# JaronTu/Multimodal_MVD_Seg

Measured on AMD Instinct MI355X. Metric: train-step samples/sec on 4-modality 128^3 patches (PlainConvUNet 3d_fullres, fp32), higher is better.
Workload: dtype f32; 1 GPU; BASELINE configs[1]: PlainConvUNet 3d_fullres 6 stages 31.2M params, 4x128x128x128 patch, 5 classes, fp32, DC+CE deep supervision, SGD-Nesterov+clip; per_gpu_batch=2, global_batch=2, parallelism=dp1, step_launch=one hipGraph replay per step (captured after 3 eager steps)

## Files before the change

include/mvdseg_hip.h:

```cpp
#ifndef MVDSEG_HIP_H
#define MVDSEG_HIP_H
#include <stddef.h>
#include <stdint.h>

#ifdef __cplusplus
extern "C" {
#endif

#define MVD_VERSION 100
#define MVD_MAX_TAPS 27

int mvd_version(void);
const char *mvd_last_error(void);
int mvd_has_mfma(void);
int mvd_set_conv_engine(int mode);
int mvd_set_wino_min_items(long n);

int mvd_pack_weight(const float *w, float *wf, float *wb, int K, int C, int T, int transposed, void *stream);

size_t mvd_conv_fwd_workspace_bytes(int N, long out_voxels, int K);
int mvd_conv3d_fwd(const float *x1, int C1, const float *x2, int C2, const float *wf, const float *bias, float *y,
                   int N, int D, int H, int W, int K, const int ksize[3], const int stride[3], void *ws,
                   size_t ws_bytes, void *stream);
int mvd_conv3d_dgrad(const float *dy, const float *wb, float *dx1, int C1, float *dx2, int C2, int N, int D, int H,
                     int W, int K, const int ksize[3], const int stride[3], void *ws, size_t ws_bytes, void *stream);
int mvd_conv_wino_applicable(int N, int D, int H, int W, int C1, int C2, int K, const int ksize[3], const int stride[3]);
size_t mvd_wino_weight_elems(int C, int K);
int mvd_wino_mode(void);
int mvd_pack_weight_wino(const float *w, float *uf, float *ub, int K, int C, void *stream);
int mvd_pack_weights_batch(int n, const float *const *w, float *const *wf, float *const *wb, float *const *uf,
                           float *const *ub, const int *K, const int *C, const int *T, const int *transposed,
                           void *stream);
int mvd_conv3d_fwd_wino(const float *x1, int C1, const float *x2, int C2, const float *wf, const float *uf,
                        const float *bias, float *y, int N, int D, int H, int W, int K, const int ksize[3],
                        const int stride[3], void *ws, size_t ws_bytes, void *stream);
size_t mvd_conv_stats_tiles(int D, int H, int W);
int mvd_conv3d_fwd_wino_stats(const float *x1, int C1, const float *x2, int C2, const float *wf, const float *uf,
                              const float *bias, float *y, float *stats, int *stats_done, int N, int D, int H, int W,
                              int K, const int ksize[3], const int stride[3], void *ws, size_t ws_bytes, void *stream);
int mvd_conv3d_dgrad_wino(const float *dy, const float *wb, const float *ub, float *dx1, int C1, float *dx2, int C2, int N,
                          int D, int H, int W, int K, const int ksize[3], const int stride[3], void *ws, size_t ws_bytes,
                          void *stream);
int mvd_set_wino3_min_items(long n);
int mvd_conv_wino3_applicable(int N, int D, int H, int W, int C1, int C2, int K, const int ksize[3], const int stride[3]);
size_t mvd_wino3_weight_elems(int C, int K);
int mvd_pack_weight_wino3(const float *w, float *vf, float *vb, int K, int C, void *stream);
int mvd_pack_weights_batch3(int n, const float *const *w, float *const *wf, float *const *wb, float *const *uf,
                            float *const *ub, float *const *vf, float *const *vb, const int *K, const int *C,
                            const int *T, const int *transposed, void *stream);
int mvd_conv3d_fwd_wino3(const float *x1, int C1, const float *x2, int C2, const float *wf, const float *vf,
                         const float *bias, float *y, int N, int D, int H, int W, int K, const int ksize[3],
                         const int stride[3], void *ws, size_t ws_bytes, void *stream);
int mvd_conv3d_fwd_wino3_stats(const float *x1, int C1, const float *x2, int C2, const float *wf, const float *vf,
                               const float *bias, float *y, float *stats, int *stats_done, int N, int D, int H, int W,
                               int K, const int ksize[3], const int stride[3], void *ws, size_t ws_bytes, void *stream);
int mvd_conv3d_dgrad_wino3(const float *dy, const float *wb, const float *vb, float *dx1, int C1, float *dx2, int C2,
                           int N, int D, int H, int W, int K, const int ksize[3], const int stride[3], void *ws,
                           size_t ws_bytes, void *stream);
int mvd_set_wgrad_wino3_min_items(long n);
int mvd_conv_wgrad_wino3_applicable(int N, int D, int H, int W, int C1, int C2, int K, const int ksize[3],
                                    const int stride[3]);
long mvd_wgrad_wino3_launches(void);
size_t mvd_conv3d_wgrad_workspace_bytes(int C, int K, int T, int N, int Do, int Ho, int Wo);
int mvd_conv3d_wgrad(const float *x1, int C1, const float *x2, int C2, const float *dy, float *dw, float *dbias,
                     int N, int D, int H, int W, int K, const int ksize[3], const int stride[3], void *ws,
                     size_t ws_bytes, void *stream);

int mvd_convT3d_fwd(const float *x, const float *wf, const float *bias, float *y, int N, int D, int H, int W, int C,
                    int K, const int stride[3], void *ws, size_t ws_bytes, void *stream);
int mvd_convT3d_dgrad(const float *dy, const float *wb, float *dx, int N, int D, int H, int W, int C, int K,
                      const int stride[3], void *ws, size_t ws_bytes, void *stream);
size_t mvd_convT3d_wgrad_workspace_bytes(int C, int K, int T, int N, int D, int H, int W);
int mvd_convT3d_wgrad(const float *x, const float *dy, float *dw, float *dbias, int N, int D, int H, int W, int C,
                      int K, const int stride[3], void *ws, size_t ws_bytes, void *stream);

int mvd_pack_weight_bf16(const float *w, uint16_t *wf, uint16_t *wb, int K, int C, int T, int transposed, void *stream);
int mvd_pack_weights_bf16_batch(int n, const float *const *w, uint16_t *const *wf, uint16_t *const *wb, const int *K,
                                const int *C, const int *T, const int *transposed, void *stream);
int mvd_pack_weights_bf16_batch_pad(int n, const float *const *w, uint16_t *const *wf, uint16_t *const *wb, const int *K,
                                    const int *C, const int *T, const int *transposed, const int *Csrc, void *stream);
int mvd_conv3d_fwd_bf16(const uint16_t *x1, int C1, const uint16_t *x2, int C2, const uint16_t *wf, const float *bias,
                        uint16_t *y, int N, int D, int H, int W, int K, const int ksize[3], const int stride[3],
                        void *ws, size_t ws_bytes, void *stream);
int mvd_conv3d_dgrad_bf16(const uint16_t *dy, const uint16_t *wb, uint16_t *dx1, int C1, uint16_t *dx2, int C2, int N,
                          int D, int H, int W, int K, const int ksize[3], const int stride[3], void *ws, size_t ws_bytes,
                          void *stream);
int mvd_convT3d_fwd_bf16(const uint16_t *x, const uint16_t *wf, const float *bias, uint16_t *y, int N, int D, int H, int W,
                         int C, int K, const int stride[3], void *ws, size_t ws_bytes, void *stream);
int mvd_convT3d_dgrad_bf16(const uint16_t *dy, const uint16_t *wb, uint16_t *dx, int N, int D, int H, int W, int C, int K,
                           const int stride[3], void *ws, size_t ws_bytes, void *stream);
int mvd_conv3d_wgrad_bf16(const uint16_t *x1, int C1, const uint16_t *x2, int C2, const uint16_t *dy, float *dw,
                          float *dbias, int N, int D, int H, int W, int K, const int ksize[3], const int stride[3],
                          void *ws, size_t ws_bytes, void *stream);
int mvd_convT3d_wgrad_bf16(const uint16_t *x, const uint16_t *dy, float *dw, float *dbias, int N, int D, int H, int W,
                           int C, int K, const int stride[3], void *ws, size_t ws_bytes, void *stream);
// ... 30 lines not shown
                                const float *mean, const float *rstd, void *dx, float *dgamma, float *dbeta, int N,
                                long V, int C, float slope, void *ws, size_t ws_bytes, void *stream);
int mvd_seghead_fwd_bf16(const uint16_t *x, const float *w, const float *bias, float *logits, int N, long V, int C,
                         int K, void *stream);
int mvd_seghead_bwd_bf16(const uint16_t *x, const float *w, const float *dlogits, uint16_t *dx, float *dw, float *dbias,
                         int N, long V, int C, int K, int accumulate, void *ws, size_t ws_bytes, void *stream);
int mvd_seghead_bf16_fused_ok(int N, long V, int C, int K);
int mvd_seghead_fwd_fused(const float *x, const float *mean, const float *rstd, const float *gamma, const float *beta, float slope,
                          const float *w, const float *bias, float *logits, int N, long V, int C, int K, void *stream);
int mvd_seghead_bwd_fused(const float *x, const float *mean, const float *rstd, const float *gamma, const float *beta, float slope,
                          const float *w, const float *dlogits, float *dx, float *dw, float *dbias, int N, long V, int C, int K,
                          int accumulate, void *ws, size_t ws_bytes, void *stream);
int mvd_instnorm_stats_from_tiles(const float *tile_stats, long ntiles, float *mean, float *rstd, int N, long V, int C, float eps,
                                  void *ws, size_t ws_bytes, void *stream);
int mvd_seghead_fwd_bf16_fused(const uint16_t *x, const float *scale, const float *shift, float slope, const float *w,
                               const float *bias, float *logits, int N, long V, int C, int K, void *stream);
int mvd_seghead_bwd_bf16_fused(const uint16_t *x, const float *scale, const float *shift, float slope, const float *w,
                               const float *dlogits, uint16_t *dx, float *dw, float *dbias, int N, long V, int C, int K,
                               int accumulate, void *ws, size_t ws_bytes, void *stream);
int mvd_cast_f32_to_bf16(const float *src, uint16_t *dst, long n, void *stream);
int mvd_cast_bf16_to_f32(const uint16_t *src, float *dst, long n, void *stream);

int mvd_instnorm_nblk(int N, long V, int C);
size_t mvd_instnorm_workspace_bytes(int N, long V, int C);
int mvd_instnorm_lrelu_fwd(const float *x, const float *gamma, const float *beta, float *y, float *mean,
                           float *rstd, int N, long V, int C, float eps, float slope, void *ws, size_t ws_bytes,
                           void *stream);
int mvd_instnorm_lrelu_fwd_prestats(const float *x, const float *tile_stats, long ntiles, const float *gamma,
                                    const float *beta, float *y, float *mean, float *rstd, int N, long V, int C, float eps,
                                    float slope, void *ws, size_t ws_bytes, void *stream);
int mvd_instnorm_lrelu_bwd(const float *x, const float *dy, const float *gamma, const float *beta,
                           const float *mean, const float *rstd, float *dx, float *dgamma, float *dbeta, int N,
                           long V, int C, float slope, void *ws, size_t ws_bytes, void *stream);

int mvd_seghead_fwd(const float *x, const float *w, const float *bias, float *logits, int N, long V, int C, int K,
                    void *stream);
size_t mvd_seghead_bwd_workspace_bytes(int N, long V, int C, int K);
int mvd_seghead_bwd(const float *x, const float *w, const float *dlogits, float *dx, float *dw, float *dbias, int N,
                    long V, int C, int K, int accumulate, void *ws, size_t ws_bytes, void *stream);

size_t mvd_dcce_workspace_bytes(int N, long V, int K);
int mvd_dcce_fwd(const float *logits, const float *target, float *stats , int N, long V, int K, void *ws,
                 size_t ws_bytes, void *stream);
int mvd_dcce_finalize(const float *stats, int N, const float *dstats, int Nd, float *loss, float *coef, long V, int K,
                      int batch_dice, int do_bg, float smooth, float w_ce, float w_dice, void *stream);
int mvd_dcce_bwd(const float *logits, const float *target, const float *coef , const float *gscale_dev,
                 float gscale_host, float *dlogits, int N, long V, int K, float w_ce, void *stream);
int mvd_softmax_select_fwd(const float *logits, float *p_sel, int N, long V, int K, int sel, void *stream);
int mvd_softmax_select_bwd(const float *logits, const float *g, float *dlogits, int N, long V, int K, int sel,
                           void *stream);
int mvd_label_mask(const float *labels, float *mask, long n, float value, void *stream);
int mvd_argmax_counts(const float *logits, const float *target, long long *counts, int N, long V, int K,
                      void *stream);

size_t mvd_kl_workspace_bytes(int N, long V);
int mvd_kl_fwd(const float *ys, const float *yt, float *out, int N, int C, long V, long sn, long sc, long sv,
               float T, float eps_s, int pad_zero_channel, void *ws, size_t ws_bytes, void *stream);
int mvd_kl_bwd(const float *ys, const float *yt, const float *gscale_dev, float gscale_host, float *gs, float *gt,
               int N, int C, long V, long sn, long sc, long sv, float T, float eps_s, int pad_zero_channel,
               void *stream);
int mvd_kl_fwd_bf16(const uint16_t *ys, const uint16_t *yt, float *out, int N, int C, long V, float T, float eps_s,
                    void *ws, size_t ws_bytes, void *stream);
int mvd_kl_bwd_bf16(const uint16_t *ys, const uint16_t *yt, const float *gscale_dev, float gscale_host, uint16_t *gs,
                    uint16_t *gt, int N, int C, long V, float T, float eps_s, void *stream);

size_t mvd_mse_workspace_bytes(long n);
// ... 135 lines not shown
```

multimodal_mvd_seg_amd/_lib.py:

```python
import ctypes
import os
from ctypes import c_float, c_int, c_long, c_size_t, c_uint64, c_void_p

_HERE = os.path.dirname(os.path.abspath(__file__))
LIB_PATH = os.path.join(_HERE, "libmvdseg_hip.so")

_P = c_void_p
_I3 = ctypes.c_int * 3

SIGNATURES = {
    "mvd_version": (c_int, []),
    "mvd_last_error": (ctypes.c_char_p, []),
    "mvd_has_mfma": (c_int, []),
    "mvd_set_conv_engine": (c_int, [c_int]),
    "mvd_set_wino_min_items": (c_int, [c_long]),
    "mvd_pack_weight": (c_int, [_P, _P, _P, c_int, c_int, c_int, c_int, _P]),
    "mvd_conv_fwd_workspace_bytes": (c_size_t, [c_int, c_long, c_int]),
    "mvd_conv3d_fwd": (c_int, [_P, c_int, _P, c_int, _P, _P, _P, c_int, c_int, c_int, c_int, c_int, _I3, _I3, _P,
                               c_size_t, _P]),
    "mvd_conv3d_dgrad": (c_int, [_P, _P, _P, c_int, _P, c_int, c_int, c_int, c_int, c_int, c_int, _I3, _I3, _P,
                                 c_size_t, _P]),
    "mvd_conv3d_wgrad_workspace_bytes": (c_size_t, [c_int, c_int, c_int, c_int, c_int, c_int, c_int]),
    "mvd_conv3d_wgrad": (c_int, [_P, c_int, _P, c_int, _P, _P, _P, c_int, c_int, c_int, c_int, c_int, _I3, _I3, _P,
                                 c_size_t, _P]),
    "mvd_convT3d_fwd": (c_int, [_P, _P, _P, _P, c_int, c_int, c_int, c_int, c_int, c_int, _I3, _P, c_size_t, _P]),
    "mvd_convT3d_dgrad": (c_int, [_P, _P, _P, c_int, c_int, c_int, c_int, c_int, c_int, _I3, _P, c_size_t, _P]),
    "mvd_convT3d_wgrad_workspace_bytes": (c_size_t, [c_int, c_int, c_int, c_int, c_int, c_int, c_int]),
    "mvd_convT3d_wgrad": (c_int, [_P, _P, _P, _P, c_int, c_int, c_int, c_int, c_int, c_int, _I3, _P, c_size_t, _P]),
    "mvd_conv_wino_applicable": (c_int, [c_int, c_int, c_int, c_int, c_int, c_int, c_int, _I3, _I3]),
    "mvd_wino_mode": (c_int, []),
    "mvd_wino_weight_elems": (c_size_t, [c_int, c_int]),
    "mvd_pack_weight_wino": (c_int, [_P, _P, _P, c_int, c_int, _P]),
    "mvd_pack_weights_batch": (c_int, [c_int] + [_P] * 9 + [_P]),
    "mvd_conv3d_fwd_wino": (c_int, [_P, c_int, _P, c_int, _P, _P, _P, _P, c_int, c_int, c_int, c_int, c_int, _I3, _I3, _P,
                                    c_size_t, _P]),
    "mvd_conv_stats_tiles": (c_size_t, [c_int, c_int, c_int]),
    "mvd_conv3d_fwd_wino_stats": (c_int, [_P, c_int, _P, c_int, _P, _P, _P, _P, _P, _P, c_int, c_int, c_int, c_int, c_int,
                                          _I3, _I3, _P, c_size_t, _P]),
    "mvd_conv3d_dgrad_wino": (c_int, [_P, _P, _P, _P, c_int, _P, c_int, c_int, c_int, c_int, c_int, c_int, _I3, _I3, _P,
                                      c_size_t, _P]),
    "mvd_set_wino3_min_items": (c_int, [c_long]),
    "mvd_conv_wino3_applicable": (c_int, [c_int, c_int, c_int, c_int, c_int, c_int, c_int, _I3, _I3]),
    "mvd_wino3_weight_elems": (c_size_t, [c_int, c_int]),
    "mvd_pack_weight_wino3": (c_int, [_P, _P, _P, c_int, c_int, _P]),
    "mvd_pack_weights_batch3": (c_int, [c_int] + [_P] * 11 + [_P]),
    "mvd_conv3d_fwd_wino3": (c_int, [_P, c_int, _P, c_int, _P, _P, _P, _P, c_int, c_int, c_int, c_int, c_int, _I3, _I3, _P,
                                     c_size_t, _P]),
    "mvd_conv3d_fwd_wino3_stats": (c_int, [_P, c_int, _P, c_int, _P, _P, _P, _P, _P, _P, c_int, c_int, c_int, c_int, c_int,
                                           _I3, _I3, _P, c_size_t, _P]),
    "mvd_conv3d_dgrad_wino3": (c_int, [_P, _P, _P, _P, c_int, _P, c_int, c_int, c_int, c_int, c_int, c_int, _I3, _I3, _P,
                                       c_size_t, _P]),
    "mvd_set_wgrad_wino3_min_items": (c_int, [c_long]),
    "mvd_conv_wgrad_wino3_applicable": (c_int, [c_int, c_int, c_int, c_int, c_int, c_int, c_int, _I3, _I3]),
    "mvd_wgrad_wino3_launches": (c_long, []),
    "mvd_conv3d_wgrad_bf16": (c_int, [_P, c_int, _P, c_int, _P, _P, _P, c_int, c_int, c_int, c_int, c_int, _I3, _I3, _P,
                                      c_size_t, _P]),
    "mvd_convT3d_wgrad_bf16": (c_int, [_P, _P, _P, _P, c_int, c_int, c_int, c_int, c_int, c_int, _I3, _P, c_size_t,
                                       _P]),
    "mvd_instnorm_lrelu_fwd_prestats": (c_int, [_P, _P, c_long, _P, _P, _P, _P, _P, c_int, c_long, c_int, c_float, c_float,
                                                _P, c_size_t, _P]),
    "mvd_conv3d_fwd_bf16_stats_tiles": (c_int, [c_int, c_int, c_int, c_int, c_int, c_int, c_int, _I3, _I3]),
    "mvd_set_bf16_zmarch_kernel": (c_int, [c_int]),
    "mvd_set_bf16_wgrad_kernel": (c_int, [c_int]),
    "mvd_conv3d_dgrad_acc_ok": (c_int, [c_int, c_int, c_int, c_int, c_int, c_int, c_int, _I3, _I3]),
    "mvd_conv3d_dgrad_acc": (c_int, [_P, _P, _P, c_int, c_int, c_int, c_int, c_int, c_int, _I3, _I3, _P]),
    "mvd_conv3d_dgrad_bf16_acc": (c_int, [_P, _P, _P, c_int, c_int, c_int, c_int, c_int, c_int, _I3, _I3, _P, c_size_t, _P]),
    "mvd_conv3d_fwd_bf16_prologue_ok": (c_int, [c_int, c_int, c_int, c_int, c_int, c_int, c_int, _I3, _I3]),
    "mvd_conv3d_wgrad_bf16_prologue_ok": (c_int, [c_int, c_int, c_int, c_int, c_int, c_int, c_int, _I3, _I3]),
    "mvd_conv3d_wgrad_bf16_fused": (c_int, [_P, c_int, _P, _P, _P, c_int, c_int, c_int, c_int, c_int, _I3, _I3, _P, _P, c_float,
                                            _P, c_size_t, _P]),
    "mvd_instnorm_stats_bf16": (c_int, [_P, c_int, _P, _P, _P, _P, _P, _P, c_int, c_long, c_int, c_float, _P, c_size_t, _P]),
    "mvd_conv3d_fwd_bf16_fused": (c_int, [_P, c_int, _P, c_int, _P, _P, _P, c_int, c_int, c_int, c_int, c_int, _I3, _I3, _P,
                                          _P, c_float, _P, _P, _P, c_size_t, _P]),
    "mvd_instnorm_finalize_tiles": (c_int, [_P, c_long, _P, _P, _P, _P, _P, _P, c_int, c_long, c_int, c_float, _P]),
    "mvd_instnorm_lrelu_apply_bf16": (c_int, [_P, _P, _P, _P, c_int, c_long, c_int, c_float, _P]),
    "mvd_instnorm_lrelu_fwd_bf16": (c_int, [_P, c_int, _P, _P, _P, _P, _P, c_int, c_long, c_int, c_float, c_float, _P,
                                            c_size_t, _P]),
    "mvd_instnorm_lrelu_bwd_bf16": (c_int, [_P, c_int, _P, _P, _P, _P, _P, _P, _P, _P, c_int, c_long, c_int, c_float, _P,
                                            c_size_t, _P]),
    "mvd_seghead_fwd_bf16": (c_int, [_P, _P, _P, _P, c_int, c_long, c_int, c_int, _P]),
    "mvd_seghead_bwd_bf16": (c_int, [_P, _P, _P, _P, _P, _P, c_int, c_long, c_int, c_int, c_int, _P, c_size_t, _P]),
    "mvd_seghead_bf16_fused_ok": (c_int, [c_int, c_long, c_int, c_int]),
    "mvd_seghead_fwd_fused": (c_int, [_P, _P, _P, _P, _P, c_float, _P, _P, _P, c_int, c_long, c_int, c_int, _P]),
    "mvd_seghead_bwd_fused": (c_int, [_P, _P, _P, _P, _P, c_float, _P, _P, _P, _P, _P, c_int, c_long, c_int, c_int, c_int, _P,
                                      c_size_t, _P]),
    "mvd_instnorm_stats_from_tiles": (c_int, [_P, c_long, _P, _P, c_int, c_long, c_int, c_float, _P, c_size_t, _P]),
    "mvd_seghead_fwd_bf16_fused": (c_int, [_P, _P, _P, c_float, _P, _P, _P, c_int, c_long, c_int, c_int, _P]),
    "mvd_seghead_bwd_bf16_fused": (c_int, [_P, _P, _P, c_float, _P, _P, _P, _P, _P, c_int, c_long, c_int, c_int, c_int, _P,
                                           c_size_t, _P]),
    "mvd_cast_f32_to_bf16": (c_int, [_P, _P, c_long, _P]),
    "mvd_cast_bf16_to_f32": (c_int, [_P, _P, c_long, _P]),
    "mvd_pack_weight_bf16": (c_int, [_P, _P, _P, c_int, c_int, c_int, c_int, _P]),
    "mvd_pack_weights_bf16_batch": (c_int, [c_int] + [_P] * 7 + [_P]),
    "mvd_pack_weights_bf16_batch_pad": (c_int, [c_int] + [_P] * 8 + [_P]),
    "mvd_conv3d_fwd_bf16": (c_int, [_P, c_int, _P, c_int, _P, _P, _P, c_int, c_int, c_int, c_int, c_int, _I3, _I3, _P,
                                    c_size_t, _P]),
    "mvd_conv3d_dgrad_bf16": (c_int, [_P, _P, _P, c_int, _P, c_int, c_int, c_int, c_int, c_int, c_int, _I3, _I3, _P,
                                      c_size_t, _P]),
    "mvd_convT3d_fwd_bf16": (c_int, [_P, _P, _P, _P, c_int, c_int, c_int, c_int, c_int, c_int, _I3, _P, c_size_t, _P]),
    "mvd_convT3d_dgrad_bf16": (c_int, [_P, _P, _P, c_int, c_int, c_int, c_int, c_int, c_int, _I3, _P, c_size_t, _P]),
    "mvd_instnorm_nblk": (c_int, [c_int, c_long, c_int]),
    "mvd_instnorm_workspace_bytes": (c_size_t, [c_int, c_long, c_int]),
    "mvd_instnorm_lrelu_fwd": (c_int, [_P, _P, _P, _P, _P, _P, c_int, c_long, c_int, c_float, c_float, _P, c_size_t, _P]),
    "mvd_instnorm_lrelu_bwd": (c_int, [_P, _P, _P, _P, _P, _P, _P, _P, _P, c_int, c_long, c_int, c_float, _P, c_size_t,
                                       _P]),
    "mvd_seghead_fwd": (c_int, [_P, _P, _P, _P, c_int, c_long, c_int, c_int, _P]),
    "mvd_seghead_bwd_workspace_bytes": (c_size_t, [c_int, c_long, c_int, c_int]),
    "mvd_seghead_bwd": (c_int, [_P, _P, _P, _P, _P, _P, c_int, c_long, c_int, c_int, c_int, _P, c_size_t, _P]),
    "mvd_dcce_workspace_bytes": (c_size_t, [c_int, c_long, c_int]),
    "mvd_dcce_fwd": (c_int, [_P, _P, _P, c_int, c_long, c_int, _P, c_size_t, _P]),
    "mvd_dcce_finalize": (c_int, [_P, c_int, _P, c_int, _P, _P, c_long, c_int, c_int, c_int, c_float, c_float, c_float,
                                  _P]),
    "mvd_dcce_bwd": (c_int, [_P, _P, _P, _P, c_float, _P, c_int, c_long, c_int, c_float, _P]),
    "mvd_argmax_counts": (c_int, [_P, _P, _P, c_int, c_long, c_int, _P]),
    "mvd_softmax_select_fwd": (c_int, [_P, _P, c_int, c_long, c_int, c_int, _P]),
    "mvd_softmax_select_bwd": (c_int, [_P, _P, _P, c_int, c_long, c_int, c_int, _P]),
    "mvd_label_mask": (c_int, [_P, _P, c_long, c_float, _P]),
    "mvd_cldice_combine": (c_int, [_P, _P, c_float, _P]),
    "mvd_kl_workspace_bytes": (c_size_t, [c_int, c_long]),
    "mvd_kl_fwd": (c_int, [_P, _P, _P, c_int, c_int, c_long, c_long, c_long, c_long, c_float, c_float, c_int, _P,
                           c_size_t, _P]),
    "mvd_kl_bwd": (c_int, [_P, _P, _P, c_float, _P, _P, c_int, c_int, c_long, c_long, c_long, c_long, c_float, c_float,
                           c_int, _P]),
    "mvd_kl_fwd_bf16": (c_int, [_P, _P, _P, c_int, c_int, c_long, c_float, c_float, _P, c_size_t, _P]),
    "mvd_kl_bwd_bf16": (c_int, [_P, _P, _P, c_float, _P, _P, c_int, c_int, c_long, c_float, c_float, _P]),
    "mvd_mse_workspace_bytes": (c_size_t, [c_long]),
    "mvd_mse_fwd": (c_int, [_P, _P, _P, c_long, _P, c_size_t, _P]),
    "mvd_mse_bwd": (c_int, [_P, _P, _P, _P, _P, c_long, _P]),
    "mvd_soft_erode_fwd": (c_int, [_P, _P, _P, c_int, c_int, c_int, c_int, _P]),
    "mvd_soft_erode_bwd": (c_int, [_P, _P, _P, c_int, c_int, c_int, c_int, _P]),
    "mvd_soft_dilate_fwd": (c_int, [_P, _P, _P, c_int, c_int, c_int, c_int, _P]),
    "mvd_soft_dilate_bwd": (c_int, [_P, _P, _P, c_int, c_int, c_int, c_int, _P]),
    "mvd_skel_update_fwd": (c_int, [_P, _P, _P, _P, c_long, c_int, _P]),
    "mvd_skel_update_bwd": (c_int, [_P, _P, _P, _P, _P, _P, _P, c_long, c_int, _P]),
    "mvd_skel_iter_fwd": (c_int, [_P] * 8 + [c_int] * 5 + [_P]),
    "mvd_dot_sum": (c_int, [_P, _P, _P, c_long, _P, c_size_t, _P]),
    "mvd_dot_sum_workspace_bytes": (c_size_t, [c_long]),
    "mvd_cc_label": (c_int, [_P, _P, _P, c_int, c_int, c_int, c_int, _P]),
# ... 95 lines not shown
```

multimodal_mvd_seg_amd/csrc/conv.hip:

```cpp
#include "common.h"
#include "conv_geom.h"

namespace mvd {

static int g_engine_mode = 0;
#define g_wino_off (wino_mode() == 0)
static const int g_transp_off = getenv("MVD_TRANSP") ? (atoi(getenv("MVD_TRANSP")) == 0) : 0;
static long g_wino_min_items = getenv("MVD_WINO_MIN") ? atol(getenv("MVD_WINO_MIN")) : 256;
static const long kWino3MinItemsDefault = 128;
static long g_wino3_min_items = getenv("MVD_WINO3_MIN") ? atol(getenv("MVD_WINO3_MIN")) : kWino3MinItemsDefault;
static long wino3_items(int D, int H, int W, int K) { return (long)((D + 3) / 4) * ((H + 7) / 8) * ((W + 7) / 8) * (K / 32); }

__global__ void k_fwd_scalar(FwdGeom g, const float *__restrict__ a1, const float *__restrict__ a2,
                             const float *__restrict__ w, const float *__restrict__ bias, float *__restrict__ y1,
                             float *__restrict__ y2) {
    const int K = g.K1 + g.K2, C = g.C1 + g.C2;
    const int CK = wl_ck(C);
    const long total = (long)g.N * g.Do * g.Ho * g.Wo * K;
    for (long idx = (long)blockIdx.x * blockDim.x + threadIdx.x; idx < total; idx += (long)gridDim.x * blockDim.x) {
        int k = (int)(idx % K);
        long r = idx / K;
        int ow = (int)(r % g.Wo);
        r /= g.Wo;
        int oh = (int)(r % g.Ho);
// ... 235 lines not shown
        }
    }
    return 0;
}

static void conv_fwd_geom(FwdGeom &g, int N, int D, int H, int W, int C1, int C2, int K, const int ks[3],
                          const int st[3]) {
    memset(&g, 0, sizeof(g));
    g.N = N;
    g.Di = D; g.Hi = H; g.Wi = W;
    g.Do = out_dim(D, ks[0], st[0]); g.Ho = out_dim(H, ks[1], st[1]); g.Wo = out_dim(W, ks[2], st[2]);
    g.Dy = g.Do; g.Hy = g.Ho; g.Wy = g.Wo;
    g.C1 = C1; g.C2 = C2; g.K1 = K; g.K2 = 0;
    int t = 0;
    for (int a = 0; a < ks[0]; a++)
        for (int b = 0; b < ks[1]; b++)
            for (int c = 0; c < ks[2]; c++) {
                g.off[t][0] = a - (ks[0] - 1) / 2;
                g.off[t][1] = b - (ks[1] - 1) / 2;
                g.off[t][2] = c - (ks[2] - 1) / 2;
                g.wt[t] = t;
                t++;
            }
    g.ntaps = g.T = t;
    for (int a = 0; a < 3; a++) {
        g.sa[a] = st[a];
        g.so[a] = 1;
        g.oo[a] = 0;
    }
}

static int run_fwd(const FwdGeom &g, const float *a1, const float *a2, const float *w, const float *bias, float *y1,
                   float *y2, void *ws, size_t ws_bytes, hipStream_t s, const float *u = nullptr, float *stats = nullptr,
                   int *stats_done = nullptr, bool u3d = false) {
    if (stats_done) *stats_done = 0;
    if (u3d) {
        if (g_engine_mode == 0 && u && !g_wino_off && wino3_enabled() &&
            wino3_items(g.Do, g.Ho, g.Wo, g.K1 + g.K2) >= g_wino3_min_items) {
            int r = fwd_wino3(g, a1, a2, u, bias, y1, y2, s, stats, stats_done);
            if (r >= 0) return r;
            if (stats_done) *stats_done = 0;
        }
        u = nullptr;
    }
    if (g_engine_mode == 0 && u && !g_wino_off) {
        const long tiles = (long)g.N * ((g.Do + 3) / 4) * ((g.Ho + 3) / 4) * ((g.Wo + 7) / 8) * ((g.K1 + g.K2) / 32);
        if (tiles >= g_wino_min_items) {
            int r = fwd_wino(g, a1, a2, u, bias, y1, y2, s, stats, stats_done);
            if (r >= 0) return r;
            if (stats_done) *stats_done = 0;
        }
    }
    if (g_engine_mode == 0) {
        int r = fwd_mfma(g, a1, a2, w, bias, y1, y2, ws, ws_bytes, s);
        if (r >= 0) return r;
    }
    return fwd_scalar(g, a1, a2, w, bias, y1, y2, s);
}

static int run_wgrad(const WgradGeom &g, const float *a1, const float *a2, const float *b, float *dw, void *ws,
                     size_t ws_bytes, hipStream_t s, float *dbias = nullptr, int *dbias_done = nullptr) {
    if (dbias_done) *dbias_done = 0;
    if (g_engine_mode == 0) {
        int r = wgrad_mfma(g, a1, a2, b, dw, ws, ws_bytes, s, false, dbias, dbias_done);
        if (r >= 0) return r;
        if (dbias_done) *dbias_done = 0;
    }
    return wgrad_scalar(g, a1, a2, b, dw, ws, ws_bytes, s);
// ... 19 lines not shown
                       size_t ws_bytes, hipStream_t s, float *dbias = nullptr, int *dbias_done = nullptr) {
    int r = wgrad_mfma(g, reinterpret_cast<const float *>(a1), reinterpret_cast<const float *>(a2),
                       reinterpret_cast<const float *>(b), dw, ws, ws_bytes, s, true, dbias, dbias_done);
    if (r < 0) {
        set_error("bf16 wgrad: unsupported shape (needs C %% 32 == 0 and K %% 32 == 0; C=%d+%d K=%d)", g.C1, g.C2, g.K);
        return 3;
    }
    return r;
}

static size_t max_sz(size_t a, size_t b) { return a > b ? a : b; }

}

using namespace mvd;

extern "C" {

int mvd_set_conv_engine(int mode) {
    g_engine_mode = mode ? 1 : 0;
    return 0;
}

int mvd_set_wino_min_items(long n) {
    g_wino_min_items = n < 0 ? 256 : n;
    return 0;
}

size_t mvd_conv_fwd_workspace_bytes(int N, long out_voxels, int K) { return fwd_mfma_ws(N, out_voxels, K); }

static int conv3d_fwd_impl(const float *x1, int C1, const float *x2, int C2, const float *wf, const float *uf,
                           const float *bias, float *y, int N, int D, int H, int W, int K, const int ksize[3],
                           const int stride[3], void *ws, size_t ws_bytes, void *stream, float *stats = nullptr,
                           int *stats_done = nullptr, bool u3d = false) {
    MVD_REQUIRE(x1 && wf && y && C1 > 0 && C2 >= 0 && (C2 == 0 || x2), "conv3d_fwd: null pointer / bad channels");
    MVD_REQUIRE(N > 0 && D > 0 && H > 0 && W > 0 && K > 0, "conv3d_fwd: bad shape");
    if (check_ks(ksize, stride, "conv3d_fwd")) return 2;
    FwdGeom g;
    conv_fwd_geom(g, N, D, H, W, C1, C2, K, ksize, stride);
    return run_fwd(g, x1, x2, wf, bias, y, nullptr, ws, ws_bytes, as_stream(stream), uf, stats, stats_done, u3d);
}

int mvd_conv3d_fwd(const float *x1, int C1, const float *x2, int C2, const float *wf, const float *bias, float *y, int N,
                   int D, int H, int W, int K, const int ksize[3], const int stride[3], void *ws, size_t ws_bytes,
                   void *stream) {
    return conv3d_fwd_impl(x1, C1, x2, C2, wf, nullptr, bias, y, N, D, H, W, K, ksize, stride, ws, ws_bytes, stream);
}

int mvd_conv3d_fwd_wino(const float *x1, int C1, const float *x2, int C2, const float *wf, const float *uf,
                        const float *bias, float *y, int N, int D, int H, int W, int K, const int ksize[3],
                        const int stride[3], void *ws, size_t ws_bytes, void *stream) {
    return conv3d_fwd_impl(x1, C1, x2, C2, wf, uf, bias, y, N, D, H, W, K, ksize, stride, ws, ws_bytes, stream);
}

int mvd_conv_wino_applicable(int N, int D, int H, int W, int C1, int C2, int K, const int ksize[3], const int stride[3]) {
    if (g_engine_mode != 0 || g_wino_off) return 0;
    for (int a = 0; a < 3; a++)
        if (ksize[a] != 3 || stride[a] != 1) return 0;
    if (C1 % 32 || C2 % 32 || K % 32 || C1 <= 0 || K <= 0) return 0;
    const long tiles_f = (long)N * ((D + 3) / 4) * ((H + 3) / 4) * ((W + 7) / 8) * (K / 32);
    const long tiles_b = (long)N * ((D + 3) / 4) * ((H + 3) / 4) * ((W + 7) / 8) * ((C1 + C2) / 32);
    return (tiles_f >= g_wino_min_items ? 1 : 0) | (tiles_b >= g_wino_min_items ? 2 : 0);
}

size_t mvd_wino_weight_elems(int C, int K) { return wino_weight_elems(C, K); }
int mvd_wino_mode(void) { return wino_mode(); }

size_t mvd_conv_stats_tiles(int D, int H, int W) { return (size_t)((D + 3) / 4) * ((H + 3) / 4) * ((W + 7) / 8); }

int mvd_conv3d_fwd_wino_stats(const float *x1, int C1, const float *x2, int C2, const float *wf, const float *uf,
                              const float *bias, float *y, float *stats, int *stats_done, int N, int D, int H, int W,
                              int K, const int ksize[3], const int stride[3], void *ws, size_t ws_bytes, void *stream) {
    MVD_REQUIRE(stats_done, "conv3d_fwd_wino_stats: stats_done is required");
    return conv3d_fwd_impl(x1, C1, x2, C2, wf, uf, bias, y, N, D, H, W, K, ksize, stride, ws, ws_bytes, stream, stats,
                           stats_done);
}

int mvd_pack_weights_batch(int n, const float *const *w, float *const *wf, float *const *wb, float *const *uf,
                           float *const *ub, const int *K, const int *C, const int *T, const int *transposed,
                           void *stream) {
    MVD_REQUIRE(n > 0 && w && wf && wb && uf && ub && K && C && T && transposed, "pack_weights_batch: null table");
    for (int q = 0; q < n; q++) {
        MVD_REQUIRE(w[q] && (wf[q] || wb[q] || uf[q] || ub[q]), "pack_weights_batch: job without source or destination");
        MVD_REQUIRE(K[q] > 0 && C[q] > 0 && T[q] > 0 && T[q] <= MVD_MAX_TAPS, "pack_weights_batch: bad K / C / T");
        if (uf[q] || ub[q]) {
            MVD_REQUIRE(wino_mode() == 2, "pack_weights_batch: Winograd tables need MVD_WINO=2 (F(2x2,3x3) layout)");
            MVD_REQUIRE(T[q] == 27 && !transposed[q] && K[q] % 32 == 0 && C[q] % 32 == 0,
                        "pack_weights_batch: Winograd tables need a 3x3x3 conv with C %% 32 == 0 and K %% 32 == 0");
        }
    }
    return pack_weights_batch(n, w, wf, wb, uf, ub, K, C, T, transposed, as_stream(stream));
}

int mvd_pack_weight_wino(const float *w, float *uf, float *ub, int K, int C, void *stream) {
    MVD_REQUIRE(w && (uf || ub) && K > 0 && C > 0, "pack_weight_wino: bad arguments");
    MVD_REQUIRE(K % 32 == 0 && C % 32 == 0, "pack_weight_wino: needs C %% 32 == 0 and K %% 32 == 0");
    return pack_weight_wino(w, uf, ub, K, C, as_stream(stream));
}

int mvd_set_wino3_min_items(long n) {
    g_wino3_min_items = n < 0 ? kWino3MinItemsDefault : n;
    return 0;
}

int mvd_conv_wino3_applicable(int N, int D, int H, int W, int C1, int C2, int K, const int ksize[3], const int stride[3]) {
    if (!wino3_enabled()) return 0;
    const int two = mvd_conv_wino_applicable(N, D, H, W, C1, C2, K, ksize, stride);
    return two & ((wino3_items(D, H, W, K) >= g_wino3_min_items ? 1 : 0) |
// ... 149 lines not shown
    g.ntaps = g.T = t;
    for (int a = 0; a < 3; a++) {
        g.sa[a] = st[a];
        g.sb[a] = 1;
    }
    g.transposed_out = 0;
}

size_t mvd_conv3d_wgrad_workspace_bytes(int C, int K, int T, int N, int Do, int Ho, int Wo) {
    WgradGeom g;
    memset(&g, 0, sizeof(g));
    g.N = N; g.Do = Do; g.Ho = Ho; g.Wo = Wo; g.C1 = C; g.C2 = 0; g.K = K; g.ntaps = g.T = T;
    size_t a = max_sz(wgrad_scalar_ws(g), wgrad_mfma_ws(g));
    return max_sz(a, colsum_ws((long)N * Do * Ho * Wo, K));
}

int mvd_set_wgrad_wino3_min_items(long n) {
    set_wgrad_wino3_min_items(n);
    return 0;
}

int mvd_conv_wgrad_wino3_applicable(int N, int D, int H, int W, int C1, int C2, int K, const int ksize[3],
                                    const int stride[3]) {
    if (N <= 0 || D <= 0 || H <= 0 || W <= 0 || C1 <= 0 || C2 < 0 || K <= 0 || !ksize || !stride) return 0;
    for (int a = 0; a < 3; a++)
        if (ksize[a] != 3 || stride[a] != 1) return 0;
    WgradGeom g;
    conv_wgrad_geom(g, N, D, H, W, C1, C2, K, ksize, stride);
    return wgrad_wino3_selected(g) ? 1 : 0;
}

long mvd_wgrad_wino3_launches(void) { return wgrad_wino3_launches(); }

int mvd_conv3d_wgrad(const float *x1, int C1, const float *x2, int C2, const float *dy, float *dw, float *dbias, int N,
                     int D, int H, int W, int K, const int ksize[3], const int stride[3], void *ws, size_t ws_bytes,
                     void *stream) {
    MVD_REQUIRE(x1 && dy && dw && ws && C1 > 0 && C2 >= 0 && (C2 == 0 || x2), "conv3d_wgrad: null pointer / bad channels");
    MVD_REQUIRE(N > 0 && D > 0 && H > 0 && W > 0 && K > 0, "conv3d_wgrad: bad shape");
    if (check_ks(ksize, stride, "conv3d_wgrad")) return 2;
    WgradGeom g;
    conv_wgrad_geom(g, N, D, H, W, C1, C2, K, ksize, stride);
    MVD_REQUIRE(ws_bytes >= mvd_conv3d_wgrad_workspace_bytes(C1 + C2, K, g.T, N, g.Do, g.Ho, g.Wo),
                "conv3d_wgrad: workspace too small");
    hipStream_t s = as_stream(stream);
    int dbias_done = 0;
    int r = run_wgrad(g, x1, x2, dy, dw, ws, ws_bytes, s, dbias, &dbias_done);
    if (r) return r;
    if (dbias && !dbias_done) return colsum(dy, dbias, (long)N * g.Do * g.Ho * g.Wo, K, ws, s);
    return 0;
}

int mvd_convT3d_fwd(const float *x, const float *wf, const float *bias, float *y, int N, int D, int H, int W, int C, int K,
                    const int stride[3], void *ws, size_t ws_bytes, void *stream) {
    MVD_REQUIRE(x && wf && y && N > 0 && D > 0 && H > 0 && W > 0 && C > 0 && K > 0, "convT3d_fwd: bad arguments");
    for (int a = 0; a < 3; a++) MVD_REQUIRE(stride[a] == 1 || stride[a] == 2, "convT3d_fwd: stride must be 1 or 2");
    if (g_engine_mode == 0 && !g_transp_off) {
        int r = convT_fwd_direct(x, wf, bias, y, N, D, H, W, C, K, stride, as_stream(stream));
        if (r >= 0) return r;
    }
    for (int pd = 0; pd < stride[0]; pd++)
        for (int ph = 0; ph < stride[1]; ph++)
            for (int pw = 0; pw < stride[2]; pw++) {
                FwdGeom g;
                memset(&g, 0, sizeof(g));
                g.N = N;
                g.Di = g.Do = D; g.Hi = g.Ho = H; g.Wi = g.Wo = W;
// ... 53 lines not shown
    g.C1 = C; g.C2 = 0; g.K = K;
    int t = 0;
    for (int pd = 0; pd < st[0]; pd++)
        for (int ph = 0; ph < st[1]; ph++)
            for (int pw = 0; pw < st[2]; pw++) {
                g.ob[t][0] = pd; g.ob[t][1] = ph; g.ob[t][2] = pw;
                g.wt[t] = t;
                t++;
            }
    g.ntaps = g.T = t;
    for (int a = 0; a < 3; a++) {
        g.sa[a] = 1;
        g.sb[a] = st[a];
    }
    g.transposed_out = 1;
}

size_t mvd_convT3d_wgrad_workspace_bytes(int C, int K, int T, int N, int D, int H, int W) {
    WgradGeom g;
    memset(&g, 0, sizeof(g));
    g.N = N; g.Do = D; g.Ho = H; g.Wo = W; g.C1 = C; g.K = K; g.ntaps = g.T = T;
    size_t a = max_sz(wgrad_scalar_ws(g), wgrad_mfma_ws(g));
    return max_sz(a, colsum_ws((long)N * D * H * W * T, K));
}

int mvd_convT3d_wgrad(const float *x, const float *dy, float *dw, float *dbias, int N, int D, int H, int W, int C, int K,
                      const int stride[3], void *ws, size_t ws_bytes, void *stream) {
    MVD_REQUIRE(x && dy && dw && ws && N > 0 && D > 0 && H > 0 && W > 0 && C > 0 && K > 0, "convT3d_wgrad: bad arguments");
    for (int a = 0; a < 3; a++) MVD_REQUIRE(stride[a] == 1 || stride[a] == 2, "convT3d_wgrad: stride must be 1 or 2");
    WgradGeom g;
    convT_wgrad_geom(g, N, D, H, W, C, K, stride);
    MVD_REQUIRE(ws_bytes >= mvd_convT3d_wgrad_workspace_bytes(C, K, g.T, N, D, H, W), "convT3d_wgrad: workspace too small");
    hipStream_t s = as_stream(stream);
    if (dbias) {
        int r = colsum(dy, dbias, (long)N * g.Db * g.Hb * g.Wb, K, ws, s);
        if (r) return r;
    }
    return run_wgrad(g, x, nullptr, dy, dw, ws, ws_bytes, s);
}

int mvd_pack_weight_bf16(const float *w, uint16_t *wf, uint16_t *wb, int K, int C, int T, int transposed, void *stream) {
    MVD_REQUIRE(w && (wf || wb) && K > 0 && C > 0 && T > 0 && T <= MVD_MAX_TAPS, "pack_weight_bf16: bad arguments");
    MVD_REQUIRE(!wf || C % 32 == 0, "pack_weight_bf16: wf needs C %% 32 == 0");
    MVD_REQUIRE(!wb || K % 32 == 0, "pack_weight_bf16: wb needs K %% 32 == 0");
    return pack_weight16(w, wf, wb, K, C, T, transposed, as_stream(stream));
}

int mvd_pack_weights_bf16_batch(int n, const float *const *w, uint16_t *const *wf, uint16_t *const *wb, const int *K,
                                const int *C, const int *T, const int *transposed, void *stream) {
    MVD_REQUIRE(n > 0 && w && wf && wb && K && C && T && transposed, "pack_weights_bf16_batch: null table");
    for (int q = 0; q < n; q++) {
        MVD_REQUIRE(w[q] && (wf[q] || wb[q]), "pack_weights_bf16_batch: job without source or destination");
        MVD_REQUIRE(K[q] > 0 && C[q] > 0 && T[q] > 0 && T[q] <= MVD_MAX_TAPS, "pack_weights_bf16_batch: bad K / C / T");
        MVD_REQUIRE(!wf[q] || C[q] % 32 == 0, "pack_weights_bf16_batch: wf needs C %% 32 == 0");
        MVD_REQUIRE(!wb[q] || K[q] % 32 == 0, "pack_weights_bf16_batch: wb needs K %% 32 == 0");
    }
    return pack_weights16_batch(n, w, reinterpret_cast<unsigned short *const *>(wf), reinterpret_cast<unsigned short *const *>(wb),
                                K, C, T, transposed, nullptr, as_stream(stream));
}

int mvd_pack_weights_bf16_batch_pad(int n, const float *const *w, uint16_t *const *wf, uint16_t *const *wb, const int *K,
                                    const int *C, const int *T, const int *transposed, const int *Csrc, void *stream) {
    MVD_REQUIRE(n > 0 && w && wf && wb && K && C && T && transposed && Csrc, "pack_weights_bf16_batch_pad: null table");
    for (int q = 0; q < n; q++) {
        MVD_REQUIRE(w[q] && (wf[q] || wb[q]), "pack_weights_bf16_batch_pad: job without source or destination");
        MVD_REQUIRE(K[q] > 0 && C[q] > 0 && T[q] > 0 && T[q] <= MVD_MAX_TAPS, "pack_weights_bf16_batch_pad: bad K / C / T");
        MVD_REQUIRE(Csrc[q] > 0 && Csrc[q] <= C[q], "pack_weights_bf16_batch_pad: needs 0 < Csrc <= C");
        MVD_REQUIRE(Csrc[q] == C[q] || !transposed[q], "pack_weights_bf16_batch_pad: no padding for transposed-conv weights");
        MVD_REQUIRE(!wf[q] || C[q] % 32 == 0, "pack_weights_bf16_batch_pad: wf needs C %% 32 == 0");
        MVD_REQUIRE(!wb[q] || K[q] % 32 == 0, "pack_weights_bf16_batch_pad: wb needs K %% 32 == 0");
    }
// ... 305 lines not shown
```

multimodal_mvd_seg_amd/csrc/conv_geom.h:

```cpp
#pragma once
#include <stdint.h>

namespace mvd {

__host__ __device__ inline int wl_ck(int C) {
    return (C % 32 == 0) ? 32 : ((C % 8 == 0) ? 8 : ((C % 4 == 0) ? 4 : 0));
}
__host__ __device__ inline size_t widx(int CK, int T, int C, int K, int t, int c, int k) {
    if (CK == 0) return ((size_t)t * C + c) * K + k;
    const int hh = CK / 2;
    const int cc = c / CK, r = c % CK;
    return ((((size_t)cc * T + t) * 2 + r / hh) * K + k) * hh + (r % hh);
}

struct FwdGeom {
    int N;
    int T;
    int Di, Hi, Wi;
    int Do, Ho, Wo;
    int Dy, Hy, Wy;
    int C1, C2, K1, K2;
    int ntaps;
    int sa[3], so[3], oo[3];
    int8_t off[27][3];
    int8_t wt[27];
    int8_t acc;
};

struct WgradGeom {
    int N;
    int Di, Hi, Wi;
    int Db, Hb, Wb;
    int Do, Ho, Wo;
    int C1, C2, K;
    int ntaps;
    int T;
    int sa[3], sb[3];
    int8_t off[27][3], ob[27][3];
    int8_t wt[27];
    int transposed_out;
};

int fwd_scalar(const FwdGeom &g, const float *a1, const float *a2, const float *w, const float *bias, float *y1,
               float *y2, hipStream_t s);
size_t fwd_mfma_ws(int N, long out_vox, int K);
int fwd_mfma(const FwdGeom &g, const float *a1, const float *a2, const float *w, const float *bias, float *y1, float *y2,
             void *ws, size_t ws_bytes, hipStream_t s);
size_t wgrad_scalar_ws(const WgradGeom &g);
int wgrad_scalar(const WgradGeom &g, const float *a1, const float *a2, const float *b, float *dw, void *ws,
                 size_t ws_bytes, hipStream_t s);
size_t wgrad_mfma_ws(const WgradGeom &g);
int wgrad_mfma(const WgradGeom &g, const float *a1, const float *a2, const float *b, float *dw, void *ws, size_t ws_bytes,
               hipStream_t s, bool bf16_in = false, float *dbias = nullptr, int *dbias_done = nullptr);

int fwd_wino(const FwdGeom &g, const float *a1, const float *a2, const float *u, const float *bias, float *y1, float *y2,
             hipStream_t s, float *stats = nullptr, int *stats_done = nullptr);
int pack_weight_wino(const float *w, float *uf, float *ub, int K, int C, hipStream_t s);
int fwd_wino3(const FwdGeom &g, const float *a1, const float *a2, const float *u, const float *bias, float *y1, float *y2,
              hipStream_t s, float *stats = nullptr, int *stats_done = nullptr);
int pack_weight_wino3(const float *w, float *uf, float *ub, int K, int C, hipStream_t s);
int wino3_enabled();
int dgrad32s(int N, int D, int H, int W, int C, int K, int Do, int Ho, int Wo, const float *dy, const float *wb, float *dx,
             hipStream_t s, int accumulate = 0);
int dgrad16s(int N, int D, int H, int W, int C, int K, int Do, int Ho, int Wo, const unsigned short *dy, const unsigned short *wb,
             unsigned short *dx, hipStream_t s, int accumulate = 0);
int launch_fwd16ys(const FwdGeom &g, const unsigned short *a1, const unsigned short *a2, const unsigned short *w, const float *bias,
                   unsigned short *y1, unsigned short *y2, hipStream_t s, int ncu);
int wgrad16z(const WgradGeom &g, const unsigned short *a1, const unsigned short *a2, const unsigned short *b, void *ws,
             size_t ws_bytes, bool want_bias, int *nsplit_out, float **pbias_out, hipStream_t s, const float *in_scale = nullptr,
             const float *in_shift = nullptr, float slope = 0.f);
int wgrad16z_run(const WgradGeom &g, const unsigned short *a1, const unsigned short *a2, const unsigned short *b, float *dw, void *ws,
                 size_t ws_bytes, hipStream_t s, float *dbias, int *dbias_done, const float *in_scale, const float *in_shift,
                 float slope);
bool wgrad16z_prologue_ok(const WgradGeom &g);
int wgrad16zs(const WgradGeom &g, const unsigned short *a1, const unsigned short *a2, const unsigned short *b, void *ws,
              size_t ws_bytes, int *nsplit_out, hipStream_t s);
void wgrad16z_enable(int on);
int pack_weights_batch(int n, const float *const *w, float *const *wf, float *const *wb, float *const *uf, float *const *ub,
                       const int *K, const int *C, const int *T, const int *transposed, hipStream_t s,
                       float *const *vf = nullptr, float *const *vb = nullptr);
int wino_mode();
int wgrad_wino3(const WgradGeom &g, const float *a1, const float *a2, const float *b, float *dw, void *ws, size_t ws_bytes,
                int nsplit, hipStream_t s, float *dbias, int *dbias_done);
bool wgrad_wino3_selected(const WgradGeom &g);
size_t wgrad_wino3_ws(int nsplit, int C, int K);
int wgrad_wino3_enabled();
void set_wgrad_wino3_min_items(long n);
long wgrad_wino3_launches();
int dbias_reduce(const float *pbias, float *dbias, int K, int nrows, hipStream_t s);
size_t wino_weight_elems(int C, int K);

int convT_fwd_direct(const float *x, const float *wf, const float *bias, float *y, int N, int D, int H, int W, int C, int K,
                     const int st[3], hipStream_t s);
int convT_dgrad_direct(const float *dy, const float *wb, float *dx, int N, int D, int H, int W, int C, int K,
                       const int st[3], hipStream_t s);

int convT_fwd_direct16(const unsigned short *x, const unsigned short *wf, const float *bias, unsigned short *y, int N, int D,
                       int H, int W, int C, int K, const int st[3], hipStream_t s);
int convT_dgrad_direct16(const unsigned short *dy, const unsigned short *wb, unsigned short *dx, int N, int D, int H, int W,
                         int C, int K, const int st[3], hipStream_t s);

struct Fwd16Fuse {
    float *tile_stats = nullptr;
    int *ntiles = nullptr;
    const float *in_scale = nullptr, *in_shift = nullptr;
    float slope = 0.01f;
};
int fwd_bf16(const FwdGeom &g, const unsigned short *a1, const unsigned short *a2, const unsigned short *w,
             const float *bias, unsigned short *y1, unsigned short *y2, void *ws, size_t ws_bytes, hipStream_t s,
             const Fwd16Fuse *fuse = nullptr);
int fwd16y_enabled();
void fwd16y_enable(int on);
int launch_fwd16y(const FwdGeom &g, const unsigned short *a1, const unsigned short *a2, const unsigned short *w,
                  const float *bias, unsigned short *y1, unsigned short *y2, hipStream_t s, const Fwd16Fuse *fuse, int ncu,
                  int *stats_tiles_only);
int fwd_bf16_stats_tiles(const FwdGeom &g);
int fwd_bf16_prologue_ok(const FwdGeom &g);
int pack_weight16(const float *w, unsigned short *wf, unsigned short *wb, int K, int C, int T, int transposed,
                  hipStream_t s);
int pack_weights16_batch(int n, const float *const *w, unsigned short *const *wf, unsigned short *const *wb, const int *K,
// ... 4 lines not shown
```

multimodal_mvd_seg_amd/csrc/conv_mfma.hip:

```cpp
#include <stdlib.h>
#include <type_traits>

#include "common.h"
#include "conv_geom.h"

namespace mvd {

typedef float f32x16 __attribute__((ext_vector_type(16)));

struct FwdTile {
    int ED, EH, EW, nslots;
    int min_off[3];
    int ntd, nth, ntw;
    int K;
    int toff[27];
    int dbg;
};

__device__ __forceinline__ void store_tile32(const FwdGeom &g, const f32x16 &acc, float bv, int n, int od, int ohb, int ow0,
                                             int k, int hh, int S, int split, int Ktot, float *__restrict__ part,
                                             float *__restrict__ y1, float *__restrict__ y2) {
    const int owl = ow0 + 4 * hh;
    if (S > 1) {
        float *pl = part + (size_t)(4 * hh) * Ktot + k;
// ... 5 lines not shown
            if (oh < g.Ho && owl + (r & 3) < g.Wo) pl[uo] = acc[r];
        }
    } else if (g.K2 == 0 || g.K1 == g.K2) {
        const int Ks = g.K1;
        float *yl = (k < g.K1 ? y1 + k : y2 + (k - g.K1)) + (size_t)(4 * hh * g.so[2]) * Ks;
        const size_t pb = ((size_t)n * g.Dy + (od * g.so[0] + g.oo[0])) * g.Hy;
#pragma unroll
        for (int r = 0; r < 16; r++) {
            const int oh = ohb + (r >> 2), owu = ow0 + (r & 3);
            const size_t uo = ((pb + (oh * g.so[1] + g.oo[1])) * g.Wy + (owu * g.so[2] + g.oo[2])) * Ks;
            if (oh < g.Ho && owl + (r & 3) < g.Wo) yl[uo] = acc[r] + bv;
        }
    } else {
#pragma unroll
        for (int r = 0; r < 16; r++) {
            const int oh = ohb + (r >> 2), ow = owl + (r & 3);
            if (oh < g.Ho && ow < g.Wo) {
                const size_t ov = (((size_t)n * g.Dy + (od * g.so[0] + g.oo[0])) * g.Hy + (oh * g.so[1] + g.oo[1])) * g.Wy +
                                  (ow * g.so[2] + g.oo[2]);
                const float val = acc[r] + bv;
                if (k < g.K1)
                    y1[ov * g.K1 + k] = val;
                else
                    y2[ov * g.K2 + (k - g.K1)] = val;
            }
        }
    }
}

template <int CK, int NT, int MT, bool L32>
__global__ __launch_bounds__(256, 2) void k_fwd_mfma(const FwdGeom g, const FwdTile tg, const float *__restrict__ a1,
                                                     const float *__restrict__ a2, const float *__restrict__ w,
                                                     const float *__restrict__ bias, float *__restrict__ y1,
                                                     float *__restrict__ y2, const int S, float *__restrict__ part) {
    extern __shared__ __attribute__((aligned(16))) float lds[];
    constexpr int HH = CK / 2;
    constexpr int KT = 32 * NT;
    float *Xs = lds;
    float *Ws = lds + (size_t)tg.nslots * CK;
    int *tapoff = reinterpret_cast<int *>(Ws + (size_t)g.ntaps * 2 * KT * HH);
    int *wts = tapoff + 32;

    const int tid = threadIdx.x, lane = tid & 63;
    const int wave = __builtin_amdgcn_readfirstlane(tid >> 6);
    const int i = lane & 31, h = lane >> 5;
    const int tile = blockIdx.x;
    const int tw_ = tile % tg.ntw, th_ = (tile / tg.ntw) % tg.nth, td_ = tile / (tg.ntw * tg.nth);
    const int nkb = tg.K / (32 * NT);
    const int kb = blockIdx.y % nkb, split = blockIdx.y / nkb, n = blockIdx.z;
    const int od0 = td_ * 4, oh0 = th_ * (4 * MT), ow0 = tw_ * 8;
    const int iz0 = od0 * g.sa[0] + tg.min_off[0], iy0 = oh0 * g.sa[1] + tg.min_off[1],
              ix0 = ow0 * g.sa[2] + tg.min_off[2];
#pragma unroll
    for (int t = 0; t < 27; t++)
        if (tid == t && t < g.ntaps) {
            tapoff[t] = tg.toff[t];
            wts[t] = g.wt[t];
        }

    f32x16 acc[MT][NT];
#pragma unroll
    for (int m = 0; m < MT; m++)
#pragma unroll
        for (int q = 0; q < NT; q++)
#pragma unroll
            for (int r = 0; r < 16; r++) acc[m][q][r] = 0.f;

// ... 78 lines not shown
#pragma unroll
            for (int m = 0; m < MT; m++) {
                const float *pa = Xs + (size_t)(sbase[m] + to) * CK + h * HH;
                if (CK == 8) {
                    float4 q = *reinterpret_cast<const float4 *>(pa);
                    af[m][0] = q.x; af[m][1] = q.y; af[m][HH - 2] = q.z; af[m][HH - 1] = q.w;
                } else {
                    float2 q = *reinterpret_cast<const float2 *>(pa);
                    af[m][0] = q.x; af[m][1] = q.y;
                }
            }
#pragma unroll
            for (int q_ = 0; q_ < NT; q_++) {
                const float *pb = Ws + ((size_t)(t * 2 + h) * KT + q_ * 32 + i) * HH;
                if (CK == 8) {
                    float4 q = *reinterpret_cast<const float4 *>(pb);
                    bf[q_][0] = q.x; bf[q_][1] = q.y; bf[q_][HH - 2] = q.z; bf[q_][HH - 1] = q.w;
                } else {
                    float2 q = *reinterpret_cast<const float2 *>(pb);
                    bf[q_][0] = q.x; bf[q_][1] = q.y;
                }
            }
#pragma unroll
            for (int e = 0; e < HH; e++)
#pragma unroll
                for (int m = 0; m < MT; m++)
#pragma unroll
                    for (int q_ = 0; q_ < NT; q_++)
                        acc[m][q_] = __builtin_amdgcn_mfma_f32_32x32x2f32(af[m][e], bf[q_][e], acc[m][q_], 0, 0, 0);
        }
    }

    const int od = od0 + wave;
    if (od >= g.Do) return;
#pragma unroll
    for (int m = 0; m < MT; m++)
#pragma unroll
        for (int q_ = 0; q_ < NT; q_++) {
            const int k = kb * KT + q_ * 32 + i;
            const float bv = settled((bias && S == 1) ? bias[k] : 0.f);
            store_tile32(g, acc[m][q_], bv, n, od, oh0 + 4 * m, ow0, k, h, S, split, tg.K, part, y1, y2);
        }
}

static const size_t LDS_LIMIT = 160 * 1024;
static const int MAX_SPLIT = 16;

__global__ void k_split_reduce(const FwdGeom g, const float *__restrict__ part, const float *__restrict__ bias,
                               float *__restrict__ y1, float *__restrict__ y2, int S) {
    const int K = g.K1 + g.K2;
    const size_t per = (size_t)g.N * g.Do * g.Ho * g.Wo * K;
    for (size_t idx = (size_t)blockIdx.x * blockDim.x + threadIdx.x; idx < per; idx += (size_t)gridDim.x * blockDim.x) {
        float s = bias ? bias[idx % K] : 0.f;
        int j = 0;
        for (; j + 3 < S; j += 4) {
            const float p0 = part[(size_t)j * per + idx], p1 = part[(size_t)(j + 1) * per + idx];
            const float p2 = part[(size_t)(j + 2) * per + idx], p3 = part[(size_t)(j + 3) * per + idx];
            s += p0;
            s += p1;
            s += p2;
            s += p3;
        }
        for (; j < S; j++) s += part[(size_t)j * per + idx];
        const int k = (int)(idx % K);
        size_t r = idx / K;
        const int ow = (int)(r % g.Wo);
// ... 172 lines not shown
#pragma unroll
                            for (int c4 = 0; c4 < 4; c4++)
#pragma unroll
                                for (int m = 0; m < MT; m++)
#pragma unroll
                                    for (int q = 0; q < NT; q++) {
                                        const float avv = c4 == 0 ? af[m][e].x : (c4 == 1 ? af[m][e].y : (c4 == 2 ? af[m][e].z : af[m][e].w));
                                        const float bvv = c4 == 0 ? bf[q][e].x : (c4 == 1 ? bf[q][e].y : (c4 == 2 ? bf[q][e].z : bf[q][e].w));
                                        acc[m][q] = __builtin_amdgcn_mfma_f32_32x32x2f32(avv, bvv, acc[m][q], 0, 0, 0);
                                    }
                        }
                    }
                }
            }
        }
    }
    const int od = od0 + wave;
    if (od >= g.Do) return;
#pragma unroll
    for (int m = 0; m < MT; m++)
#pragma unroll
        for (int q = 0; q < NT; q++) {
            const int k = kb * KT + q * 32 + i;
            const float bv = settled((bias && tg.S == 1) ? bias[k] : 0.f);
            store_tile32(g, acc[m][q], bv, n, od, oh0 + 4 * m, ow0, k, h, tg.S, split, tg.K, part, y1, y2);
        }
}

constexpr int SXR = 12;
constexpr int SXB = 6;
__global__ __launch_bounds__(512, 1) void k_fwd32s(const FwdGeom g, const Fwd32Tile tg, const float *__restrict__ a1,
                                                   const float *__restrict__ a2, const float *__restrict__ w,
                                                   const float *__restrict__ bias, float *__restrict__ y1,
                                                   float *__restrict__ y2) {
    extern __shared__ __attribute__((aligned(16))) float Xs[];
    constexpr int XS = 36;
    const int tid = threadIdx.x, lane = tid & 63;
    const int wave = __builtin_amdgcn_readfirstlane(tid >> 6);
    const int i = lane & 31, h = lane >> 5;
    const int per_xcd = (tg.nitems + 7) >> 3;
    const int item = (int)(blockIdx.x & 7) * per_xcd + (int)(blockIdx.x >> 3);
    if (item >= tg.nitems) return;
    unsigned r_ = (unsigned)item;
    const int kb = (int)(r_ % (unsigned)tg.nkb); r_ /= (unsigned)tg.nkb;
    const int tw_ = (int)(r_ % (unsigned)tg.ntw); r_ /= (unsigned)tg.ntw;
    const int th_ = (int)(r_ % (unsigned)tg.nth); r_ /= (unsigned)tg.nth;
    const int td_ = (int)(r_ % (unsigned)tg.ntd);
    const int n = (int)(r_ / (unsigned)tg.ntd);

    const int C = g.C1 + g.C2;
    const int nch = C >> 5;
    const int EHW = tg.EH * tg.EW;
    const int nx = tg.nslots * 8;
    const int od0 = td_ * 2, oh0 = th_ * 4, ow0 = tw_ * 8;
    const int iz0 = od0 * 2 + tg.min_off[0], iy0 = oh0 * 2 + tg.min_off[1], ix0 = ow0 * 2 + tg.min_off[2];
    const int dl = wave & 1, kh = (wave >> 1) & 1, tap_half = wave >> 2;
    const int tb = tap_half ? 14 : 0, nt = tap_half ? g.ntaps - 14 : 14;
    const int sbase = ((2 * dl) * tg.EH + 2 * (i >> 3)) * tg.EW + 2 * (i & 7);
    const float4 *xlane = reinterpret_cast<const float4 *>(Xs + (size_t)sbase * XS + h * 16);
    const int kcol = kb * 64 + kh * 32 + i;
    const float *wlane = w + (((size_t)h * tg.K + kcol) << 4);
    const size_t wtap = (size_t)2 * tg.K * 16;

    const bool fastst = tg.EH == 9 && tg.EW == 17 && tg.nslots == 765;
    const int r3 = tid / 136, rem = tid - r3 * 136;
    const int sx = rem >> 3, part = rem & 7;
    const bool st_act = tid < 408;
// ... 93 lines not shown
#pragma unroll
                    for (int e = 0; e < 4; e++)
                        wb[(u + 3) & 3][e] =
                            *reinterpret_cast<const float4 *>(wc + (size_t)__builtin_amdgcn_readlane(wt_l, tn) * wtap + e * 4);
                    const float4 *pa = xlane + (size_t)__builtin_amdgcn_readlane(toff_l, sidx + 1 < nt ? t + 1 : tb + nt - 1) * (XS / 4);
#pragma unroll
                    for (int e = 0; e < 4; e++) af[(u + 1) & 1][e] = pa[e];
#pragma unroll
                    for (int e = 0; e < 4; e++) {
                        acc = __builtin_amdgcn_mfma_f32_32x32x2f32(af[u & 1][e].x, wb[u][e].x, acc, 0, 0, 0);
                        acc = __builtin_amdgcn_mfma_f32_32x32x2f32(af[u & 1][e].y, wb[u][e].y, acc, 0, 0, 0);
                        acc = __builtin_amdgcn_mfma_f32_32x32x2f32(af[u & 1][e].z, wb[u][e].z, acc, 0, 0, 0);
                        acc = __builtin_amdgcn_mfma_f32_32x32x2f32(af[u & 1][e].w, wb[u][e].w, acc, 0, 0, 0);
                    }
                    __builtin_amdgcn_sched_barrier(0);
                }
            }
        }
    }
    __syncthreads();
    if (tap_half) {
        float *xo = Xs + (size_t)(wave & 3) * 1024 + lane;
#pragma unroll
        for (int r = 0; r < 16; r++) xo[r * 64] = acc[r];
    }
    __syncthreads();
    if (tap_half) return;
    {
        const float *xi = Xs + (size_t)wave * 1024 + lane;
#pragma unroll
        for (int r = 0; r < 16; r++) acc[r] += xi[r * 64];
    }
    const int od = od0 + dl;
    if (od >= g.Do) return;
    const float bv = settled(bias ? bias[kcol] : 0.f);
#pragma unroll
    for (int r = 0; r < 16; r++) {
        const int row = (r & 3) + 8 * (r >> 2) + 4 * h;
        const int oh = oh0 + (row >> 3), ow = ow0 + (row & 7);
        if (oh < g.Ho && ow < g.Wo) {
            const size_t ov = (((size_t)n * g.Dy + od) * g.Hy + oh) * g.Wy + ow;
            const float val = acc[r] + bv;
            if (kcol < g.K1)
                y1[ov * g.K1 + kcol] = val;
            else
                y2[ov * g.K2 + (kcol - g.K1)] = val;
        }
    }
}

struct Dg2Tile {
    int ntd, nth, ntw, ncb, nitems, C;
    int acc;
};
__global__ __launch_bounds__(512, 2) void k_dgrad32s(const FwdGeom g, const Dg2Tile tg, const float *__restrict__ dy,
                                                     const float *__restrict__ wb, float *__restrict__ dx) {
    __shared__ __attribute__((aligned(16))) float Xs[135 * 36];
    constexpr int XS = 36;
    const int tid = threadIdx.x, lane = tid & 63;
    const int wave = __builtin_amdgcn_readfirstlane(tid >> 6);
    const int i = lane & 31, h = lane >> 5;
    const int per_xcd = (tg.nitems + 7) >> 3;
    const int item = (int)(blockIdx.x & 7) * per_xcd + (int)(blockIdx.x >> 3);
    if (item >= tg.nitems) return;
    unsigned r_ = (unsigned)item;
    const int cb = (int)(r_ % (unsigned)tg.ncb); r_ /= (unsigned)tg.ncb;
    const int tw_ = (int)(r_ % (unsigned)tg.ntw); r_ /= (unsigned)tg.ntw;
    const int th_ = (int)(r_ % (unsigned)tg.nth); r_ /= (unsigned)tg.nth;
// ... 90 lines not shown
        for (int r = 0; r < 16; r++) {
            const int iy = 2 * (oy0 + (r >> 2)) + py, ixu = 2 * (ox0 + (r & 3)) + px;
            const size_t uo = ((((size_t)n * g.Dy + iz) * g.Hy + iy) * g.Wy + ixu) * C;
            if (iz < g.Dy && iy < g.Hy && ixu + 8 * h < g.Wy) xl[uo] = tg.acc ? xl[uo] + acc[m][r] : acc[m][r];
        }
    }
}

int dgrad32s(int N, int D, int H, int W, int C, int K, int Do, int Ho, int Wo, const float *dy, const float *wb, float *dx,
             hipStream_t s, int accumulate) {
    if (C % 32 || K % 32 || (((uintptr_t)dy | (uintptr_t)wb) & 15)) return -1;
    if ((long)Do * Ho * Wo * K * 4 >= (1L << 31)) return -1;
    FwdGeom g;
    memset(&g, 0, sizeof(g));
    g.N = N;
    g.Di = Do; g.Hi = Ho; g.Wi = Wo;
    g.Dy = D; g.Hy = H; g.Wy = W;
    g.C1 = K;
    Dg2Tile tg;
    tg.ntd = (Do + 1) / 2; tg.nth = (Ho + 3) / 4; tg.ntw = (Wo + 7) / 8;
    tg.ncb = C / 32;
    tg.C = C;
    tg.acc = accumulate;
    const long nitems = (long)N * tg.ntd * tg.nth * tg.ntw * tg.ncb;
    if (nitems > (1L << 30)) return -1;
    tg.nitems = (int)nitems;
    const unsigned grid = (unsigned)(((nitems + 7) / 8) * 8);
    hipLaunchKernelGGL(k_dgrad32s, dim3(grid), dim3(512), 0, s, g, tg, dy, wb, dx);
    return check_launch("conv dgrad (stride 2, fused parity classes)");
}

static int num_cus();
static int launch_fwd32s(const FwdGeom &g, const float *a1, const float *a2, const float *w, const float *bias, float *y1,
                         float *y2, hipStream_t s) {
    const int K = g.K1 + g.K2;
    Fwd32Tile tg;
    memset(&tg, 0, sizeof(tg));
    int mn[3] = {127, 127, 127}, mx[3] = {-127, -127, -127};
    for (int t = 0; t < g.ntaps; t++)
        for (int a = 0; a < 3; a++) {
            if (g.off[t][a] < mn[a]) mn[a] = g.off[t][a];
            if (g.off[t][a] > mx[a]) mx[a] = g.off[t][a];
        }
    const int T3[3] = {2, 4, 8};
    int E[3];
    for (int a = 0; a < 3; a++) {
        E[a] = (T3[a] - 1) * 2 + (mx[a] - mn[a]) + 1;
        tg.min_off[a] = mn[a];
    }
    tg.EH = E[1]; tg.EW = E[2];
    tg.nslots = E[0] * E[1] * E[2];
    if (tg.nslots > SXR * 64 || g.ntaps != 27) return -1;
    int m = (1 << 16) / tg.EW + 1;
    for (int nn = 0; nn < tg.EH * tg.EW; nn++)
        if (((nn * m) >> 16) != nn / tg.EW) return -1;
    tg.magW = m;
    for (int t = 0; t < g.ntaps; t++)
        tg.toff[t] = ((g.off[t][0] - mn[0]) * tg.EH + (g.off[t][1] - mn[1])) * tg.EW + (g.off[t][2] - mn[2]);
    tg.ntd = (g.Do + 1) / 2;
    tg.nth = (g.Ho + 3) / 4;
    tg.ntw = (g.Wo + 7) / 8;
    tg.nkb = K / 64;
    tg.K = K;
    const long nitems = (long)g.N * tg.ntd * tg.nth * tg.ntw * tg.nkb;
    if (nitems > (1L << 30)) return -1;
    tg.nitems = (int)nitems;
    const size_t lds = (size_t)tg.nslots * 36 * sizeof(float);
    static PerDeviceFlag cfgd;
    if (!cfgd()) {
        if (hipFuncSetAttribute(reinterpret_cast<const void *>(k_fwd32s), hipFuncAttributeMaxDynamicSharedMemorySize,
                                (int)LDS_LIMIT) != hipSuccess) {
            set_error("conv fwd (stride 2): cannot raise the dynamic LDS limit");
            return 1;
        }
        cfgd() = true;
    }
    const unsigned grid = (unsigned)(((nitems + 7) / 8) * 8);
    hipLaunchKernelGGL(k_fwd32s, dim3(grid), dim3(512), lds, s, g, tg, a1, a2, w, bias, y1, y2);
    return check_launch("conv fwd (stride 2, CK=32)");
}

static int num_cus() {
    static int n = 0;
    if (!n) {
        hipDeviceProp_t p;
        int dev = 0;
        if (hipGetDevice(&dev) == hipSuccess && hipGetDeviceProperties(&p, dev) == hipSuccess) n = p.multiProcessorCount;
        if (n <= 0) n = 256;
    }
    return n;
}

static int split_for(const void *ws, size_t ws_bytes, long wgs, int nch, size_t out_elems, int nkb) {
    int S = 1;
    if (ws && wgs < 256 && nch >= 4) {
        long want = 512 / wgs;
        if (want > MAX_SPLIT) want = MAX_SPLIT;
        if (want > nch / 2) want = nch / 2;
        while (want > 1 && (size_t)want * out_elems * sizeof(float) > ws_bytes) want--;
        if (want > 1 && (long)nkb * want <= 65535) S = (int)want;
    }
    return S;
}

static int run_split_reduce(const FwdGeom &g, const float *part, const float *bias, float *y1, float *y2, int S,
                            size_t out_elems, hipStream_t s) {
    long blocks = cdiv((long)out_elems, 256);
    if (blocks > 2048) blocks = 2048;
    hipLaunchKernelGGL(k_split_reduce, dim3(blocks), dim3(256), 0, s, g, part, bias, y1, y2, S);
    return check_launch("conv fwd split reduce");
}

template <int NT, int TG>
static int launch_fwd32(const FwdGeom &g, Fwd32Tile &tg, const float *a1, const float *a2, const float *w,
                        const float *bias, float *y1, float *y2, void *ws, size_t ws_bytes, hipStream_t s) {
    auto kern = k_fwd32<NT, TG>;
    constexpr int XR = 12;
    const size_t lds = ((size_t)XR * 32 * 36 + 2 * (size_t)TG * 2 * (32 * NT) * 20) * 4;
    static PerDeviceFlag configured;
    if (!configured()) {
        if (hipFuncSetAttribute(reinterpret_cast<const void *>(kern), hipFuncAttributeMaxDynamicSharedMemorySize,
                                (int)LDS_LIMIT) != hipSuccess) {
            set_error("conv fwd32 (mfma): cannot raise the dynamic LDS limit");
            return 1;
        }
        configured() = true;
    }
    const int K = g.K1 + g.K2;
    tg.nkb = K / (32 * NT);
    const long tiles = (long)tg.ntd * tg.nth * tg.ntw;
    const size_t out_elems = (size_t)g.N * g.Do * g.Ho * g.Wo * K;
    tg.S = split_for(ws, ws_bytes, tiles * tg.nkb * g.N, (g.C1 + g.C2) / 32, out_elems, tg.nkb);
    const long nitems = tiles * tg.nkb * tg.S * g.N;
    if (nitems > (1L << 30)) return -1;
    tg.nitems = (int)nitems;
    const long grid = ((nitems + 7) / 8) * 8;
    float *part = reinterpret_cast<float *>(ws);
    hipLaunchKernelGGL(kern, dim3((unsigned)grid), dim3(256), lds, s, g, tg, a1, a2, w, bias, y1, y2, part);
    if (check_launch("conv fwd32 (mfma)")) return 1;
    if (tg.S > 1) return run_split_reduce(g, part, bias, y1, y2, tg.S, out_elems, s);
    return 0;
}

template <int CK, int NT, int MT, bool L32>
static int launch_fwd(const FwdGeom &g, FwdTile &tg, size_t lds, const float *a1, const float *a2, const float *w,
                      const float *bias, float *y1, float *y2, void *ws, size_t ws_bytes, hipStream_t s) {
    auto kern = k_fwd_mfma<CK, NT, MT, L32>;
    static size_t configured = 0;
    if (lds > configured) {
        if (hipFuncSetAttribute(reinterpret_cast<const void *>(kern), hipFuncAttributeMaxDynamicSharedMemorySize,
                                (int)LDS_LIMIT) != hipSuccess) {
            set_error("conv fwd (mfma): cannot raise the dynamic LDS limit");
            return 1;
        }
        configured = LDS_LIMIT;
    }
    const int K = g.K1 + g.K2;
    const int nkb = K / (32 * NT);
    const long tiles = (long)tg.ntd * tg.nth * tg.ntw;
    const size_t out_elems = (size_t)g.N * g.Do * g.Ho * g.Wo * K;
    const int S = split_for(ws, ws_bytes, tiles * nkb * g.N, (g.C1 + g.C2) / CK, out_elems, nkb);
    dim3 grid((unsigned)tiles, nkb * S, g.N);
    float *part = reinterpret_cast<float *>(ws);
    hipLaunchKernelGGL(kern, grid, dim3(256), lds, s, g, tg, a1, a2, w, bias, y1, y2, S, part);
    if (check_launch("conv fwd (mfma)")) return 1;
    if (S > 1) return run_split_reduce(g, part, bias, y1, y2, S, out_elems, s);
    return 0;
}

int fwd_mfma(const FwdGeom &g, const float *a1, const float *a2, const float *w, const float *bias, float *y1, float *y2,
             void *ws, size_t ws_bytes, hipStream_t s) {
    const int C = g.C1 + g.C2, K = g.K1 + g.K2;
    const int LCK = wl_ck(C);
    if (LCK == 0 || g.ntaps < 1 || g.ntaps > 27) return -1;
    if (g.C1 % LCK != 0 || g.C2 % LCK != 0) return -1;
    if (K % 32 != 0 || g.K1 % 32 != 0 || g.K2 % 32 != 0) return -1;
    if (g.N > 65535 || K / 32 > 65535) return -1;
    if (((uintptr_t)a1 | (uintptr_t)a2 | (uintptr_t)w) & 15) return -1;
    static int dbg = -1;
    if (dbg < 0) dbg = getenv("MVD_CONV_DBG") ? atoi(getenv("MVD_CONV_DBG")) : 0;
    int mn[3] = {127, 127, 127}, mx[3] = {-127, -127, -127};
    for (int t = 0; t < g.ntaps; t++)
        for (int a = 0; a < 3; a++) {
            if (g.off[t][a] < mn[a]) mn[a] = g.off[t][a];
            if (g.off[t][a] > mx[a]) mx[a] = g.off[t][a];
        }
    const bool unit_stride = g.sa[0] == 1 && g.sa[1] == 1 && g.sa[2] == 1;
    if (LCK == 32 && unit_stride && !(dbg & 4)) {
        static int nt_rule = -1;
        if (nt_rule < 0) nt_rule = getenv("MVD_CONV_NT") ? atoi(getenv("MVD_CONV_NT")) : 1;
        const long wg64 = (long)g.N * ((g.Do + 3) / 4) * ((g.Ho + 3) / 4) * ((g.Wo + 7) / 8) * (K / 64);
        const int NT = (K % 64 == 0 && !(nt_rule == 1 && wg64 < 128)) ? 2 : 1;
        Fwd32Tile t32;
        memset(&t32, 0, sizeof(t32));
        t32.dbg = dbg;
        const int T3[3] = {4, 4, 8};
        int E[3];
        for (int a = 0; a < 3; a++) {
            E[a] = (T3[a] - 1) + (mx[a] - mn[a]) + 1;
            t32.min_off[a] = mn[a];
        }
        t32.EH = E[1]; t32.EW = E[2];
        t32.nslots = E[0] * E[1] * E[2];
        auto magic = [](int d, int nmax) -> int {
            int m = (1 << 16) / d + 1;
            for (int n = 0; n < nmax; n++)
                if (((n * m) >> 16) != n / d) return -1;
            return m;
        };
        t32.magHW = magic(t32.EH * t32.EW, t32.nslots);
        t32.magW = magic(t32.EW, t32.EH * t32.EW);
        if (t32.nslots <= 12 * 32 && t32.magHW > 0 && t32.magW > 0) {
            for (int t = 0; t < g.ntaps; t++)
                t32.toff[t] = ((g.off[t][0] - mn[0]) * t32.EH + (g.off[t][1] - mn[1])) * t32.EW + (g.off[t][2] - mn[2]);
            t32.ntd = (g.Do + 3) / 4;
            t32.nth = (g.Ho + 3) / 4;
            t32.ntw = (g.Wo + 7) / 8;
            t32.K = K;
            if (NT == 2) return launch_fwd32<2, 1>(g, t32, a1, a2, w, bias, y1, y2, ws, ws_bytes, s);
            return launch_fwd32<1, 2>(g, t32, a1, a2, w, bias, y1, y2, ws, ws_bytes, s);
        }
    }
    if (LCK == 32 && g.sa[0] == 2 && g.sa[1] == 2 && g.sa[2] == 2 && g.ntaps == 27 && g.T == 27 && K % 64 == 0 &&
        g.K1 % 64 == 0 && g.so[0] == 1 && g.so[1] == 1 && g.so[2] == 1 && g.oo[0] == 0 && g.oo[1] == 0 && g.oo[2] == 0 &&
        !(dbg & 8)) {
        const long items = (long)g.N * ((g.Do + 1) / 2) * ((g.Ho + 3) / 4) * ((g.Wo + 7) / 8) * (K / 64);
        if (items >= 256) {
            int r = launch_fwd32s(g, a1, a2, w, bias, y1, y2, s);
            if (r >= 0) return r;
        }
    }
    const int CK = LCK == 32 ? 8 : LCK;
    FwdTile tg;
    memset(&tg, 0, sizeof(tg));
    tg.dbg = dbg;
    tg.K = K;
    const int cand[3][2] = {{2, 2}, {2, 1}, {1, 1}};
    for (int ci = 0; ci < 3; ci++) {
        const int MT = cand[ci][0], NT = cand[ci][1];
        if (K % (32 * NT) != 0) continue;
        const int T3[3] = {4, 4 * MT, 8};
        int E[3];
        for (int a = 0; a < 3; a++) {
            E[a] = (T3[a] - 1) * g.sa[a] + (mx[a] - mn[a]) + 1;
            tg.min_off[a] = mn[a];
        }
        tg.ED = E[0]; tg.EH = E[1]; tg.EW = E[2];
        tg.nslots = E[0] * E[1] * E[2];
        const size_t lds = ((size_t)tg.nslots * CK + (size_t)g.ntaps * 2 * (32 * NT) * (CK / 2)) * 4 + 64 * 4;
        const bool fits2 = lds <= LDS_LIMIT / 2;
        const bool last = (ci == 2);
        if (!fits2 && !(last && lds <= LDS_LIMIT)) {
            if (!last) continue;
            return -1;
        }
        for (int t = 0; t < g.ntaps; t++)
            tg.toff[t] = ((g.off[t][0] - mn[0]) * tg.EH + (g.off[t][1] - mn[1])) * tg.EW + (g.off[t][2] - mn[2]);
        tg.ntd = (g.Do + 3) / 4;
        tg.nth = (g.Ho + 4 * MT - 1) / (4 * MT);
        tg.ntw = (g.Wo + 7) / 8;
#define MVD_FWD_DISPATCH(CKV, L32V)                                                                                      \
    {                                                                                                                    \
        if (MT == 2 && NT == 2) return launch_fwd<CKV, 2, 2, L32V>(g, tg, lds, a1, a2, w, bias, y1, y2, ws, ws_bytes, s); \
        if (MT == 2 && NT == 1) return launch_fwd<CKV, 1, 2, L32V>(g, tg, lds, a1, a2, w, bias, y1, y2, ws, ws_bytes, s); \
        return launch_fwd<CKV, 1, 1, L32V>(g, tg, lds, a1, a2, w, bias, y1, y2, ws, ws_bytes, s);                         \
    }
        if (LCK == 32) MVD_FWD_DISPATCH(8, true)
        else if (CK == 8) MVD_FWD_DISPATCH(8, false)
        else MVD_FWD_DISPATCH(4, false)
#undef MVD_FWD_DISPATCH
    }
    return -1;
}

struct WgTile {
    int TD, TH, TW, lTH, lTW;
    int EAh, EAw, nslotsA, minA[3];
    int EBh, EBw, nslotsB, minB[3];
    int magAw, magAhw, magBw, magBhw;
    int ntd, nth, ntw, nsplit, nkb;
    int ntiles;
    int toffA[27], toffB[27];
    int dbg;
};

template <int TPW, int NA, int NB, int SH>
__global__ __launch_bounds__(512, 1) void k_wgrad_mfma(const WgradGeom g, const WgTile tg, const float *__restrict__ a1,
                                                       const float *__restrict__ a2, const float *__restrict__ b,
                                                       float *__restrict__ partial, float *__restrict__ pbias) {
    extern __shared__ __attribute__((aligned(16))) float lds[];
    float *As = lds;
    float *Bs = lds + (size_t)NA * 2048;
    const int tid = threadIdx.x, lane = tid & 63;
    const int wave8 = __builtin_amdgcn_readfirstlane(tid >> 6);
    const int wave = wave8 & 3, grp = wave8 >> 2;
    const int i = lane & 31, h = lane >> 5;
    const int cb = blockIdx.y / tg.nkb, kb = blockIdx.y % tg.nkb;
    const int split = blockIdx.x;
// ... 126 lines not shown
                rb[u] = make_float4(0.f, 0.f, 0.f, 0.f);
                if (bok && idx < nb && !(tg.dbg & 1) && id >= 0 && id < g.Db && ih >= 0 && ih < g.Hb && iw >= 0 && iw < g.Wb) {
                    const size_t e = ((((size_t)n * g.Db + id) * g.Hb + ih) * g.Wb + iw) * K + k0 + part * 4;
                    rb[u] = *reinterpret_cast<const float4 *>(b + e);
                }
            }
        }
    };
    constexpr int IMG = (NA + NB) * 2048;
    auto store_tile = [&](int par) {
#pragma unroll
        for (int u = 0; u < NA; u++) *reinterpret_cast<float4 *>(As + par * IMG + (size_t)(u * 512 + tid) * 4) = ra[u];
#pragma unroll
        for (int u = 0; u < NB; u++) *reinterpret_cast<float4 *>(Bs + par * IMG + (size_t)(u * 512 + tid) * 4) = rb[u];
    };
    int aoff[TPW], boff[TPW];
#pragma unroll
    for (int j = 0; j < TPW; j++) {
        aoff[j] = ta[j] * 128 + i * 4 + h * g.sa[2] * 128;
        boff[j] = tb[j] * 128 + i * 4 + h * g.sb[2] * 128;
    }
    const char *Ab = reinterpret_cast<const char *>(As), *Bb = reinterpret_cast<const char *>(Bs);
    constexpr int NAV = SH == 2 ? 1 : TPW, NBV = SH == 1 ? 1 : TPW;
    auto read_ops = [&](int s2, float (&av)[NAV], float (&bv)[NBV]) {
        const int v = s2 < TV ? s2 : TV - 2;
        const int wx = v & (tg.TW - 1), hy = (v >> tg.lTW) & (tg.TH - 1), dz = v >> (tg.lTW + tg.lTH);
        const int sa_ = (((dz * g.sa[0]) * tg.EAh + hy * g.sa[1]) * tg.EAw + wx * g.sa[2]) * 128;
        const int sb_ = (((dz * g.sb[0]) * tg.EBh + hy * g.sb[1]) * tg.EBw + wx * g.sb[2]) * 128;
#pragma unroll
        for (int j = 0; j < NAV; j++) av[j] = *reinterpret_cast<const float *>(Ab + sa_ + aoff[j]);
#pragma unroll
        for (int j = 0; j < NBV; j++) bv[j] = *reinterpret_cast<const float *>(Bb + sb_ + boff[j]);
    };
    const bool dob = SH == 1 && pbias != nullptr && cb == 0 && wave == 0;
    float bsum = 0.f;
    auto mfmas = [&](const float (&av)[NAV], const float (&bv)[NBV]) {
#pragma unroll
        for (int j = 0; j < TPW; j++)
            acc[j] = __builtin_amdgcn_mfma_f32_32x32x2f32(av[SH == 2 ? 0 : j], bv[SH == 1 ? 0 : j], acc[j], 0, 0, 0);
        if (SH == 1 && dob) bsum += bv[0];
    };
    auto interleave = [&]() {
#pragma unroll
        for (int j = 0; j < TPW; j++) {
            __builtin_amdgcn_sched_group_barrier(0x008, 1, 0);
            __builtin_amdgcn_sched_group_barrier(0x100, 2, 0);
            __builtin_amdgcn_sched_group_barrier(0x002, 4, 0);
        }
    };

    int tile = split, par = 0;
    if (tile < tg.ntiles) load_tile(tile);
    if (db) {
        if (tile < tg.ntiles) store_tile(0);
        __syncthreads();
    }
    while (tile < tg.ntiles) {
        if (!db) {
            __syncthreads();
            store_tile(0);
            __syncthreads();
        }
        const int next = tile + tg.nsplit;
        if (db) load_tile_buf(next);
        else if (next < tg.ntiles) load_tile(next);
        if (!(tg.dbg & 2)) {
            float a0[NAV], b0[NBV], a1_[NAV], b1_[NBV];
            read_ops(2 * grp, a0, b0);
            __builtin_amdgcn_sched_barrier(0);
            for (int s2 = 2 * grp; s2 < TV; s2 += 8) {
                read_ops(s2 + 4, a1_, b1_);
                mfmas(a0, b0);
                interleave();
                __builtin_amdgcn_sched_barrier(0);
                read_ops(s2 + 8, a0, b0);
                mfmas(a1_, b1_);
                interleave();
                __builtin_amdgcn_sched_barrier(0);
            }
        }
        if (db) {
            if (next < tg.ntiles) store_tile(par ^ 1);
            __syncthreads();
            par ^= 1;
            Ab = reinterpret_cast<const char *>(As + par * IMG);
            Bb = reinterpret_cast<const char *>(Bs + par * IMG);
        }
        tile = next;
    }
    if (SH == 1 && dob && i < kvalid) pbias[((size_t)(split * 2 + grp) * 2 + h) * K + k0 + i] = bsum;
#pragma unroll
    for (int j = 0; j < TPW; j++) {
        const int t = wave + 4 * j;
        if (t < g.ntaps) {
            float *po = partial + ((size_t)(split * 2 + grp) * g.ntaps + t) * C * K;
#pragma unroll
            for (int r = 0; r < 16; r++) {
                const int row = (r & 3) + 8 * (r >> 2) + 4 * h;
                if (row < cvalid && i < kvalid) po[(size_t)(c0 + row) * K + k0 + i] = acc[j][r];
            }
        }
    }
}

template <int NA, int NB, int NQ>
__global__ __launch_bounds__(256, 1) void k_wgrad_wino(const WgradGeom g, const WgTile tg, const float *__restrict__ a1,
                                                       const float *__restrict__ a2, const float *__restrict__ b,
                                                       float *__restrict__ partial) {
    extern __shared__ __attribute__((aligned(16))) float lds[];
    float *As = lds;
    float *Bs = lds + (size_t)NA * 1024;
    const int tid = threadIdx.x, lane = tid & 63;
    const int wave = __builtin_amdgcn_readfirstlane(tid >> 6);
    const int i = lane & 31, h = lane >> 5;
    const int cb = blockIdx.y / tg.nkb, kb = blockIdx.y % tg.nkb;
    const int split = blockIdx.x;
    const int C = g.C1 + g.C2, K = g.K;

    const int ja = wave == 0 ? 0 : (wave == 2 ? 2 : 1);
    const int jb = wave == 0 ? 2 : (wave == 1 ? 2 : (wave == 2 ? 1 : 3));
    const float sg = wave == 1 ? 1.f : -1.f;
    const float ea = wave == 3 ? 0.f : 1.f;
    const float eb = wave == 0 ? 0.f : (wave == 1 ? 1.f : -1.f);
// ... 557 lines not shown

__global__ __launch_bounds__(256) void k_wgrad_reduce_wino(const float *__restrict__ partial, float *__restrict__ dw,
                                                           int C, int K, int nsplit) {
    __shared__ double red[4][64];
    const long per = (long)36 * C * K;
    const long nout = (long)9 * C * K;
    const int e = threadIdx.x & 63, p = threadIdx.x >> 6;
    const long j = (long)blockIdx.x * 64 + e;
    double s0 = 0, s1 = 0;
    if (j < nout) {
        const long gi = j / ((long)C * K), ck = j - gi * (long)C * K;
        const float *src = partial + ((size_t)gi * 4 + p) * C * K + ck;
        int bsp = 0;
        for (; bsp + 1 < nsplit; bsp += 2) {
            s0 += (double)src[(size_t)bsp * per];
            s1 += (double)src[(size_t)(bsp + 1) * per];
        }
        if (bsp < nsplit) s0 += (double)src[(size_t)bsp * per];
    }
    red[p][e] = s0 + s1;
    __syncthreads();
    if (p != 0 || j >= nout) return;
    const double m0 = red[0][e], m1 = red[1][e], m2 = red[2][e], m3 = red[3][e];
    const long gi = j / ((long)C * K), ck = j - gi * (long)C * K;
    const int c = (int)(ck / K), k = (int)(ck - (long)c * K);
    float *o = dw + ((size_t)k * C + c) * 27 + gi * 3;
    o[0] = (float)(m0 + 0.5 * (m1 + m2));
    o[1] = (float)(0.5 * (m1 - m2));
    o[2] = (float)(0.5 * (m1 + m2) + m3);
}

template <int NAS, int NB>
__global__ __launch_bounds__(256, 2) void k_wgrad_smallc(const WgradGeom g, const WgTile tg, const float *__restrict__ a1,
                                                         const float *__restrict__ b, float *__restrict__ partial) {
    extern __shared__ __attribute__((aligned(16))) float lds[];
    float *As = lds;
    float *Bs = lds + (size_t)NAS * 1024;
    int *toffs = reinterpret_cast<int *>(Bs + (size_t)NB * 1024);
    const int tid = threadIdx.x, lane = tid & 63;
    const int wave = __builtin_amdgcn_readfirstlane(tid >> 6);
    const int i = lane & 31, h = lane >> 5;
    const int kb = blockIdx.y, split = blockIdx.x;
    const int C = g.C1, K = g.K;
    const int PARTS = C / 4;
#pragma unroll
    for (int t = 0; t < 27; t++)
        if (tid == t && t < g.ntaps) toffs[t] = tg.toffA[t];
    __syncthreads();
    const int row = wave * 32 + i;
    const bool rvalid = row < g.ntaps * C;
    const int rtap = rvalid ? row / C : 0, rc = rvalid ? row % C : 0;
    const int arow = (toffs[rtap] * C + rc) * 4 + h * g.sa[2] * C * 4;
    const int k0 = kb * 32;
    const int kvalid = (K - k0) < 32 ? (K - k0) : 32;
    const int EAhw = tg.EAh * tg.EAw, EBhw = tg.EBh * tg.EBw;
    const int TV = tg.TD * tg.TH * tg.TW;
    const int na = tg.nslotsA * PARTS, nb = tg.nslotsB * 8;
    const int tb0 = tg.toffB[0] * 128 + i * 4 + h * g.sb[2] * 128;
    f32x16 acc;
#pragma unroll
    for (int r = 0; r < 16; r++) acc[r] = 0.f;
    float4 ra[NAS], rb[NB];
    auto load_tile = [&](int tile) {
        unsigned r_ = (unsigned)tile;
        const int tw_ = (int)(r_ % (unsigned)tg.ntw); r_ /= (unsigned)tg.ntw;
        const int th_ = (int)(r_ % (unsigned)tg.nth); r_ /= (unsigned)tg.nth;
        const int td_ = (int)(r_ % (unsigned)tg.ntd);
        const int n = (int)(r_ / (unsigned)tg.ntd);
        const int od0 = td_ * tg.TD, oh0 = th_ * tg.TH, ow0 = tw_ * tg.TW;
        {
            const int z0 = od0 * g.sa[0] + tg.minA[0], y0 = oh0 * g.sa[1] + tg.minA[1], x0 = ow0 * g.sa[2] + tg.minA[2];
#pragma unroll
            for (int u = 0; u < NAS; u++) {
                const int idx = u * 256 + tid;
                const int slot = idx / PARTS, part = idx - slot * PARTS;
                const int ez = (slot * tg.magAhw) >> 16, rem = slot - ez * EAhw;
                const int ey = (rem * tg.magAw) >> 16, ex = rem - ey * tg.EAw;
                const int id = z0 + ez, ih = y0 + ey, iw = x0 + ex;
                ra[u] = make_float4(0.f, 0.f, 0.f, 0.f);
                if (idx < na && id >= 0 && id < g.Di && ih >= 0 && ih < g.Hi && iw >= 0 && iw < g.Wi)
                    ra[u] = *reinterpret_cast<const float4 *>(
                        a1 + ((((size_t)n * g.Di + id) * g.Hi + ih) * g.Wi + iw) * C + part * 4);
            }
        }
        {
            const int z0 = od0 * g.sb[0] + tg.minB[0], y0 = oh0 * g.sb[1] + tg.minB[1], x0 = ow0 * g.sb[2] + tg.minB[2];
            const int part = tid & 7;
#pragma unroll
            for (int u = 0; u < NB; u++) {
                const int idx = u * 256 + tid;
                const int slot = idx >> 3;
                const int ez = (slot * tg.magBhw) >> 16, rem = slot - ez * EBhw;
                const int ey = (rem * tg.magBw) >> 16, ex = rem - ey * tg.EBw;
                const int id = z0 + ez, ih = y0 + ey, iw = x0 + ex;
                rb[u] = make_float4(0.f, 0.f, 0.f, 0.f);
                if (part * 4 < kvalid && idx < nb && id >= 0 && id < g.Db && ih >= 0 && ih < g.Hb && iw >= 0 && iw < g.Wb)
                    rb[u] = *reinterpret_cast<const float4 *>(
                        b + ((((size_t)n * g.Db + id) * g.Hb + ih) * g.Wb + iw) * K + k0 + part * 4);
            }
        }
    };
    const char *Ab = reinterpret_cast<const char *>(As), *Bb = reinterpret_cast<const char *>(Bs);
    auto read_ops = [&](int s2, float &av, float &bv) {
        const int v = s2 < TV ? s2 : TV - 2;
        const int wx = v & (tg.TW - 1), hy = (v >> tg.lTW) & (tg.TH - 1), dz = v >> (tg.lTW + tg.lTH);
        const int sa_ = ((dz * g.sa[0]) * tg.EAh + hy * g.sa[1]) * tg.EAw + wx * g.sa[2];
        const int sb_ = ((dz * g.sb[0]) * tg.EBh + hy * g.sb[1]) * tg.EBw + wx * g.sb[2];
        av = *reinterpret_cast<const float *>(Ab + sa_ * C * 4 + arow);
        bv = *reinterpret_cast<const float *>(Bb + sb_ * 128 + tb0);
    };
    int tile = split;
    if (tile < tg.ntiles) load_tile(tile);
    while (tile < tg.ntiles) {
        __syncthreads();
#pragma unroll
        for (int u = 0; u < NAS; u++) *reinterpret_cast<float4 *>(As + (size_t)(u * 256 + tid) * 4) = ra[u];
#pragma unroll
        for (int u = 0; u < NB; u++) *reinterpret_cast<float4 *>(Bs + (size_t)(u * 256 + tid) * 4) = rb[u];
        __syncthreads();
        const int next = tile + tg.nsplit;
        if (next < tg.ntiles) load_tile(next);
        float a0, b0, a1_, b1_;
        read_ops(0, a0, b0);
        for (int s2 = 0; s2 < TV; s2 += 4) {
            read_ops(s2 + 2, a1_, b1_);
            __builtin_amdgcn_sched_barrier(0);
            acc = __builtin_amdgcn_mfma_f32_32x32x2f32(a0, b0, acc, 0, 0, 0);
            __builtin_amdgcn_sched_barrier(0);
            read_ops(s2 + 4, a0, b0);
            __builtin_amdgcn_sched_barrier(0);
            acc = __builtin_amdgcn_mfma_f32_32x32x2f32(a1_, b1_, acc, 0, 0, 0);
            __builtin_amdgcn_sched_barrier(0);
        }
        tile = next;
    }
#pragma unroll
    for (int r = 0; r < 16; r++) {
        const int rr = wave * 32 + (r & 3) + 8 * (r >> 2) + 4 * h;
        if (rr < g.ntaps * C && i < kvalid) {
            const int t = rr / C, c = rr - t * C;
            partial[(((size_t)split * g.ntaps + t) * C + c) * K + k0 + i] = acc[r];
        }
    }
}

typedef short s16x4 __attribute__((ext_vector_type(4)));
typedef short s16x8 __attribute__((ext_vector_type(8)));
typedef __bf16 bf16x8w __attribute__((ext_vector_type(8)));

__device__ inline bf16x8w tr_operand(const unsigned char *p0, const unsigned char *p1) {
    typedef __attribute__((address_space(3))) s16x4 lds_s16x4;
    const s16x4 lo = __builtin_amdgcn_ds_read_tr16_b64_v4i16((lds_s16x4 *)p0);
    const s16x4 hi = __builtin_amdgcn_ds_read_tr16_b64_v4i16((lds_s16x4 *)p1);
    return __builtin_bit_cast(bf16x8w, __builtin_shufflevector(lo, hi, 0, 1, 2, 3, 4, 5, 6, 7));
}

template <int TPW, int NA, int NB, int SH, bool TRI = false>
__global__ __launch_bounds__(256, 2) void k_wgrad16(const WgradGeom g, const WgTile tg,
                                                    const unsigned short *__restrict__ a1,
                                                    const unsigned short *__restrict__ a2,
                                                    const unsigned short *__restrict__ b, float *__restrict__ partial,
                                                    float *__restrict__ pbias) {
    extern __shared__ __attribute__((aligned(16))) unsigned char lds8[];
    unsigned char *As = lds8;
    unsigned char *Bs = lds8 + (size_t)NA * 4096;
    const int tid = threadIdx.x, lane = tid & 63;
    const int wave = __builtin_amdgcn_readfirstlane(tid >> 6);
    const int i = lane & 31, h = lane >> 5;
    const int cb = blockIdx.y / tg.nkb, kb = blockIdx.y % tg.nkb;
    const int split = blockIdx.x;
    const int C = g.C1 + g.C2, K = g.K;

    static_assert(!TRI || (TPW == 7 && SH == 1), "TRI: 27 taps over 4 waves x 7 slots, one dy fragment for all taps");
    auto tap_of = [&](int j) { return TRI ? (j < 6 ? 6 * wave + j : 24 + wave) : wave + 4 * j; };
    int ta[TPW], tb[TPW];
// ... 339 lines not shown
    }
    red[q][e] = (s0 + s1) + (s2 + s3);
    __syncthreads();
    if (q != 0 || j >= per) return;
    const double s = combine();
    const int k = (int)(j % K);
    const int c = (int)((j / K) % C);
    const int t = g.wt[(int)(j / ((long)K * C))];
    size_t o = g.transposed_out ? ((size_t)c * K + k) * g.T + t : ((size_t)k * C + c) * g.T + t;
    dw[o] = (float)s;
}

static void launch_wgrad_reduce_f(unsigned blocks, hipStream_t s, const WgradGeom &g, const float *partial, float *dw, int nsplit,
                                  const float *pbias, float *dbias, int nrows, int wblocks) {
    static const int g16 = getenv("MVD_WGRAD_REDUCE_G16") ? atoi(getenv("MVD_WGRAD_REDUCE_G16")) : 1;
    if (g16 && nsplit >= 64)
        hipLaunchKernelGGL(k_wgrad_reduce_f<16>, dim3(blocks), dim3(1024), 0, s, g, partial, dw, nsplit, pbias, dbias, nrows, wblocks);
    else
        hipLaunchKernelGGL(k_wgrad_reduce_f<4>, dim3(blocks), dim3(256), 0, s, g, partial, dw, nsplit, pbias, dbias, nrows, wblocks);
}

static int wgrad_max_split(const WgradGeom &g, int per_cu = 2) {
    const int C = g.C1 + g.C2;
    const int ncb = (C + 31) / 32, nkb = (g.K + 31) / 32;
    long ns = 256L * per_cu / ((long)ncb * nkb);
    if (ns < 1) ns = 1;
    const long per = (long)g.ntaps * C * g.K * 4;
    long cap = (256L << 20) / per;
    if (cap < 1) cap = 1;
    if (ns > cap) ns = cap;
    return (int)ns;
}

static bool wgrad_mfma_ok(const WgradGeom &g) {
    const int C = g.C1 + g.C2;
    if (g.ntaps < 1 || g.ntaps > 27) return false;
    if (g.C1 % 4 != 0 || g.C2 % 4 != 0 || g.K % 4 != 0) return false;
    if (g.C2 > 0 && g.C1 % 32 != 0) return false;
    if (C < 4 || g.K < 4) return false;
    return true;
}

size_t wgrad_mfma_ws(const WgradGeom &g) {
    if (!wgrad_mfma_ok(g)) return 0;
    size_t ws = (size_t)wgrad_max_split(g) * (g.ntaps * (size_t)(g.C1 + g.C2) + 2) * g.K * sizeof(float) + 256;
    const int C = g.C1 + g.C2;
    if (g.ntaps == 27 && C % 32 == 0 && g.K % 32 == 0) {
        const size_t w3 = wgrad_wino3_ws(wgrad_max_split(g, 1), C, g.K) + 256;
        if (w3 > ws) ws = w3;
    }
    return ws;
}

int wgrad16z_run(const WgradGeom &g, const unsigned short *a1, const unsigned short *a2, const unsigned short *b, float *dw, void *ws,
                 size_t ws_bytes, hipStream_t s, float *dbias, int *dbias_done, const float *in_scale, const float *in_shift,
                 float slope) {
    int nsplit_z = 0;
    float *pbias_z = nullptr;
    const int C = g.C1 + g.C2;
    const int rz = wgrad16z(g, a1, a2, b, ws, ws_bytes, dbias && dbias_done, &nsplit_z, &pbias_z, s, in_scale, in_shift, slope);
    if (rz != 0) return rz;
    float *partial_z = reinterpret_cast<float *>(ws);
    const int wblocks = (int)cdiv((long)27 * C * g.K, 64);
    if (pbias_z) {
        launch_wgrad_reduce_f((unsigned)(wblocks + cdiv(g.K, 64)), s, g, partial_z, dw, nsplit_z, pbias_z, dbias,
                           nsplit_z, wblocks);
        *dbias_done = 1;
    } else {
        launch_wgrad_reduce_f((unsigned)(wblocks), s, g, partial_z, dw, nsplit_z, (const float *)nullptr,
                           (float *)nullptr, 0, 0);
    }
    return check_launch("conv wgrad reduce (bf16 z-marching)");
}

int wgrad_mfma(const WgradGeom &g, const float *a1, const float *a2, const float *b, float *dw, void *ws, size_t ws_bytes,
               hipStream_t s, bool bf16_in, float *dbias, int *dbias_done) {
    if (dbias_done) *dbias_done = 0;
    if (!wgrad_mfma_ok(g)) return -1;
// ... 88 lines not shown
    tg.ntw = (g.Wo + tg.TW - 1) / tg.TW;
    const long ntiles = (long)g.N * tg.ntd * tg.nth * tg.ntw;
    if (ntiles > (1L << 30)) return -1;
    tg.ntiles = (int)ntiles;
    const int ncb = (C + 31) / 32;
    tg.nkb = (g.K + 31) / 32;
    long ns = wgrad_max_split(g, bf16_in ? 2 : 1);
    if (ns > ntiles) ns = ntiles;
    tg.nsplit = (int)ns;
    const size_t need_ws = (size_t)tg.nsplit * g.ntaps * C * g.K * sizeof(float);
    if (ws_bytes < need_ws) {
        set_error("conv wgrad (mfma): workspace too small (%zu < %zu)", ws_bytes, need_ws);
        return 1;
    }
    if ((long)ncb * tg.nkb > 65535) return -1;
    float *partial = reinterpret_cast<float *>(ws);
    const int tpw = (g.ntaps + 3) / 4;
    dim3 grid(tg.nsplit, ncb * tg.nkb);
    static const int db_mfma = getenv("MVD_WGRAD_DB") ? atoi(getenv("MVD_WGRAD_DB")) : 1;
    if (!bf16_in) tg.dbg = (tg.dbg & ~16) | (db_mfma ? 0 : 16);
#define WG_LAUNCH(TPW, NA, NB, SH)                                                                                   \
    {                                                                                                              \
        auto kern = k_wgrad_mfma<TPW, NA, NB, SH>;                                                                 \
        const size_t lds = (size_t)(NA + NB) * 8192 * (db_mfma ? 2 : 1);                                           \
        static PerDeviceFlag cfgd;                                                                                  \
        if (!cfgd()) {                                                                                               \
            if (hipFuncSetAttribute(reinterpret_cast<const void *>(kern), hipFuncAttributeMaxDynamicSharedMemorySize, \
                                    (int)LDS_LIMIT) != hipSuccess) {                                               \
                set_error("conv wgrad (mfma): cannot raise the dynamic LDS limit");                                \
                return 1;                                                                                          \
            }                                                                                                      \
            cfgd() = true;                                                                                           \
        }                                                                                                          \
        hipLaunchKernelGGL(kern, grid, dim3(512), lds, s, g, tg, a1, a2, b, partial, (SH) == 1 ? pbias_g : nullptr); \
    }
    bool sameA = true, sameB = true;
    for (int t = 1; t < g.ntaps; t++) {
        sameA = sameA && tg.toffA[t] == tg.toffA[0];
        sameB = sameB && tg.toffB[t] == tg.toffB[0];
    }
    if (bf16_in) {
        const unsigned short *h1 = reinterpret_cast<const unsigned short *>(a1);
        const unsigned short *h2 = reinterpret_cast<const unsigned short *>(a2);
        const unsigned short *hb = reinterpret_cast<const unsigned short *>(b);
        float *pbias16 = nullptr;
        if (dbias && dbias_done && (cfg == 0 || cfg == 2) && sameB && tpw == 7 && g.ntaps < 28 &&
            need_ws + (size_t)tg.nsplit * g.K * sizeof(float) <= ws_bytes)
            pbias16 = partial + need_ws / sizeof(float);
        static int tri_env = -1;
        if (tri_env < 0) tri_env = getenv("MVD_WGRAD16_TRI") ? atoi(getenv("MVD_WGRAD16_TRI")) : 1;
        bool tri = tri_env != 0 && sameB && tpw == 7 && g.ntaps == 27 && tg.TW == 8 && g.sa[2] == 1 &&
                   tg.TD * tg.TH * tg.TW == (cfg == 2 ? 256 : 128);
        for (int t = 0; t < 27 && tri; t++) tri = tg.toffA[t] == tg.toffA[t - t % 3] + t % 3;
#define WG16T(TPW, NA, NB, SH, TRI)                                                                                          \
    hipLaunchKernelGGL((k_wgrad16<TPW, NA, NB, SH, TRI>), grid, dim3(256),                                                  \
                       (size_t)(NA + NB) * 4096 + (size_t)(tg.TD * tg.TH * tg.TW) * 64 + ((TRI) ? 64 : 0), s, g, tg, h1, h2, \
                       hb, partial,                                                                                          \
                       (TPW) == 7 && (SH) == 1 ? pbias16 : nullptr)
#define WG16(TPW, NA, NB, SH) WG16T(TPW, NA, NB, SH, false)
#define WG16_TPW(NA, NB, SH)                  \
    {                                         \
        if (tpw <= 1) WG16(1, NA, NB, SH);    \
        else if (tpw == 2) WG16(2, NA, NB, SH); \
        else if (tpw <= 4) WG16(4, NA, NB, SH); \
        else WG16(7, NA, NB, SH);             \
    }
        if (cfg == 2) {
// ... 80 lines not shown
                    hipLaunchKernelGGL(k_dbias_reduce, dim3(cdiv(g.K, 64)), dim3(1024), 0, s, pbias, dbias, g.K, tg.nsplit * 2);
                    if (check_launch("conv wgrad dbias reduce")) return 1;
                    *dbias_done = 1;
                }
                hipLaunchKernelGGL(k_wgrad_reduce_wino2, dim3(cdiv((long)3 * C * g.K, 64)), dim3(1024), 0, s, partial, dw, C,
                                   g.K, tg.nsplit);
                return check_launch("conv wgrad reduce (winograd 2-D)");
            }
            auto kern = tg.TW == 8 ? k_wgrad_wino<13, 4, 4> : k_wgrad_wino<13, 4, 2>;
            static PerDeviceFlag cfgd_w[2];
            if (!cfgd_w[tg.TW == 8]()) {
                if (hipFuncSetAttribute(reinterpret_cast<const void *>(kern), hipFuncAttributeMaxDynamicSharedMemorySize,
                                        (int)LDS_LIMIT) != hipSuccess) {
                    set_error("conv wgrad (winograd): cannot raise the dynamic LDS limit");
                    return 1;
                }
                cfgd_w[tg.TW == 8]() = true;
            }
            hipLaunchKernelGGL(kern, grid, dim3(256), (size_t)(13 + 4) * 4096, s, g, tg, a1, a2, b, partial);
            if (check_launch("conv wgrad (winograd)")) return 1;
            hipLaunchKernelGGL(k_wgrad_reduce_wino, dim3(cdiv((long)9 * C * g.K, 64)), dim3(256), 0, s, partial, dw, C, g.K,
                               tg.nsplit);
            return check_launch("conv wgrad reduce (winograd)");
        }
    }
    if (cfg == 0 && sameB && g.C2 == 0 && C <= 8 && C % 4 == 0 && g.ntaps * C <= 128 && tg.nslotsA * (C / 4) <= 2 * 256) {
        long ns2 = 512 / tg.nkb;
        if (ns2 < 1) ns2 = 1;
        if (ns2 > tg.nsplit * 2) ns2 = tg.nsplit * 2;
        if (ns2 > ntiles) ns2 = ntiles;
        if ((size_t)ns2 * g.ntaps * C * g.K * sizeof(float) <= ws_bytes) tg.nsplit = (int)ns2;
        auto kern = k_wgrad_smallc<2, 4>;
        const size_t lds2 = (size_t)(2 + 4) * 4096 + 32 * 4;
        hipLaunchKernelGGL(kern, dim3(tg.nsplit, tg.nkb), dim3(256), lds2, s, g, tg, a1, b, partial);
        if (check_launch("conv wgrad (mfma, narrow input)")) return 1;
        const long per2 = (long)g.ntaps * C * g.K;
        launch_wgrad_reduce_f((unsigned)(cdiv(per2, 64)), s, g, partial, dw, tg.nsplit, (const float *)nullptr,
                           (float *)nullptr, 0, 0);
        return check_launch("conv wgrad reduce (mfma)");
    }
#define WG_TPW(NA, NB, SH)                     \
    {                                          \
        if (tpw <= 1) WG_LAUNCH(1, NA, NB, SH) \
        else if (tpw == 2) WG_LAUNCH(2, NA, NB, SH) \
        else if (tpw <= 4) WG_LAUNCH(4, NA, NB, SH) \
        else WG_LAUNCH(7, NA, NB, SH)          \
    }
    if ((size_t)2 * tg.nsplit * g.ntaps * C * g.K * sizeof(float) > ws_bytes) {
        set_error("conv wgrad (mfma): workspace too small for two partials per split");
        return 1;
    }
    const size_t need_g = (size_t)2 * tg.nsplit * g.ntaps * C * g.K * sizeof(float);
    float *pbias_g = nullptr;
    if (dbias && dbias_done && cfg == 0 && sameB && need_g + (size_t)4 * tg.nsplit * g.K * sizeof(float) <= ws_bytes)
        pbias_g = partial + need_g / sizeof(float);
    if (cfg == 0) {
        if (sameB) WG_TPW(7, 2, 1)
        else WG_TPW(7, 2, 0)
    } else {
        if (sameA) WG_TPW(1, 8, 2)
        else WG_TPW(1, 8, 0)
    }
#undef WG_TPW
#undef WG_LAUNCH
    if (check_launch("conv wgrad (mfma)")) return 1;
    const long per = (long)g.ntaps * C * g.K;
    const int wblocks = (int)cdiv(per, 64);
    if (pbias_g) {
        launch_wgrad_reduce_f((unsigned)(wblocks + cdiv(g.K, 64)), s, g, partial, dw, 2 * tg.nsplit,
                           (const float *)pbias_g, dbias, tg.nsplit * 4, wblocks);
        *dbias_done = 1;
    } else {
        launch_wgrad_reduce_f((unsigned)(wblocks), s, g, partial, dw, 2 * tg.nsplit, (const float *)nullptr,
                           (float *)nullptr, 0, 0);
    }
    return check_launch("conv wgrad reduce (mfma)");
}

}
```

multimodal_mvd_seg_amd/csrc/instnorm.hip:

```cpp
#include "common.h"

namespace mvd {

struct NormGeom {
    int C, CG, R, threads, nblk;
    long V, chunk;
};

static NormGeom norm_geom(int N, long V, int C) {
    NormGeom g;
    g.C = C;
    g.V = V;
    int vec = (C % 4 == 0) ? 4 : 1;
    g.CG = C / vec;
    if (g.CG > 256) {
        g.CG = C;
    }
    g.R = 256 / g.CG;
    if (g.R < 1) g.R = 1;
    g.threads = ((g.R * g.CG + 63) / 64) * 64;
    if (g.threads > 1024) g.threads = 1024;
    long want = 2048 / (N > 0 ? N : 1);
    if (want < 1) want = 1;
    long rows_min = (long)g.R * 16;
// ... 202 lines not shown
        be[i] = beta[c];
    }
    const size_t base = ((size_t)n * V) * C + (size_t)g * 4;
    long v = v0 + r;
    for (; v + 3L * R < v1; v += 4L * R) {
        float4 q[4];
#pragma unroll
        for (int u = 0; u < 4; u++) q[u] = ld4<XB>(x, base + (size_t)(v + (long)u * R) * C);
#pragma unroll
        for (int u = 0; u < 4; u++) {
            float f[4] = {q[u].x, q[u].y, q[u].z, q[u].w};
#pragma unroll
            for (int i = 0; i < 4; i++) {
                const float xh = (f[i] - mu[i]) * rs[i];
                const float z = fmaf(xh, ga[i], be[i]);
                f[i] = z > 0.f ? z : z * slope;
            }
            st4<YB>(y, base + (size_t)(v + (long)u * R) * C, f[0], f[1], f[2], f[3]);
        }
    }
    for (; v < v1; v += R) {
        float4 q = ld4<XB>(x, base + (size_t)v * C);
        float f[4] = {q.x, q.y, q.z, q.w};
#pragma unroll
        for (int i = 0; i < 4; i++) {
            const float xh = (f[i] - mu[i]) * rs[i];
            const float z = fmaf(xh, ga[i], be[i]);
            f[i] = z > 0.f ? z : z * slope;
        }
        st4<YB>(y, base + (size_t)v * C, f[0], f[1], f[2], f[3]);
    }
}

#ifndef MVD_IN_NRB
#define MVD_IN_NRB 4
#endif
constexpr int NRB = MVD_IN_NRB;
template <bool XB, bool YB>
__global__ void k_in_bwd_apply_rows(const float *__restrict__ x, const float *__restrict__ dy,
                                    const float *__restrict__ gamma, const float *__restrict__ beta,
                                    const float *__restrict__ mean, const float *__restrict__ rstd,
                                    const float *__restrict__ sums, float *__restrict__ dx, int C, int CG, int R, long V,
                                    long chunk, float slope) {
    const int n = blockIdx.y, t = threadIdx.x;
    const int g = t % CG, r = t / CG;
    if (r >= R) return;
    const long v0 = (long)blockIdx.x * chunk;
    long v1 = v0 + chunk;
    if (v1 > V) v1 = V;
    const float invV = 1.0f / (float)V;
    float mu[4], rs[4], ga[4], be[4], m1[4], m2[4];
#pragma unroll
    for (int i = 0; i < 4; i++) {
        const int c = g * 4 + i;
        const size_t nc = (size_t)n * C + c;
        mu[i] = mean[nc];
        rs[i] = rstd[nc];
        ga[i] = gamma[c];
        be[i] = beta[c];
        m1[i] = sums[nc * 2 + 0] * invV;
        m2[i] = sums[nc * 2 + 1] * invV;
    }
    const size_t base = ((size_t)n * V) * C + (size_t)g * 4;
    long v = v0 + r;
    for (; v + (NRB - 1L) * R < v1; v += (long)NRB * R) {
        float4 q[NRB], e[NRB];
#pragma unroll
        for (int u = 0; u < NRB; u++) {
            q[u] = ld4<XB>(x, base + (size_t)(v + (long)u * R) * C);
            e[u] = ld4<YB>(dy, base + (size_t)(v + (long)u * R) * C);
        }
#pragma unroll
        for (int u = 0; u < NRB; u++) {
            float f[4] = {q[u].x, q[u].y, q[u].z, q[u].w}, d[4] = {e[u].x, e[u].y, e[u].z, e[u].w};
#pragma unroll
            for (int i = 0; i < 4; i++) {
                const float xh = (f[i] - mu[i]) * rs[i];
                const float z = fmaf(xh, ga[i], be[i]);
                const float dz = z > 0.f ? d[i] : d[i] * slope;
                f[i] = ga[i] * rs[i] * (dz - m1[i] - xh * m2[i]);
            }
            st4<XB>(dx, base + (size_t)(v + (long)u * R) * C, f[0], f[1], f[2], f[3]);
        }
    }
    for (; v < v1; v += R) {
        float4 q = ld4<XB>(x, base + (size_t)v * C);
        float4 e = ld4<YB>(dy, base + (size_t)v * C);
        float f[4] = {q.x, q.y, q.z, q.w}, d[4] = {e.x, e.y, e.z, e.w};
#pragma unroll
        for (int i = 0; i < 4; i++) {
            const float xh = (f[i] - mu[i]) * rs[i];
            const float z = fmaf(xh, ga[i], be[i]);
            const float dz = z > 0.f ? d[i] : d[i] * slope;
            f[i] = ga[i] * rs[i] * (dz - m1[i] - xh * m2[i]);
        }
        st4<XB>(dx, base + (size_t)v * C, f[0], f[1], f[2], f[3]);
    }
}

template <int VEC, bool XB, bool YB>
__global__ void k_in_bwd_stats(const float *__restrict__ x, const float *__restrict__ dy,
                               const float *__restrict__ gamma, const float *__restrict__ beta,
                               const float *__restrict__ mean, const float *__restrict__ rstd,
                               double *__restrict__ partial, int C, int CG, int R, long V, long chunk, float slope) {
    extern __shared__ double sm[];
    const int n = blockIdx.y, b = blockIdx.x, nblk = gridDim.x;
    const int t = threadIdx.x;
    const int g = t % CG, r = t / CG;
    const long v0 = (long)b * chunk;
    long v1 = v0 + chunk;
    if (v1 > V) v1 = V;
    double s[VEC], ss[VEC];
    float mu[VEC], rs[VEC], ga[VEC], be[VEC];
#pragma unroll
    for (int i = 0; i < VEC; i++) s[i] = ss[i] = 0.0;
    if (r < R) {
#pragma unroll
        for (int i = 0; i < VEC; i++) {
            int c = g * VEC + i;
            mu[i] = mean[(size_t)n * C + c];
            rs[i] = rstd[(size_t)n * C + c];
            ga[i] = gamma[c];
            be[i] = beta[c];
        }
        const size_t base = ((size_t)n * V) * C + (size_t)g * VEC;
        long v = v0 + r;
        if (VEC == 4) {
            for (; v + R < v1; v += 2L * R) {
                const float4 q0 = ld4<XB>(x, base + (size_t)v * C), e0 = ld4<YB>(dy, base + (size_t)v * C);
                const float4 q1 = ld4<XB>(x, base + (size_t)(v + R) * C), e1 = ld4<YB>(dy, base + (size_t)(v + R) * C);
                const float fx[2][4] = {{q0.x, q0.y, q0.z, q0.w}, {q1.x, q1.y, q1.z, q1.w}};
                const float dd[2][4] = {{e0.x, e0.y, e0.z, e0.w}, {e1.x, e1.y, e1.z, e1.w}};
#pragma unroll
                for (int u = 0; u < 2; u++)
#pragma unroll
                    for (int i = 0; i < 4; i++) {
                        const float xh = (fx[u][i] - mu[i]) * rs[i];
                        const float z = fmaf(xh, ga[i], be[i]);
                        const float dz = z > 0.f ? dd[u][i] : dd[u][i] * slope;
                        s[i] += (double)dz;
                        ss[i] += (double)dz * (double)xh;
                    }
            }
        }
        for (; v < v1; v += R) {
            float f[VEC], d[VEC];
            if (VEC == 4) {
                float4 q = ld4<XB>(x, base + (size_t)v * C);
                float4 e = ld4<YB>(dy, base + (size_t)v * C);
                f[0] = q.x; f[1] = q.y; f[2] = q.z; f[3] = q.w;
                d[0] = e.x; d[1] = e.y; d[2] = e.z; d[3] = e.w;
            } else {
                f[0] = x[base + (size_t)v * C];
                d[0] = dy[base + (size_t)v * C];
            }
#pragma unroll
            for (int i = 0; i < VEC; i++) {
                float xh = (f[i] - mu[i]) * rs[i];
                float z = fmaf(xh, ga[i], be[i]);
                float dz = z > 0.f ? d[i] : d[i] * slope;
                s[i] += (double)dz;
                ss[i] += (double)dz * (double)xh;
            }
        }
#pragma unroll
        for (int i = 0; i < VEC; i++) {
            sm[((size_t)r * C + g * VEC + i) * 2 + 0] = s[i];
            sm[((size_t)r * C + g * VEC + i) * 2 + 1] = ss[i];
        }
    }
    __syncthreads();
    for (int c = t; c < C; c += blockDim.x) {
        double a = 0, q = 0;
        for (int rr = 0; rr < R; rr++) {
            a += sm[((size_t)rr * C + c) * 2 + 0];
            q += sm[((size_t)rr * C + c) * 2 + 1];
        }
        size_t o = (((size_t)n * nblk + b) * C + c) * 2;
        partial[o] = a;
        partial[o + 1] = q;
    }
}
// ... 120 lines not shown
    const int n = blockIdx.y;
    const long per_n = V * C / VEC;
    const size_t off = (size_t)n * V * C;
    const float invV = 1.0f / (float)V;
    for (long i = (long)blockIdx.x * blockDim.x + threadIdx.x; i < per_n; i += (long)gridDim.x * blockDim.x) {
        int c = (int)((i * VEC) % C);
        float f[VEC], d[VEC];
        if (VEC == 4) {
            float4 q = reinterpret_cast<const float4 *>(x + off)[i];
            float4 e = reinterpret_cast<const float4 *>(dy + off)[i];
            f[0] = q.x; f[1] = q.y; f[2] = q.z; f[3] = q.w;
            d[0] = e.x; d[1] = e.y; d[2] = e.z; d[3] = e.w;
        } else {
            f[0] = x[off + i];
            d[0] = dy[off + i];
        }
#pragma unroll
        for (int k = 0; k < VEC; k++) {
            size_t nc = (size_t)n * C + c + k;
            float rs = rstd[nc];
            float xh = (f[k] - mean[nc]) * rs;
            float z = fmaf(xh, gamma[c + k], beta[c + k]);
            float dz = z > 0.f ? d[k] : d[k] * slope;
            float m1 = sums[nc * 2 + 0] * invV, m2 = sums[nc * 2 + 1] * invV;
            f[k] = gamma[c + k] * rs * (dz - m1 - xh * m2);
        }
        if (VEC == 4)
            reinterpret_cast<float4 *>(dx + off)[i] = make_float4(f[0], f[1], f[2], f[3]);
        else
            dx[off + i] = f[0];
    }
}

}

using namespace mvd;

extern "C" {

int mvd_instnorm_nblk(int N, long V, int C) { return norm_geom(N, V, C).nblk; }

size_t mvd_instnorm_workspace_bytes(int N, long V, int C) {
    NormGeom g = norm_geom(N, V, C);
    return (size_t)N * g.nblk * C * 2 * sizeof(double) + (size_t)N * C * 2 * sizeof(float) + 256;
}

static int in_fwd(const float *x, bool xb, const float *gamma, const float *beta, float *y, bool yb, float *mean,
                  float *rstd, int N, long V, int C, float eps, float slope, void *ws, size_t ws_bytes, void *stream,
                  const float *tile_stats = nullptr, long ntiles = 0) {
    MVD_REQUIRE(x && gamma && beta && y && mean && rstd && ws, "instnorm_fwd: null pointer");
    MVD_REQUIRE(N > 0 && N <= 65535 && V > 0 && C > 0 && C <= 1024, "instnorm_fwd: bad shape N=%d V=%ld C=%d", N, V, C);
    MVD_REQUIRE(ws_bytes >= mvd_instnorm_workspace_bytes(N, V, C), "instnorm_fwd: workspace too small");
    NormGeom g = norm_geom(N, V, C);
    hipStream_t s = as_stream(stream);
    double *partial = reinterpret_cast<double *>(ws);
    size_t sm = (size_t)g.R * C * 2 * sizeof(double);
    MVD_REQUIRE(sm <= 64 * 1024, "instnorm_fwd: C too large for the LDS reduce");
    const bool v4 = (C % 4 == 0) && (g.CG * 4 == C);
    MVD_REQUIRE(v4 || !(xb || yb), "instnorm_fwd: bf16 I/O needs C %% 4 == 0");
    dim3 grid(g.nblk, N);
    if (tile_stats) {
        long nb2 = (ntiles + 63) / 64;
        if (nb2 > g.nblk) nb2 = g.nblk;
        if (nb2 > 64) nb2 = 64;
        const long chunk2 = (ntiles + nb2 - 1) / nb2;
        nb2 = (ntiles + chunk2 - 1) / chunk2;
        const int CW = C < 256 ? C : 256, R2 = 256 / CW;
        hipLaunchKernelGGL(k_in_tiles_reduce, dim3((unsigned)nb2, N), dim3(256), (size_t)R2 * CW * 2 * sizeof(double), s,
                           tile_stats, partial, C, CW, R2, ntiles, chunk2);
        if (check_launch("instnorm statistics from conv tiles")) return 1;
        hipLaunchKernelGGL(k_in_finalize, dim3(C, N), dim3(64), 0, s, partial, mean, rstd, C, (int)nb2, V, eps);
        if (check_launch("instnorm finalize")) return 1;
    } else {
        if (v4 && xb)
            hipLaunchKernelGGL((k_in_stats<4, true>), grid, dim3(g.threads), sm, s, x, partial, C, g.CG, g.R, V, g.chunk);
        else if (v4)
            hipLaunchKernelGGL((k_in_stats<4, false>), grid, dim3(g.threads), sm, s, x, partial, C, g.CG, g.R, V, g.chunk);
        else
            hipLaunchKernelGGL((k_in_stats<1, false>), grid, dim3(g.threads), sm, s, x, partial, C, g.CG, g.R, V, g.chunk);
        if (check_launch("instnorm stats")) return 1;
        float *ss = reinterpret_cast<float *>(partial + (size_t)N * g.nblk * C * 2);
        const bool ssf = v4 && xb && yb;
        hipLaunchKernelGGL(k_in_finalize, dim3(C, N), dim3(64), 0, s, partial, mean, rstd, C, g.nblk, V, eps,
                           ssf ? gamma : nullptr, ssf ? beta : nullptr, ssf ? ss : nullptr, ssf ? ss + (size_t)N * C : nullptr);
        if (check_launch("instnorm finalize")) return 1;
        if (ssf) {
            long nb2 = V / ((long)g.R * 8);
            if (nb2 < 1) nb2 = 1;
            long cap2 = 8192 / N > 0 ? 8192 / N : 1;
            if (nb2 > cap2) nb2 = cap2;
            const long chunk2 = cdiv(V, nb2);
            hipLaunchKernelGGL(k_in_apply_ss16, dim3((unsigned)cdiv(V, chunk2), N), dim3(g.threads), 0, s,
                               reinterpret_cast<const unsigned short *>(x), ss, ss + (size_t)N * C,
                               reinterpret_cast<unsigned short *>(y), C, g.CG, g.R, V, chunk2, slope);
            return check_launch("instnorm apply (scale / shift form)");
        }
    }
    long per_n = V * C / (v4 ? 4 : 1);
    long bx = cdiv(per_n, 256);
    long cap = 4096 / N > 0 ? 4096 / N : 1;
    if (bx > cap) bx = cap;
    if (v4) {
        long nb2 = V / ((long)g.R * 8);
        if (nb2 < 1) nb2 = 1;
        long cap2 = 8192 / N > 0 ? 8192 / N : 1;
        if (nb2 > cap2) nb2 = cap2;
        const long chunk2 = cdiv(V, nb2);
        auto kern = xb ? (yb ? k_in_apply_rows<true, true> : k_in_apply_rows<true, false>)
                       : (yb ? k_in_apply_rows<false, true> : k_in_apply_rows<false, false>);
        hipLaunchKernelGGL(kern, dim3((unsigned)cdiv(V, chunk2), N), dim3(g.threads), 0, s, x, gamma, beta, mean, rstd, y, C,
                           g.CG, g.R, V, chunk2, slope);
    }
    else
        hipLaunchKernelGGL(k_in_apply<1>, dim3(bx, N), dim3(256), 0, s, x, gamma, beta, mean, rstd, y, C, V, slope);
    return check_launch("instnorm apply");
}

static int in_bwd(const float *x, bool xb, const float *dy, bool yb, const float *gamma, const float *beta,
                  const float *mean, const float *rstd, float *dx, float *dgamma, float *dbeta, int N, long V, int C,
                  float slope, void *ws, size_t ws_bytes, void *stream) {
    MVD_REQUIRE(x && dy && gamma && beta && mean && rstd && dx && dgamma && dbeta && ws, "instnorm_bwd: null pointer");
    MVD_REQUIRE(N > 0 && N <= 65535 && V > 0 && C > 0 && C <= 1024, "instnorm_bwd: bad shape");
    MVD_REQUIRE(ws_bytes >= mvd_instnorm_workspace_bytes(N, V, C), "instnorm_bwd: workspace too small");
    NormGeom g = norm_geom(N, V, C);
    hipStream_t s = as_stream(stream);
    double *partial = reinterpret_cast<double *>(ws);
    float *sums = reinterpret_cast<float *>(partial + (size_t)N * g.nblk * C * 2);
    size_t sm = (size_t)g.R * C * 2 * sizeof(double);
    MVD_REQUIRE(sm <= 64 * 1024, "instnorm_bwd: C too large for the LDS reduce");
    const bool v4 = (C % 4 == 0) && (g.CG * 4 == C);
    dim3 grid(g.nblk, N);
    MVD_REQUIRE(v4 || !(xb || yb), "instnorm_bwd: bf16 I/O needs C %% 4 == 0");
    if (v4) {
        auto kern = xb ? (yb ? k_in_bwd_stats<4, true, true> : k_in_bwd_stats<4, true, false>)
                       : (yb ? k_in_bwd_stats<4, false, true> : k_in_bwd_stats<4, false, false>);
        hipLaunchKernelGGL(kern, grid, dim3(g.threads), sm, s, x, dy, gamma, beta, mean, rstd, partial, C, g.CG, g.R, V,
                           g.chunk, slope);
    } else
        hipLaunchKernelGGL((k_in_bwd_stats<1, false, false>), grid, dim3(g.threads), sm, s, x, dy, gamma, beta, mean, rstd,
                           partial, C, g.CG, g.R, V, g.chunk, slope);
    if (check_launch("instnorm bwd stats")) return 1;
    hipLaunchKernelGGL(k_in_bwd_finalize, dim3(C), dim3(64), 0, s, partial, sums, dgamma, dbeta, N, C,
                       g.nblk);
    if (check_launch("instnorm bwd finalize")) return 1;
    long per_n = V * C / (v4 ? 4 : 1);
    long bx = cdiv(per_n, 256);
    long cap = 4096 / N > 0 ? 4096 / N : 1;
    if (bx > cap) bx = cap;
    if (v4) {
        long nb2 = V / ((long)g.R * 8);
        if (nb2 < 1) nb2 = 1;
        long cap2 = 8192 / N > 0 ? 8192 / N : 1;
        if (nb2 > cap2) nb2 = cap2;
        const long chunk2 = cdiv(V, nb2);
        auto kern = xb ? (yb ? k_in_bwd_apply_rows<true, true> : k_in_bwd_apply_rows<true, false>)
                       : (yb ? k_in_bwd_apply_rows<false, true> : k_in_bwd_apply_rows<false, false>);
        hipLaunchKernelGGL(kern, dim3((unsigned)cdiv(V, chunk2), N), dim3(g.threads), 0, s, x, dy, gamma, beta, mean, rstd,
                           sums, dx, C, g.CG, g.R, V, chunk2, slope);
    }
    else
        hipLaunchKernelGGL(k_in_bwd_apply<1>, dim3(bx, N), dim3(256), 0, s, x, dy, gamma, beta, mean, rstd, sums, dx, C,
                           V, slope);
    return check_launch("instnorm bwd apply");
}

int mvd_instnorm_lrelu_fwd(const float *x, const float *gamma, const float *beta, float *y, float *mean, float *rstd,
                           int N, long V, int C, float eps, float slope, void *ws, size_t ws_bytes, void *stream) {
    return in_fwd(x, false, gamma, beta, y, false, mean, rstd, N, V, C, eps, slope, ws, ws_bytes, stream);
}

int mvd_instnorm_lrelu_bwd(const float *x, const float *dy, const float *gamma, const float *beta, const float *mean,
                           const float *rstd, float *dx, float *dgamma, float *dbeta, int N, long V, int C,
                           float slope, void *ws, size_t ws_bytes, void *stream) {
    return in_bwd(x, false, dy, false, gamma, beta, mean, rstd, dx, dgamma, dbeta, N, V, C, slope, ws, ws_bytes, stream);
}

int mvd_instnorm_lrelu_fwd_prestats(const float *x, const float *tile_stats, long ntiles, const float *gamma,
                                    const float *beta, float *y, float *mean, float *rstd, int N, long V, int C, float eps,
                                    float slope, void *ws, size_t ws_bytes, void *stream) {
    MVD_REQUIRE(tile_stats && ntiles > 0, "instnorm_fwd_prestats: tile statistics required");
    return in_fwd(x, false, gamma, beta, y, false, mean, rstd, N, V, C, eps, slope, ws, ws_bytes, stream, tile_stats, ntiles);
}

int mvd_instnorm_finalize_tiles(const float *tile_stats, long ntiles, const float *gamma, const float *beta, float *mean,
                                float *rstd, float *scale, float *shift, int N, long V, int C, float eps, void *stream) {
    MVD_REQUIRE(tile_stats && gamma && beta && mean && rstd && scale && shift, "instnorm_finalize_tiles: null pointer");
    MVD_REQUIRE(ntiles > 0 && N > 0 && N <= 65535 && V > 0 && C > 0 && C <= 65535, "instnorm_finalize_tiles: bad shape");
    hipLaunchKernelGGL(k_in_finalize_tiles, dim3(C, N), dim3(64), 0, as_stream(stream), tile_stats, gamma, beta, mean, rstd,
                       scale, shift, C, ntiles, V, eps);
    return check_launch("instnorm finalize (conv tile statistics)");
}

__global__ void k_in_scale_shift(const float *__restrict__ gamma, const float *__restrict__ beta, const float *__restrict__ mean,
                                 const float *__restrict__ rstd, float *__restrict__ scale, float *__restrict__ shift, int N,
                                 int C) {
    const int i = blockIdx.x * blockDim.x + threadIdx.x;
    if (i >= N * C) return;
    const float sc = gamma[i % C] * rstd[i];
    scale[i] = sc;
    shift[i] = fmaf(-mean[i], sc, beta[i % C]);
}

int mvd_instnorm_stats_bf16(const void *x, int x_is_bf16, const float *gamma, const float *beta, float *mean, float *rstd,
                            float *scale, float *shift, int N, long V, int C, float eps, void *ws, size_t ws_bytes,
                            void *stream) {
    MVD_REQUIRE(x && gamma && beta && mean && rstd && scale && shift && ws, "instnorm_stats: null pointer");
    MVD_REQUIRE(N > 0 && N <= 65535 && V > 0 && C > 0 && C % 4 == 0 && C <= 1024, "instnorm_stats: bad shape (C %% 4 == 0)");
// ... 69 lines not shown
```

multimodal_mvd_seg_amd/ops.py:

```python
import ctypes
import os
import typing
import weakref

import numpy as np
import torch
from torch.autograd import Function
from torch.autograd.function import once_differentiable

from . import _lib
from ._lib import call, i3, query

CL3D = torch.channels_last_3d


def _stream():
    return ctypes.c_void_p(torch.cuda.current_stream().cuda_stream)


def _p(t):
    return ctypes.c_void_p(t.data_ptr()) if t is not None else None


def _require_cuda(*ts):
# ... 393 lines not shown
    if t.requires_grad:
        t._mvd_gshare = _GradShare()
    return t


def _share_of(t):
    return getattr(t, "_mvd_gshare", None)


def _publish(share, dx):
    if share is not None:
        share.buf = dx
    return dx


def _joinable(share, shape, dtype):
    b = share.buf if share is not None else None
    return b if (b is not None and tuple(b.shape) == tuple(shape) and b.dtype == dtype and _is_cl3d(b)) else None


class LaunchTimer:

    def __init__(self, key):
        self.key, self.pairs, self.on = tuple(key), [], False

    def mean_ms(self):
        return sum(a.elapsed_time(b) for a, b in self.pairs) / len(self.pairs) if self.pairs else None


LAUNCH_TIMER = None


BF16_CONV_STATS = [os.environ.get("MVD_BF16_CONV_STATS", "1") != "0"]


def conv3d_fwd_bf16(x1, C1, x2, C2, wf, bias, y, N, D, H, W, K, ks, stride, ws, in_scale=None, in_shift=None, slope=0.01):
    nt = query("mvd_conv3d_fwd_bf16_stats_tiles", N, D, H, W, C1, C2, K, i3(ks), i3(stride)) \
        if (BF16_CONV_STATS[0] or in_scale is not None) else 0
    if nt <= 0 and in_scale is None:
        call("mvd_conv3d_fwd_bf16", _p(x1), C1, _p(x2), C2, _p(wf), _p(bias), _p(y), N, D, H, W, K, i3(ks), i3(stride),
             _p(ws), ws.numel(), _stream())
        return
    stats = torch.empty((N, nt, K, 2), dtype=torch.float32, device=y.device) if (nt > 0 and BF16_CONV_STATS[0]) else None
    got = ctypes.c_int(0)
    call("mvd_conv3d_fwd_bf16_fused", _p(x1), C1, _p(x2), C2, _p(wf), _p(bias), _p(y), N, D, H, W, K, i3(ks), i3(stride),
         _p(in_scale), _p(in_shift), float(slope), _p(stats), ctypes.byref(got), _p(ws), ws.numel(), _stream())
    if stats is not None and got.value > 0:
        y._mvd_tile_stats16 = (stats, int(got.value))


class Conv3dFn(Function):

    @staticmethod
    def forward(ctx, x1, x2, weight, bias, stride):
        _require_cuda(x1, x2, weight, bias)
        ctx.share1, ctx.share2 = _share_of(x1), (_share_of(x2) if x2 is not None else None)
        x1 = to_ndhwc(x1)
        x2 = to_ndhwc(x2) if x2 is not None else None
        K, C = weight.shape[:2]
        ks = tuple(weight.shape[2:])
        N, C1, D, H, W = x1.shape
        C2 = x2.shape[1] if x2 is not None else 0
        if C1 + C2 != C:
            raise RuntimeError(f"conv3d: weight expects {C} input channels, got {C1}+{C2}")
        if x2 is not None and tuple(x2.shape[2:]) != (D, H, W):
            raise RuntimeError("conv3d: the two concatenated inputs differ in spatial size")
# ... 1 lines not shown
        if x2 is not None and _is_bf16(x2) != bf:
            raise RuntimeError("conv3d: the two concatenated inputs differ in dtype")
        od = [_out_dim(i, k, s) for i, k, s in zip((D, H, W), ks, stride)]
        y = empty_cl3d((N, K, *od), x1.device, x1.dtype)
        ws = _Workspace.get(query("mvd_conv_fwd_workspace_bytes", N, od[0] * od[1] * od[2], K), x1.device)
        ub = None
        tm = LAUNCH_TIMER
        timed = tm is not None and tm.on and tm.key == (bf, N, C1, C2, K, D, H, W, tuple(ks), tuple(stride))
        if timed:
            ev0 = torch.cuda.Event(enable_timing=True)
            ev0.record()
        if bf:
            wf, wb = _packed_bf16(weight, False)
            conv3d_fwd_bf16(x1, C1, x2, C2, wf, bias, y, N, D, H, W, K, ks, stride, ws)
        else:
            wino = query("mvd_conv_wino_applicable", N, D, H, W, C1, C2, K, i3(ks), i3(stride)) if len(ks) == 3 else 0
            wino3 = query("mvd_conv_wino3_applicable", N, D, H, W, C1, C2, K, i3(ks), i3(stride)) if wino else 0
            wino2 = wino & ~wino3
            pk = _packed(weight, False, bool(wino2 & 1), bool(wino2 & 2), bool(wino3 & 1), bool(wino3 & 2))
            wf, wb = pk.wf, pk.wb
            uf = pk.vf if wino3 & 1 else (pk.uf if wino2 & 1 else None)
            ub = pk.vb if wino3 & 2 else (pk.ub if wino2 & 2 else None)
            sfx3 = "3" if wino3 & 1 else ""
            ctx.ub3 = bool(wino3 & 2)
            if uf is not None:
                ntiles = query("mvd_conv_stats_tiles", od[0], od[1], od[2])
                stats = torch.empty((N, ntiles, K, 2), dtype=torch.float32, device=x1.device)
                done = ctypes.c_int(0)
                call("mvd_conv3d_fwd_wino" + sfx3 + "_stats", _p(x1), C1, _p(x2), C2, _p(wf), _p(uf), _p(bias), _p(y),
                     _p(stats), ctypes.byref(done), N, D, H, W, K, i3(ks), i3(stride), _p(ws), ws.numel(), _stream())
                if done.value:
                    y._mvd_tile_stats = (stats, ntiles)
            else:
                call("mvd_conv3d_fwd_wino", _p(x1), C1, _p(x2), C2, _p(wf), _p(uf), _p(bias), _p(y), N, D, H, W, K, i3(ks),
                     i3(stride), _p(ws), ws.numel(), _stream())
        if timed:
            ev1 = torch.cuda.Event(enable_timing=True)
            ev1.record()
            tm.pairs.append((ev0, ev1))
        ctx.bf = bf
        ctx.params = (weight, bias)
        ctx.pack = None if bf else (pk, pk.gen)
        ctx.pack16_gen = _pack16_guard(weight) if bf else None
        ctx.save_for_backward(x1, x2, wb, ub)
        ctx.geom = (N, C1, C2, D, H, W, K, ks, tuple(stride), tuple(od), bias is not None)
        return y

    @staticmethod
    @once_differentiable
    def backward(ctx, dy):
        x1, x2, wb, ub = ctx.saved_tensors
        _check_pack_generation(ctx.pack, "conv3d backward")
        _check_pack16_generation(ctx.pack16_gen, "conv3d backward")
        N, C1, C2, D, H, W, K, ks, stride, od, has_bias = ctx.geom
        dy = to_ndhwc(dy)
        dev = dy.device
        sfx = "_bf16" if ctx.bf else ""
        dx1 = dx2 = dw = db = None
        need1, need2 = ctx.needs_input_grad[0], (x2 is not None and ctx.needs_input_grad[1])
        joined = None
        if need1 and x2 is None and len(ks) == 3:
            joined = _joinable(ctx.share1, (N, C1, D, H, W), dy.dtype)
            if joined is not None and not query("mvd_conv3d_dgrad_acc_ok", int(ctx.bf), N, D, H, W, C1, K, i3(ks), i3(stride)):
                joined = None
        if joined is not None:
            if ctx.bf:
                ws = _Workspace.get(query("mvd_conv_fwd_workspace_bytes", N, D * H * W, C1), dev)
                call("mvd_conv3d_dgrad_bf16_acc", _p(dy), _p(wb), _p(joined), C1, N, D, H, W, K, i3(ks), i3(stride), _p(ws),
# ... 375 lines not shown
        N, C = x.shape[:2]
        K = weight.shape[0]
        V = x[0, 0].numel()
        w = weight.detach().reshape(K, C).contiguous()
        logits = torch.empty((N, K, *x.shape[2:]), dtype=torch.float32, device=x.device)
        call("mvd_seghead_fwd_bf16" if _is_bf16(x) else "mvd_seghead_fwd", _p(x), _p(w), _p(bias), _p(logits), N, V, C, K,
             _stream())
        ctx.save_for_backward(x, w)
        ctx.wshape = tuple(weight.shape)
        return logits

    @staticmethod
    @once_differentiable
    def backward(ctx, dl):
        x, w = ctx.saved_tensors
        N, C = x.shape[:2]
        K = w.shape[0]
        V = x[0, 0].numel()
        dl = dl.contiguous()
        dev = x.device
        joined = _joinable(ctx.share, x.shape, x.dtype) if ctx.needs_input_grad[0] else None
        dx = joined if joined is not None else (empty_cl3d(x.shape, dev, x.dtype) if ctx.needs_input_grad[0] else None)
        dw = torch.empty((K, C), dtype=torch.float32, device=dev)
        db = torch.empty((K,), dtype=torch.float32, device=dev)
        nb = query("mvd_seghead_bwd_workspace_bytes", N, V, C, K)
        ws = _Workspace.get(nb, dev)
        call("mvd_seghead_bwd_bf16" if _is_bf16(x) else "mvd_seghead_bwd", _p(x), _p(w), _p(dl), _p(dx), _p(dw), _p(db), N, V, C, K,
             1 if joined is not None else 0, _p(ws), ws.numel(), _stream())
        if ctx.share is not None:
            ctx.share.buf = None if joined is not None else dx
        return (None if joined is not None else dx), dw.view(ctx.wshape), db


class NormActSegHeadFn(Function):

    @staticmethod
    def forward(ctx, y0, gamma, beta, eps, slope, weight, bias):
        _require_cuda(y0, gamma, beta, weight, bias)
        bf = _is_bf16(y0)
        if not _is_cl3d(y0) or y0.dtype not in (BF16, torch.float32):
            raise RuntimeError("NormActSegHeadFn: needs the raw NDHWC conv output (bf16 or fp32)")
        N, C, D, H, W = y0.shape
        K = weight.shape[0]
        V = D * H * W
        dev = y0.device
        g, b = gamma.detach().contiguous(), beta.detach().contiguous()
        mean = torch.empty((N, C), dtype=torch.float32, device=dev)
        rstd, scale, shift = torch.empty_like(mean), torch.empty_like(mean), torch.empty_like(mean)
        ws = _Workspace.get(query("mvd_instnorm_workspace_bytes", N, V, C), dev)
        pre16 = getattr(y0, '_mvd_tile_stats16', None) if bf else None
        pre = getattr(y0, '_mvd_tile_stats', None) if not bf else None
        if pre16 is not None and pre16[0].shape[0] == N and pre16[0].shape[2] == C:
            call("mvd_instnorm_finalize_tiles", _p(pre16[0]), pre16[1], _p(g), _p(b), _p(mean), _p(rstd), _p(scale), _p(shift), N,
                 V, C, float(eps), _stream())
        elif pre is not None and pre[0].shape[0] == N and pre[0].shape[2] == C:
            call("mvd_instnorm_stats_from_tiles", _p(pre[0]), pre[1], _p(mean), _p(rstd), N, V, C, float(eps), _p(ws), ws.numel(),
                 _stream())
        else:
            call("mvd_instnorm_stats_bf16", _p(y0), int(bf), _p(g), _p(b), _p(mean), _p(rstd), _p(scale), _p(shift), N, V, C,
                 float(eps), _p(ws), ws.numel(), _stream())
        w = weight.detach().reshape(K, C).contiguous()
        logits = torch.empty((N, K, D, H, W), dtype=torch.float32, device=dev)
        if bf:
            call("mvd_seghead_fwd_bf16_fused", _p(y0), _p(scale), _p(shift), float(slope), _p(w), _p(bias), _p(logits), N, V, C,
                 K, _stream())
        else:
            call("mvd_seghead_fwd_fused", _p(y0), _p(mean), _p(rstd), _p(g), _p(b), float(slope), _p(w), _p(bias), _p(logits), N,
                 V, C, K, _stream())
        ctx.save_for_backward(y0, g, b, mean, rstd, scale, shift, w)
        ctx.params = (gamma, beta)
        ctx.slope = float(slope)
        ctx.wshape = tuple(weight.shape)
        return logits

    @staticmethod
    @once_differentiable
    def backward(ctx, dl):
        y0, g, b, mean, rstd, scale, shift, w = ctx.saved_tensors
        gamma, beta = ctx.params
        bf = _is_bf16(y0)
        N, C, D, H, W = y0.shape
        K = w.shape[0]
        V = D * H * W
        dev = y0.device
        dl = dl.contiguous()
        need_x = ctx.needs_input_grad[0] or ctx.needs_input_grad[1] or ctx.needs_input_grad[2]
        da = empty_cl3d(y0.shape, dev, y0.dtype) if need_x else None
        dw = torch.empty((K, C), dtype=torch.float32, device=dev)
        db = torch.empty((K,), dtype=torch.float32, device=dev)
        ws = _Workspace.get(query("mvd_seghead_bwd_workspace_bytes", N, V, C, K), dev)
        if bf:
            call("mvd_seghead_bwd_bf16_fused", _p(y0), _p(scale), _p(shift), ctx.slope, _p(w), _p(dl), _p(da), _p(dw), _p(db), N,
                 V, C, K, 0, _p(ws), ws.numel(), _stream())
        else:
            call("mvd_seghead_bwd_fused", _p(y0), _p(mean), _p(rstd), _p(g), _p(b), ctx.slope, _p(w), _p(dl), _p(da), _p(dw),
                 _p(db), N, V, C, K, 0, _p(ws), ws.numel(), _stream())
        dy0 = dg = db_ = None
        if need_x:
            dy0 = empty_cl3d(y0.shape, dev, y0.dtype)
            sink_g, sink_b = _take_grad(gamma), _take_grad(beta)
            dg = sink_g if sink_g is not None else torch.empty((C,), dtype=torch.float32, device=dev)
            db_ = sink_b if sink_b is not None else torch.empty((C,), dtype=torch.float32, device=dev)
            ws = _Workspace.get(query("mvd_instnorm_workspace_bytes", N, V, C), dev)
            if bf:
                call("mvd_instnorm_lrelu_bwd_bf16", _p(y0), 1, _p(da), _p(g), _p(b), _p(mean), _p(rstd), _p(dy0), _p(dg),
                     _p(db_), N, V, C, ctx.slope, _p(ws), ws.numel(), _stream())
            else:
                call("mvd_instnorm_lrelu_bwd", _p(y0), _p(da), _p(g), _p(b), _p(mean), _p(rstd), _p(dy0), _p(dg), _p(db_), N, V,
                     C, ctx.slope, _p(ws), ws.numel(), _stream())
            if sink_g is not None:
                dg = None
                _grad_done(gamma)
            if sink_b is not None:
                db_ = None
                _grad_done(beta)
        return dy0, dg, db_, None, None, dw.view(ctx.wshape), db


def fused_norm_seghead_ok(y0, weight):
    if not (y0.dtype in (BF16, torch.float32) and y0.dim() == 5 and _is_cl3d(y0) and y0.is_cuda):
        return False
    N, C = y0.shape[:2]
    return weight.shape[1] == C and query("mvd_seghead_bf16_fused_ok", N, y0[0, 0].numel(), C, weight.shape[0]) > 0


class CastFn(Function):

    @staticmethod
    def forward(ctx, x):
        _require_cuda(x)
        if not _is_bf16(x):
            raise RuntimeError("CastFn widens bf16 tensors")
        x = to_ndhwc(x)
        y = torch.empty_like(x, dtype=torch.float32)
        call("mvd_cast_bf16_to_f32", _p(x), _p(y), x.numel(), _stream())
        return y

# ... 684 lines not shown
```

Before: 60.23 samples/s.

## Fuse instance-norm stats into direct MFMA conv and recompute seghead grads in norm bwd

The direct MFMA fp32 conv kernels now emit per-tile sum and sum-of-squares, so instance norm can skip its separate statistics pass. The seghead backward no longer writes the intermediate activation gradient; the norm backward recomputes it from the logit gradient and head weight. ConvT wgrad can fold the bias reduction into the wgrad kernel, and small instance norms get a single-launch path. These changes aim to cut full-tensor memory passes and kernel launches, at the cost of extra epilogue work in the conv kernels and more template variants.

```diff
diff --git a/include/mvdseg_hip.h b/include/mvdseg_hip.h
--- a/include/mvdseg_hip.h
+++ b/include/mvdseg_hip.h
@@ -54,6 +54,10 @@
 int mvd_conv3d_fwd_wino3_stats(const float *x1, int C1, const float *x2, int C2, const float *wf, const float *vf,
                                const float *bias, float *y, float *stats, int *stats_done, int N, int D, int H, int W,
                                int K, const int ksize[3], const int stride[3], void *ws, size_t ws_bytes, void *stream);
+long mvd_conv3d_fwd_stats_tiles(int N, int D, int H, int W, int C1, int C2, int K, const int ksize[3], const int stride[3]);
+int mvd_conv3d_fwd_stats(const float *x1, int C1, const float *x2, int C2, const float *wf, const float *bias, float *y,
+                         float *stats, long stats_tiles, int *stats_done, int N, int D, int H, int W, int K,
+                         const int ksize[3], const int stride[3], void *ws, size_t ws_bytes, void *stream);
 int mvd_conv3d_dgrad_wino3(const float *dy, const float *wb, const float *vb, float *dx1, int C1, float *dx2, int C2,
                            int N, int D, int H, int W, int K, const int ksize[3], const int stride[3], void *ws,
                            size_t ws_bytes, void *stream);
@@ -61,6 +65,7 @@
 int mvd_conv_wgrad_wino3_applicable(int N, int D, int H, int W, int C1, int C2, int K, const int ksize[3],
                                     const int stride[3]);
 long mvd_wgrad_wino3_launches(void);
+int mvd_set_wgrad_bias_fold(int on);
 size_t mvd_conv3d_wgrad_workspace_bytes(int C, int K, int T, int N, int Do, int Ho, int Wo);
 int mvd_conv3d_wgrad(const float *x1, int C1, const float *x2, int C2, const float *dy, float *dw, float *dbias,
                      int N, int D, int H, int W, int K, const int ksize[3], const int stride[3], void *ws,
@@ -157,6 +162,13 @@
 int mvd_instnorm_lrelu_bwd(const float *x, const float *dy, const float *gamma, const float *beta,
                            const float *mean, const float *rstd, float *dx, float *dgamma, float *dbeta, int N,
                            long V, int C, float slope, void *ws, size_t ws_bytes, void *stream);
+int mvd_instnorm_single_launch(long V, int C);
+long mvd_instnorm_stats_pass_launches(void);
+long mvd_instnorm_single_launches(void);
+int mvd_set_instnorm_small_max(long max_elems);
+int mvd_instnorm_lrelu_bwd_head(const float *x, const float *dlogits, const float *w, int K, const float *gamma,
+                                const float *beta, const float *mean, const float *rstd, float *dx, float *dgamma,
+                                float *dbeta, int N, long V, int C, float slope, void *ws, size_t ws_bytes, void *stream);
 
 int mvd_seghead_fwd(const float *x, const float *w, const float *bias, float *logits, int N, long V, int C, int K,
                     void *stream);
diff --git a/multimodal_mvd_seg_amd/_lib.py b/multimodal_mvd_seg_amd/_lib.py
--- a/multimodal_mvd_seg_amd/_lib.py
+++ b/multimodal_mvd_seg_amd/_lib.py
@@ -35,6 +35,9 @@
     "mvd_conv3d_fwd_wino": (c_int, [_P, c_int, _P, c_int, _P, _P, _P, _P, c_int, c_int, c_int, c_int, c_int, _I3, _I3, _P,
                                     c_size_t, _P]),
     "mvd_conv_stats_tiles": (c_size_t, [c_int, c_int, c_int]),
+    "mvd_conv3d_fwd_stats_tiles": (c_long, [c_int, c_int, c_int, c_int, c_int, c_int, c_int, _I3, _I3]),
+    "mvd_conv3d_fwd_stats": (c_int, [_P, c_int, _P, c_int, _P, _P, _P, _P, c_long, _P, c_int, c_int, c_int, c_int, c_int, _I3,
+                                     _I3, _P, c_size_t, _P]),
     "mvd_conv3d_fwd_wino_stats": (c_int, [_P, c_int, _P, c_int, _P, _P, _P, _P, _P, _P, c_int, c_int, c_int, c_int, c_int,
                                           _I3, _I3, _P, c_size_t, _P]),
     "mvd_conv3d_dgrad_wino": (c_int, [_P, _P, _P, _P, c_int, _P, c_int, c_int, c_int, c_int, c_int, c_int, _I3, _I3, _P,
@@ -53,6 +56,7 @@
     "mvd_set_wgrad_wino3_min_items": (c_int, [c_long]),
     "mvd_conv_wgrad_wino3_applicable": (c_int, [c_int, c_int, c_int, c_int, c_int, c_int, c_int, _I3, _I3]),
     "mvd_wgrad_wino3_launches": (c_long, []),
+    "mvd_set_wgrad_bias_fold": (c_int, [c_int]),
     "mvd_conv3d_wgrad_bf16": (c_int, [_P, c_int, _P, c_int, _P, _P, _P, c_int, c_int, c_int, c_int, c_int, _I3, _I3, _P,
                                       c_size_t, _P]),
     "mvd_convT3d_wgrad_bf16": (c_int, [_P, _P, _P, _P, c_int, c_int, c_int, c_int, c_int, c_int, _I3, _P, c_size_t,
@@ -104,6 +108,12 @@
     "mvd_instnorm_lrelu_fwd": (c_int, [_P, _P, _P, _P, _P, _P, c_int, c_long, c_int, c_float, c_float, _P, c_size_t, _P]),
     "mvd_instnorm_lrelu_bwd": (c_int, [_P, _P, _P, _P, _P, _P, _P, _P, _P, c_int, c_long, c_int, c_float, _P, c_size_t,
                                        _P]),
+    "mvd_instnorm_single_launch": (c_int, [c_long, c_int]),
+    "mvd_instnorm_single_launches": (c_long, []),
+    "mvd_instnorm_stats_pass_launches": (c_long, []),
+    "mvd_set_instnorm_small_max": (c_int, [c_long]),
+    "mvd_instnorm_lrelu_bwd_head": (c_int, [_P, _P, _P, c_int, _P, _P, _P, _P, _P, _P, _P, c_int, c_long, c_int, c_float, _P,
+                                            c_size_t, _P]),
     "mvd_seghead_fwd": (c_int, [_P, _P, _P, _P, c_int, c_long, c_int, c_int, _P]),
     "mvd_seghead_bwd_workspace_bytes": (c_size_t, [c_int, c_long, c_int, c_int]),
     "mvd_seghead_bwd": (c_int, [_P, _P, _P, _P, _P, _P, c_int, c_long, c_int, c_int, c_int, _P, c_size_t, _P]),
diff --git a/multimodal_mvd_seg_amd/csrc/conv.hip b/multimodal_mvd_seg_amd/csrc/conv.hip
--- a/multimodal_mvd_seg_amd/csrc/conv.hip
+++ b/multimodal_mvd_seg_amd/csrc/conv.hip
@@ -291,8 +291,16 @@
 
 static int run_fwd(const FwdGeom &g, const float *a1, const float *a2, const float *w, const float *bias, float *y1,
                    float *y2, void *ws, size_t ws_bytes, hipStream_t s, const float *u = nullptr, float *stats = nullptr,
-                   int *stats_done = nullptr, bool u3d = false) {
+                   int *stats_done = nullptr, bool u3d = false, long direct_tiles = 0) {
     if (stats_done) *stats_done = 0;
+    if (direct_tiles > 0) {
+        if (g_engine_mode == 0) {
+            int r = fwd_mfma(g, a1, a2, w, bias, y1, y2, ws, ws_bytes, s, stats, direct_tiles, stats_done);
+            if (r >= 0) return r;
+            if (stats_done) *stats_done = 0;
+        }
+        return fwd_scalar(g, a1, a2, w, bias, y1, y2, s);
+    }
     if (u3d) {
         if (g_engine_mode == 0 && u && !g_wino_off && wino3_enabled() &&
             wino3_items(g.Do, g.Ho, g.Wo, g.K1 + g.K2) >= g_wino3_min_items) {
@@ -378,13 +386,13 @@
 static int conv3d_fwd_impl(const float *x1, int C1, const float *x2, int C2, const float *wf, const float *uf,
                            const float *bias, float *y, int N, int D, int H, int W, int K, const int ksize[3],
                            const int stride[3], void *ws, size_t ws_bytes, void *stream, float *stats = nullptr,
-                           int *stats_done = nullptr, bool u3d = false) {
+                           int *stats_done = nullptr, bool u3d = false, long direct_tiles = 0) {
     MVD_REQUIRE(x1 && wf && y && C1 > 0 && C2 >= 0 && (C2 == 0 || x2), "conv3d_fwd: null pointer / bad channels");
     MVD_REQUIRE(N > 0 && D > 0 && H > 0 && W > 0 && K > 0, "conv3d_fwd: bad shape");
     if (check_ks(ksize, stride, "conv3d_fwd")) return 2;
     FwdGeom g;
     conv_fwd_geom(g, N, D, H, W, C1, C2, K, ksize, stride);
-    return run_fwd(g, x1, x2, wf, bias, y, nullptr, ws, ws_bytes, as_stream(stream), uf, stats, stats_done, u3d);
+    return run_fwd(g, x1, x2, wf, bias, y, nullptr, ws, ws_bytes, as_stream(stream), uf, stats, stats_done, u3d, direct_tiles);
 }
 
 int mvd_conv3d_fwd(const float *x1, int C1, const float *x2, int C2, const float *wf, const float *bias, float *y, int N,
@@ -420,6 +428,27 @@
     MVD_REQUIRE(stats_done, "conv3d_fwd_wino_stats: stats_done is required");
     return conv3d_fwd_impl(x1, C1, x2, C2, wf, uf, bias, y, N, D, H, W, K, ksize, stride, ws, ws_bytes, stream, stats,
                            stats_done);
+}
+
+long mvd_conv3d_fwd_stats_tiles(int N, int D, int H, int W, int C1, int C2, int K, const int ksize[3], const int stride[3]) {
+    if (N <= 0 || D <= 0 || H <= 0 || W <= 0 || C1 <= 0 || C2 < 0 || K <= 0 || !ksize || !stride || g_engine_mode != 0) return 0;
+    for (int a = 0; a < 3; a++)
+        if (!(ksize[a] == 1 || ksize[a] == 3) || !(stride[a] == 1 || stride[a] == 2)) return 0;
+    FwdGeom g;
+    conv_fwd_geom(g, N, D, H, W, C1, C2, K, ksize, stride);
+    long tiles = 0;
+    const float *al = reinterpret_cast<const float *>(uintptr_t(64));
+    if (fwd_mfma(g, al, C2 ? al : nullptr, al, nullptr, nullptr, nullptr, nullptr, 0, nullptr, nullptr, 0, nullptr, &tiles) != 0)
+        return 0;
+    return tiles;
+}
+
+int mvd_conv3d_fwd_stats(const float *x1, int C1, const float *x2, int C2, const float *wf, const float *bias, float *y,
+                         float *stats, long stats_tiles, int *stats_done, int N, int D, int H, int W, int K,
+                         const int ksize[3], const int stride[3], void *ws, size_t ws_bytes, void *stream) {
+    MVD_REQUIRE(stats && stats_done && stats_tiles > 0, "conv3d_fwd_stats: stats, stats_tiles and stats_done are required");
+    return conv3d_fwd_impl(x1, C1, x2, C2, wf, nullptr, bias, y, N, D, H, W, K, ksize, stride, ws, ws_bytes, stream, stats,
+                           stats_done, false, stats_tiles);
 }
 
 int mvd_pack_weights_batch(int n, const float *const *w, float *const *wf, float *const *wb, float *const *uf,
@@ -635,6 +664,11 @@
 
 long mvd_wgrad_wino3_launches(void) { return wgrad_wino3_launches(); }
 
+int mvd_set_wgrad_bias_fold(int on) {
+    set_wgrad_bias_fold(on);
+    return 0;
+}
+
 int mvd_conv3d_wgrad(const float *x1, int C1, const float *x2, int C2, const float *dy, float *dw, float *dbias, int N,
                      int D, int H, int W, int K, const int ksize[3], const int stride[3], void *ws, size_t ws_bytes,
                      void *stream) {
@@ -754,11 +788,11 @@
     convT_wgrad_geom(g, N, D, H, W, C, K, stride);
     MVD_REQUIRE(ws_bytes >= mvd_convT3d_wgrad_workspace_bytes(C, K, g.T, N, D, H, W), "convT3d_wgrad: workspace too small");
     hipStream_t s = as_stream(stream);
-    if (dbias) {
-        int r = colsum(dy, dbias, (long)N * g.Db * g.Hb * g.Wb, K, ws, s);
-        if (r) return r;
-    }
-    return run_wgrad(g, x, nullptr, dy, dw, ws, ws_bytes, s);
+    int dbias_done = 0;
+    int r = run_wgrad(g, x, nullptr, dy, dw, ws, ws_bytes, s, dbias, &dbias_done);
+    if (r) return r;
+    if (dbias && !dbias_done) return colsum(dy, dbias, (long)N * g.Db * g.Hb * g.Wb, K, ws, s);
+    return 0;
 }
 
 int mvd_pack_weight_bf16(const float *w, uint16_t *wf, uint16_t *wb, int K, int C, int T, int transposed, void *stream) {
diff --git a/multimodal_mvd_seg_amd/csrc/conv_geom.h b/multimodal_mvd_seg_amd/csrc/conv_geom.h
--- a/multimodal_mvd_seg_amd/csrc/conv_geom.h
+++ b/multimodal_mvd_seg_amd/csrc/conv_geom.h
@@ -45,7 +45,8 @@
                float *y2, hipStream_t s);
 size_t fwd_mfma_ws(int N, long out_vox, int K);
 int fwd_mfma(const FwdGeom &g, const float *a1, const float *a2, const float *w, const float *bias, float *y1, float *y2,
-             void *ws, size_t ws_bytes, hipStream_t s);
+             void *ws, size_t ws_bytes, hipStream_t s, float *stats = nullptr, long stats_tiles = 0, int *stats_done = nullptr,
+             long *plan = nullptr);
 size_t wgrad_scalar_ws(const WgradGeom &g);
 int wgrad_scalar(const WgradGeom &g, const float *a1, const float *a2, const float *b, float *dw, void *ws,
                  size_t ws_bytes, hipStream_t s);
@@ -86,6 +87,7 @@
 size_t wgrad_wino3_ws(int nsplit, int C, int K);
 int wgrad_wino3_enabled();
 void set_wgrad_wino3_min_items(long n);
+void set_wgrad_bias_fold(int on);
 long wgrad_wino3_launches();
 int dbias_reduce(const float *pbias, float *dbias, int K, int nrows, hipStream_t s);
 size_t wino_weight_elems(int C, int K);
diff --git a/multimodal_mvd_seg_amd/csrc/conv_mfma.hip b/multimodal_mvd_seg_amd/csrc/conv_mfma.hip
--- a/multimodal_mvd_seg_amd/csrc/conv_mfma.hip
+++ b/multimodal_mvd_seg_amd/csrc/conv_mfma.hip
@@ -61,7 +61,8 @@
 __global__ __launch_bounds__(256, 2) void k_fwd_mfma(const FwdGeom g, const FwdTile tg, const float *__restrict__ a1,
                                                      const float *__restrict__ a2, const float *__restrict__ w,
                                                      const float *__restrict__ bias, float *__restrict__ y1,
-                                                     float *__restrict__ y2, const int S, float *__restrict__ part) {
+                                                     float *__restrict__ y2, const int S, float *__restrict__ part,
+                                                     float *__restrict__ stats) {
     extern __shared__ __attribute__((aligned(16))) float lds[];
     constexpr int HH = CK / 2;
     constexpr int KT = 32 * NT;
@@ -206,6 +207,32 @@
     }
 
     const int od = od0 + wave;
+    if (stats) {
+        const size_t tl = ((size_t)(td_ * 4 + wave) * tg.nth + th_) * tg.ntw + tw_;
+        float *so = stats + (((size_t)n * tg.ntd * 4 * tg.nth * tg.ntw + tl) * tg.K) * 2;
+#pragma unroll
+        for (int q_ = 0; q_ < NT; q_++) {
+            const int k = kb * KT + q_ * 32 + i;
+            const float bv = settled(bias ? bias[k] : 0.f);
+            float sa = 0.f, sq = 0.f;
+            if (od < g.Do) {
+#pragma unroll
+                for (int m = 0; m < MT; m++)
+#pragma unroll
+                    for (int r = 0; r < 16; r++) {
+                        const int oh = oh0 + 4 * m + (r >> 2), ow = ow0 + 4 * h + (r & 3);
+                        if (oh < g.Ho && ow < g.Wo) {
+                            const float val = acc[m][q_][r] + bv;
+                            sa += val;
+                            sq += val * val;
+                        }
+                    }
+            }
+            sa += __shfl_xor(sa, 32);
+            sq += __shfl_xor(sq, 32);
+            if (h == 0) *reinterpret_cast<float2 *>(so + (size_t)k * 2) = make_float2(sa, sq);
+        }
+    }
     if (od >= g.Do) return;
 #pragma unroll
     for (int m = 0; m < MT; m++)
@@ -444,7 +471,7 @@
 __global__ __launch_bounds__(512, 1) void k_fwd32s(const FwdGeom g, const Fwd32Tile tg, const float *__restrict__ a1,
                                                    const float *__restrict__ a2, const float *__restrict__ w,
                                                    const float *__restrict__ bias, float *__restrict__ y1,
-                                                   float *__restrict__ y2) {
+                                                   float *__restrict__ y2, float *__restrict__ stats) {
     extern __shared__ __attribute__((aligned(16))) float Xs[];
     constexpr int XS = 36;
     const int tid = threadIdx.x, lane = tid & 63;
@@ -604,8 +631,28 @@
         for (int r = 0; r < 16; r++) acc[r] += xi[r * 64];
     }
     const int od = od0 + dl;
+    const float bv = settled(bias ? bias[kcol] : 0.f);
+    if (stats) {
+        const size_t tl = ((size_t)(td_ * 2 + dl) * tg.nth + th_) * tg.ntw + tw_;
+        float *so = stats + (((size_t)n * tg.ntd * 2 * tg.nth * tg.ntw + tl) * tg.K) * 2;
+        float sa = 0.f, sq = 0.f;
+        if (od < g.Do) {
+#pragma unroll
+            for (int r = 0; r < 16; r++) {
+                const int row = (r & 3) + 8 * (r >> 2) + 4 * h;
+                const int oh = oh0 + (row >> 3), ow = ow0 + (row & 7);
+                if (oh < g.Ho && ow < g.Wo) {
+                    const float val = acc[r] + bv;
+                    sa += val;
+                    sq += val * val;
+                }
+            }
+        }
+        sa += __shfl_xor(sa, 32);
+        sq += __shfl_xor(sq, 32);
+        if (h == 0) *reinterpret_cast<float2 *>(so + (size_t)kcol * 2) = make_float2(sa, sq);
+    }
     if (od >= g.Do) return;
-    const float bv = settled(bias ? bias[kcol] : 0.f);
 #pragma unroll
     for (int r = 0; r < 16; r++) {
         const int row = (r & 3) + 8 * (r >> 2) + 4 * h;
@@ -762,7 +809,7 @@
 
 static int num_cus();
 static int launch_fwd32s(const FwdGeom &g, const float *a1, const float *a2, const float *w, const float *bias, float *y1,
-                         float *y2, hipStream_t s) {
+                         float *y2, hipStream_t s, float *stats, long stats_tiles, int *stats_done, long *plan) {
     const int K = g.K1 + g.K2;
     Fwd32Tile tg;
     memset(&tg, 0, sizeof(tg));
@@ -795,6 +842,12 @@
     const long nitems = (long)g.N * tg.ntd * tg.nth * tg.ntw * tg.nkb;
     if (nitems > (1L << 30)) return -1;
     tg.nitems = (int)nitems;
+    const long my_tiles = (long)tg.ntd * 2 * tg.nth * tg.ntw;
+    if (plan) {
+        *plan = my_tiles;
+        return 0;
+    }
+    float *st = (stats && stats_done && stats_tiles == my_tiles) ? stats : nullptr;
     const size_t lds = (size_t)tg.nslots * 36 * sizeof(float);
     static PerDeviceFlag cfgd;
     if (!cfgd()) {
@@ -806,8 +859,10 @@
         cfgd() = true;
     }
     const unsigned grid = (unsigned)(((nitems + 7) / 8) * 8);
-    hipLaunchKernelGGL(k_fwd32s, dim3(grid), dim3(512), lds, s, g, tg, a1, a2, w, bias, y1, y2);
-    return check_launch("conv fwd (stride 2, CK=32)");
+    hipLaunchKernelGGL(k_fwd32s, dim3(grid), dim3(512), lds, s, g, tg, a1, a2, w, bias, y1, y2, st);
+    if (check_launch("conv fwd (stride 2, CK=32)")) return 1;
+    if (st) *stats_done = 1;
+    return 0;
 }
 
 static int num_cus() {
@@ -874,7 +929,14 @@
 
 template <int CK, int NT, int MT, bool L32>
 static int launch_fwd(const FwdGeom &g, FwdTile &tg, size_t lds, const float *a1, const float *a2, const float *w,
-                      const float *bias, float *y1, float *y2, void *ws, size_t ws_bytes, hipStream_t s) {
+                      const float *bias, float *y1, float *y2, void *ws, size_t ws_bytes, hipStream_t s, float *stats,
+                      long stats_tiles, int *stats_done, long *plan) {
+    const long my_tiles = (long)tg.ntd * 4 * tg.nth * tg.ntw;
+    if (plan) {
+        *plan = my_tiles;
+        return 0;
+    }
+    float *st = (stats && stats_done && stats_tiles == my_tiles) ? stats : nullptr;
     auto kern = k_fwd_mfma<CK, NT, MT, L32>;
     static size_t configured = 0;
     if (lds > configured) {
@@ -889,17 +951,24 @@
     const int nkb = K / (32 * NT);
     const long tiles = (long)tg.ntd * tg.nth * tg.ntw;
     const size_t out_elems = (size_t)g.N * g.Do * g.Ho * g.Wo * K;
-    const int S = split_for(ws, ws_bytes, tiles * nkb * g.N, (g.C1 + g.C2) / CK, out_elems, nkb);
+    const int S = st ? 1 : split_for(ws, ws_bytes, tiles * nkb * g.N, (g.C1 + g.C2) / CK, out_elems, nkb);
     dim3 grid((unsigned)tiles, nkb * S, g.N);
     float *part = reinterpret_cast<float *>(ws);
-    hipLaunchKernelGGL(kern, grid, dim3(256), lds, s, g, tg, a1, a2, w, bias, y1, y2, S, part);
+    hipLaunchKernelGGL(kern, grid, dim3(256), lds, s, g, tg, a1, a2, w, bias, y1, y2, S, part, st);
     if (check_launch("conv fwd (mfma)")) return 1;
     if (S > 1) return run_split_reduce(g, part, bias, y1, y2, S, out_elems, s);
+    if (st) *stats_done = 1;
     return 0;
 }
 
 int fwd_mfma(const FwdGeom &g, const float *a1, const float *a2, const float *w, const float *bias, float *y1, float *y2,
-             void *ws, size_t ws_bytes, hipStream_t s) {
+             void *ws, size_t ws_bytes, hipStream_t s, float *stats, long stats_tiles, int *stats_done, long *plan) {
+    if (plan) *plan = 0;
+    if (stats_done) *stats_done = 0;
+    if (g.K2 != 0 || g.so[0] != 1 || g.so[1] != 1 || g.so[2] != 1 || g.oo[0] || g.oo[1] || g.oo[2]) {
+        stats = nullptr;
+        if (plan) return 0;
+    }
     const int C = g.C1 + g.C2, K = g.K1 + g.K2;
     const int LCK = wl_ck(C);
     if (LCK == 0 || g.ntaps < 1 || g.ntaps > 27) return -1;
@@ -947,6 +1016,7 @@
             t32.nth = (g.Ho + 3) / 4;
             t32.ntw = (g.Wo + 7) / 8;
             t32.K = K;
+            if (plan) return 0;
             if (NT == 2) return launch_fwd32<2, 1>(g, t32, a1, a2, w, bias, y1, y2, ws, ws_bytes, s);
             return launch_fwd32<1, 2>(g, t32, a1, a2, w, bias, y1, y2, ws, ws_bytes, s);
         }
@@ -956,7 +1026,7 @@
         !(dbg & 8)) {
         const long items = (long)g.N * ((g.Do + 1) / 2) * ((g.Ho + 3) / 4) * ((g.Wo + 7) / 8) * (K / 64);
         if (items >= 256) {
-            int r = launch_fwd32s(g, a1, a2, w, bias, y1, y2, s);
+            int r = launch_fwd32s(g, a1, a2, w, bias, y1, y2, s, stats, stats_tiles, stats_done, plan);
             if (r >= 0) return r;
         }
     }
@@ -991,9 +1061,9 @@
         tg.ntw = (g.Wo + 7) / 8;
 #define MVD_FWD_DISPATCH(CKV, L32V)                                                                                      \
     {                                                                                                                    \
-        if (MT == 2 && NT == 2) return launch_fwd<CKV, 2, 2, L32V>(g, tg, lds, a1, a2, w, bias, y1, y2, ws, ws_bytes, s); \
-        if (MT == 2 && NT == 1) return launch_fwd<CKV, 1, 2, L32V>(g, tg, lds, a1, a2, w, bias, y1, y2, ws, ws_bytes, s); \
-        return launch_fwd<CKV, 1, 1, L32V>(g, tg, lds, a1, a2, w, bias, y1, y2, ws, ws_bytes, s);                         \
+        if (MT == 2 && NT == 2) return launch_fwd<CKV, 2, 2, L32V>(g, tg, lds, a1, a2, w, bias, y1, y2, ws, ws_bytes, s, stats, stats_tiles, stats_done, plan); \
+        if (MT == 2 && NT == 1) return launch_fwd<CKV, 1, 2, L32V>(g, tg, lds, a1, a2, w, bias, y1, y2, ws, ws_bytes, s, stats, stats_tiles, stats_done, plan); \
+        return launch_fwd<CKV, 1, 1, L32V>(g, tg, lds, a1, a2, w, bias, y1, y2, ws, ws_bytes, s, stats, stats_tiles, stats_done, plan); \
     }
         if (LCK == 32) MVD_FWD_DISPATCH(8, true)
         else if (CK == 8) MVD_FWD_DISPATCH(8, false)
@@ -1186,13 +1256,16 @@
 #pragma unroll
         for (int j = 0; j < NBV; j++) bv[j] = *reinterpret_cast<const float *>(Bb + sb_ + boff[j]);
     };
-    const bool dob = SH == 1 && pbias != nullptr && cb == 0 && wave == 0;
+    const bool dob = pbias != nullptr && cb == 0 && (SH == 1 ? wave == 0 : SH == 2);
     float bsum = 0.f;
     auto mfmas = [&](const float (&av)[NAV], const float (&bv)[NBV]) {
 #pragma unroll
         for (int j = 0; j < TPW; j++)
             acc[j] = __builtin_amdgcn_mfma_f32_32x32x2f32(av[SH == 2 ? 0 : j], bv[SH == 1 ? 0 : j], acc[j], 0, 0, 0);
         if (SH == 1 && dob) bsum += bv[0];
+        if (SH == 2 && dob)
+#pragma unroll
+            for (int j = 0; j < NBV; j++) bsum += bv[j];
     };
     auto interleave = [&]() {
 #pragma unroll
@@ -1243,6 +1316,7 @@
         tile = next;
     }
     if (SH == 1 && dob && i < kvalid) pbias[((size_t)(split * 2 + grp) * 2 + h) * K + k0 + i] = bsum;
+    if (SH == 2 && dob && i < kvalid) pbias[(((size_t)(split * 2 + grp) * 2 + h) * 4 + wave) * K + k0 + i] = bsum;
 #pragma unroll
     for (int j = 0; j < TPW; j++) {
         const int t = wave + 4 * j;
@@ -1866,7 +1940,8 @@
 
 template <int NAS, int NB>
 __global__ __launch_bounds__(256, 2) void k_wgrad_smallc(const WgradGeom g, const WgTile tg, const float *__restrict__ a1,
-                                                         const float *__restrict__ b, float *__restrict__ partial) {
+                                                         const float *__restrict__ b, float *__restrict__ partial,
+                                                         float *__restrict__ pbias) {
     extern __shared__ __attribute__((aligned(16))) float lds[];
     float *As = lds;
     float *Bs = lds + (size_t)NAS * 1024;
@@ -1885,6 +1960,7 @@
     const bool rvalid = row < g.ntaps * C;
     const int rtap = rvalid ? row / C : 0, rc = rvalid ? row % C : 0;
     const int arow = (toffs[rtap] * C + rc) * 4 + h * g.sa[2] * C * 4;
+    const bool ones = pbias != nullptr && row == g.ntaps * C;
     const int k0 = kb * 32;
     const int kvalid = (K - k0) < 32 ? (K - k0) : 32;
     const int EAhw = tg.EAh * tg.EAw, EBhw = tg.EBh * tg.EBw;
@@ -1941,6 +2017,7 @@
         const int sa_ = ((dz * g.sa[0]) * tg.EAh + hy * g.sa[1]) * tg.EAw + wx * g.sa[2];
         const int sb_ = ((dz * g.sb[0]) * tg.EBh + hy * g.sb[1]) * tg.EBw + wx * g.sb[2];
         av = *reinterpret_cast<const float *>(Ab + sa_ * C * 4 + arow);
+        av = ones ? 1.f : av;
         bv = *reinterpret_cast<const float *>(Bb + sb_ * 128 + tb0);
     };
     int tile = split;
@@ -1975,6 +2052,7 @@
             const int t = rr / C, c = rr - t * C;
             partial[(((size_t)split * g.ntaps + t) * C + c) * K + k0 + i] = acc[r];
         }
+        if (pbias && rr == g.ntaps * C && i < kvalid) pbias[(size_t)split * K + k0 + i] = acc[r];
     }
 }
 
@@ -2380,6 +2458,13 @@
     return (int)ns;
 }
 
+static int g_wgrad_bias_fold = -1;
+static bool wgrad_bias_fold() {
+    if (g_wgrad_bias_fold < 0) g_wgrad_bias_fold = getenv("MVD_WGRAD_BIAS_FOLD") ? (atoi(getenv("MVD_WGRAD_BIAS_FOLD")) != 0) : 1;
+    return g_wgrad_bias_fold != 0;
+}
+void set_wgrad_bias_fold(int on) { g_wgrad_bias_fold = on < 0 ? -1 : (on != 0); }
+
 static bool wgrad_mfma_ok(const WgradGeom &g) {
     const int C = g.C1 + g.C2;
     if (g.ntaps < 1 || g.ntaps > 27) return false;
@@ -2391,7 +2476,7 @@
 
 size_t wgrad_mfma_ws(const WgradGeom &g) {
     if (!wgrad_mfma_ok(g)) return 0;
-    size_t ws = (size_t)wgrad_max_split(g) * (g.ntaps * (size_t)(g.C1 + g.C2) + 2) * g.K * sizeof(float) + 256;
+    size_t ws = (size_t)wgrad_max_split(g) * (g.ntaps * (size_t)(g.C1 + g.C2) + 8) * g.K * sizeof(float) + 256;
     const int C = g.C1 + g.C2;
     if (g.ntaps == 27 && C % 32 == 0 && g.K % 32 == 0) {
         const size_t w3 = wgrad_wino3_ws(wgrad_max_split(g, 1), C, g.K) + 256;
@@ -2546,7 +2631,8 @@
             }                                                                                                      \
             cfgd() = true;                                                                                           \
         }                                                                                                          \
-        hipLaunchKernelGGL(kern, grid, dim3(512), lds, s, g, tg, a1, a2, b, partial, (SH) == 1 ? pbias_g : nullptr); \
+        hipLaunchKernelGGL(kern, grid, dim3(512), lds, s, g, tg, a1, a2, b, partial,                               \
+                           (SH) == 1 ? pbias_g : (SH) == 2 ? pbias_t : nullptr);                                    \
     }
     bool sameA = true, sameB = true;
     for (int t = 1; t < g.ntaps; t++) {
@@ -2693,11 +2779,23 @@
         if ((size_t)ns2 * g.ntaps * C * g.K * sizeof(float) <= ws_bytes) tg.nsplit = (int)ns2;
         auto kern = k_wgrad_smallc<2, 4>;
         const size_t lds2 = (size_t)(2 + 4) * 4096 + 32 * 4;
-        hipLaunchKernelGGL(kern, dim3(tg.nsplit, tg.nkb), dim3(256), lds2, s, g, tg, a1, b, partial);
+        const size_t need_s = (size_t)tg.nsplit * g.ntaps * C * g.K * sizeof(float);
+        float *pbias_s = nullptr;
+        if (wgrad_bias_fold() && dbias && dbias_done && g.ntaps * C < 128 && g.sb[0] == 1 && g.sb[1] == 1 && g.sb[2] == 1 &&
+            need_s + (size_t)tg.nsplit * g.K * sizeof(float) <= ws_bytes)
+            pbias_s = partial + need_s / sizeof(float);
+        hipLaunchKernelGGL(kern, dim3(tg.nsplit, tg.nkb), dim3(256), lds2, s, g, tg, a1, b, partial, pbias_s);
         if (check_launch("conv wgrad (mfma, narrow input)")) return 1;
         const long per2 = (long)g.ntaps * C * g.K;
-        launch_wgrad_reduce_f((unsigned)(cdiv(per2, 64)), s, g, partial, dw, tg.nsplit, (const float *)nullptr,
-                           (float *)nullptr, 0, 0);
+        const int wblocks2 = (int)cdiv(per2, 64);
+        if (pbias_s) {
+            launch_wgrad_reduce_f((unsigned)(wblocks2 + cdiv(g.K, 64)), s, g, partial, dw, tg.nsplit, (const float *)pbias_s,
+                               dbias, tg.nsplit, wblocks2);
+            *dbias_done = 1;
+        } else {
+            launch_wgrad_reduce_f((unsigned)wblocks2, s, g, partial, dw, tg.nsplit, (const float *)nullptr, (float *)nullptr, 0,
+                               0);
+        }
         return check_launch("conv wgrad reduce (mfma)");
     }
 #define WG_TPW(NA, NB, SH)                     \
@@ -2715,6 +2813,15 @@
     float *pbias_g = nullptr;
     if (dbias && dbias_done && cfg == 0 && sameB && need_g + (size_t)4 * tg.nsplit * g.K * sizeof(float) <= ws_bytes)
         pbias_g = partial + need_g / sizeof(float);
+    float *pbias_t = nullptr;
+    if (wgrad_bias_fold() && dbias && dbias_done && cfg == 1 && sameA && g.ntaps == 4 * tpw &&
+        g.ntaps == g.sb[0] * g.sb[1] * g.sb[2] && need_g + (size_t)16 * tg.nsplit * g.K * sizeof(float) <= ws_bytes) {
+        bool box = true;
+        for (int t = 0; t < g.ntaps; t++)
+            box = box && g.ob[t][0] == t / (g.sb[1] * g.sb[2]) && g.ob[t][1] == (t / g.sb[2]) % g.sb[1] &&
+                  g.ob[t][2] == t % g.sb[2];
+        if (box) pbias_t = partial + need_g / sizeof(float);
+    }
     if (cfg == 0) {
         if (sameB) WG_TPW(7, 2, 1)
         else WG_TPW(7, 2, 0)
@@ -2731,6 +2838,10 @@
         launch_wgrad_reduce_f((unsigned)(wblocks + cdiv(g.K, 64)), s, g, partial, dw, 2 * tg.nsplit,
                            (const float *)pbias_g, dbias, tg.nsplit * 4, wblocks);
         *dbias_done = 1;
+    } else if (pbias_t && cfg == 1) {
+        launch_wgrad_reduce_f((unsigned)(wblocks + cdiv(g.K, 64)), s, g, partial, dw, 2 * tg.nsplit,
+                           (const float *)pbias_t, dbias, tg.nsplit * 16, wblocks);
+        *dbias_done = 1;
     } else {
         launch_wgrad_reduce_f((unsigned)(wblocks), s, g, partial, dw, 2 * tg.nsplit, (const float *)nullptr,
                            (float *)nullptr, 0, 0);
diff --git a/multimodal_mvd_seg_amd/csrc/instnorm.hip b/multimodal_mvd_seg_amd/csrc/instnorm.hip
--- a/multimodal_mvd_seg_amd/csrc/instnorm.hip
+++ b/multimodal_mvd_seg_amd/csrc/instnorm.hip
@@ -258,16 +258,40 @@
     }
 }
 
+constexpr int HKMAX = 8;
+template <int HK>
+__device__ __forceinline__ void head_w_load(float4 (&wk)[HK], const float *__restrict__ w, int C, int g) {
+#pragma unroll
+    for (int k = 0; k < HK; k++) wk[k] = *reinterpret_cast<const float4 *>(w + (size_t)k * C + g * 4);
+}
+template <int HK>
+__device__ __forceinline__ void head_dl_load(float (&dq)[HK], const float *__restrict__ dl, int n, long V, long v) {
+#pragma unroll
+    for (int k = 0; k < HK; k++) dq[k] = dl[((size_t)n * HK + k) * V + v];
+}
+template <int HK>
+__device__ __forceinline__ float4 head_da(const float (&dq)[HK], const float4 (&wk)[HK]) {
+    float4 a = make_float4(0.f, 0.f, 0.f, 0.f);
+#pragma unroll
+    for (int k = 0; k < HK; k++) {
+        a.x = fmaf(dq[k], wk[k].x, a.x);
+        a.y = fmaf(dq[k], wk[k].y, a.y);
+        a.z = fmaf(dq[k], wk[k].z, a.z);
+        a.w = fmaf(dq[k], wk[k].w, a.w);
+    }
+    return a;
+}
+
 #ifndef MVD_IN_NRB
 #define MVD_IN_NRB 4
 #endif
 constexpr int NRB = MVD_IN_NRB;
-template <bool XB, bool YB>
-__global__ void k_in_bwd_apply_rows(const float *__restrict__ x, const float *__restrict__ dy,
+template <bool XB, bool YB, int HK = 0>
+__global__ __launch_bounds__(HK > 0 ? 256 : 1024) void k_in_bwd_apply_rows(const float *__restrict__ x, const float *__restrict__ dy,
                                     const float *__restrict__ gamma, const float *__restrict__ beta,
                                     const float *__restrict__ mean, const float *__restrict__ rstd,
                                     const float *__restrict__ sums, float *__restrict__ dx, int C, int CG, int R, long V,
-                                    long chunk, float slope) {
+                                    long chunk, float slope, const float *__restrict__ hw = nullptr) {
     const int n = blockIdx.y, t = threadIdx.x;
     const int g = t % CG, r = t / CG;
     if (r >= R) return;
@@ -288,13 +312,26 @@
         m2[i] = sums[nc * 2 + 1] * invV;
     }
     const size_t base = ((size_t)n * V) * C + (size_t)g * 4;
+    float4 wk[HK > 0 ? HK : 1];
+    if constexpr (HK > 0) head_w_load(wk, hw, C, g);
     long v = v0 + r;
     for (; v + (NRB - 1L) * R < v1; v += (long)NRB * R) {
         float4 q[NRB], e[NRB];
-#pragma unroll
-        for (int u = 0; u < NRB; u++) {
-            q[u] = ld4<XB>(x, base + (size_t)(v + (long)u * R) * C);
-            e[u] = ld4<YB>(dy, base + (size_t)(v + (long)u * R) * C);
+        if constexpr (HK > 0) {
+            float dq[NRB][HK];
+#pragma unroll
+            for (int u = 0; u < NRB; u++) {
+                q[u] = ld4<XB>(x, base + (size_t)(v + (long)u * R) * C);
+                head_dl_load(dq[u], dy, n, V, v + (long)u * R);
+            }
+#pragma unroll
+            for (int u = 0; u < NRB; u++) e[u] = head_da(dq[u], wk);
+        } else {
+#pragma unroll
+            for (int u = 0; u < NRB; u++) {
+                q[u] = ld4<XB>(x, base + (size_t)(v + (long)u * R) * C);
+                e[u] = ld4<YB>(dy, base + (size_t)(v + (long)u * R) * C);
+            }
         }
 #pragma unroll
         for (int u = 0; u < NRB; u++) {
@@ -311,7 +348,13 @@
     }
     for (; v < v1; v += R) {
         float4 q = ld4<XB>(x, base + (size_t)v * C);
-        float4 e = ld4<YB>(dy, base + (size_t)v * C);
+        float4 e;
+        if constexpr (HK > 0) {
+            float dq[HK];
+            head_dl_load(dq, dy, n, V, v);
+            e = head_da(dq, wk);
+        } else
+            e = ld4<YB>(dy, base + (size_t)v * C);
         float f[4] = {q.x, q.y, q.z, q.w}, d[4] = {e.x, e.y, e.z, e.w};
 #pragma unroll
         for (int i = 0; i < 4; i++) {
@@ -324,11 +367,13 @@
     }
 }
 
-template <int VEC, bool XB, bool YB>
-__global__ void k_in_bwd_stats(const float *__restrict__ x, const float *__restrict__ dy,
+template <int VEC, bool XB, bool YB, int HK = 0>
+__global__ __launch_bounds__(HK > 0 ? 256 : 1024) void k_in_bwd_stats(const float *__restrict__ x, const float *__restrict__ dy,
                                const float *__restrict__ gamma, const float *__restrict__ beta,
                                const float *__restrict__ mean, const float *__restrict__ rstd,
-                               double *__restrict__ partial, int C, int CG, int R, long V, long chunk, float slope) {
+                               double *__restrict__ partial, int C, int CG, int R, long V, long chunk, float slope,
+                               const float *__restrict__ hw = nullptr) {
+    static_assert(HK == 0 || VEC == 4, "the head form works on 4-channel groups");
     extern __shared__ double sm[];
     const int n = blockIdx.y, b = blockIdx.x, nblk = gridDim.x;
     const int t = threadIdx.x;
@@ -350,11 +395,23 @@
             be[i] = beta[c];
         }
         const size_t base = ((size_t)n * V) * C + (size_t)g * VEC;
+        float4 wk[HK > 0 ? HK : 1];
+        if constexpr (HK > 0) head_w_load(wk, hw, C, g);
         long v = v0 + r;
         if (VEC == 4) {
             for (; v + R < v1; v += 2L * R) {
-                const float4 q0 = ld4<XB>(x, base + (size_t)v * C), e0 = ld4<YB>(dy, base + (size_t)v * C);
-                const float4 q1 = ld4<XB>(x, base + (size_t)(v + R) * C), e1 = ld4<YB>(dy, base + (size_t)(v + R) * C);
+                const float4 q0 = ld4<XB>(x, base + (size_t)v * C), q1 = ld4<XB>(x, base + (size_t)(v + R) * C);
+                float4 e0, e1;
+                if constexpr (HK > 0) {
+                    float d0[HK], d1[HK];
+                    head_dl_load(d0, dy, n, V, v);
+                    head_dl_load(d1, dy, n, V, v + R);
+                    e0 = head_da(d0, wk);
+                    e1 = head_da(d1, wk);
+                } else {
+                    e0 = ld4<YB>(dy, base + (size_t)v * C);
+                    e1 = ld4<YB>(dy, base + (size_t)(v + R) * C);
+                }
                 const float fx[2][4] = {{q0.x, q0.y, q0.z, q0.w}, {q1.x, q1.y, q1.z, q1.w}};
                 const float dd[2][4] = {{e0.x, e0.y, e0.z, e0.w}, {e1.x, e1.y, e1.z, e1.w}};
 #pragma unroll
@@ -371,9 +428,15 @@
         }
         for (; v < v1; v += R) {
             float f[VEC], d[VEC];
-            if (VEC == 4) {
+            if constexpr (VEC == 4) {
                 float4 q = ld4<XB>(x, base + (size_t)v * C);
-                float4 e = ld4<YB>(dy, base + (size_t)v * C);
+                float4 e;
+                if constexpr (HK > 0) {
+                    float dq[HK];
+                    head_dl_load(dq, dy, n, V, v);
+                    e = head_da(dq, wk);
+                } else
+                    e = ld4<YB>(dy, base + (size_t)v * C);
                 f[0] = q.x; f[1] = q.y; f[2] = q.z; f[3] = q.w;
                 d[0] = e.x; d[1] = e.y; d[2] = e.z; d[3] = e.w;
             } else {
@@ -560,11 +623,210 @@
     }
 }
 
+constexpr int SMW = 4;
+constexpr int SM_MAXR = 16;
+__device__ __forceinline__ void small_reduce(double (&s)[4], double (&ss)[4], double (*sm)[SMW][8], int gl) {
+#pragma unroll
+    for (int off = SMW; off < 64; off <<= 1)
+#pragma unroll
+        for (int i = 0; i < 4; i++) {
+            s[i] += __shfl_xor(s[i], off);
+            ss[i] += __shfl_xor(ss[i], off);
+        }
+    const int wv = threadIdx.x >> 6, nw = blockDim.x >> 6;
+    if (nw == 1) return;
+    if ((threadIdx.x & 63) < SMW)
+#pragma unroll
+        for (int i = 0; i < 4; i++) {
+            sm[wv][gl][2 * i] = s[i];
+            sm[wv][gl][2 * i + 1] = ss[i];
+        }
+    __syncthreads();
+#pragma unroll
+    for (int i = 0; i < 4; i++) s[i] = ss[i] = 0.0;
+    for (int w = 0; w < nw; w++)
+#pragma unroll
+        for (int i = 0; i < 4; i++) {
+            s[i] += sm[w][gl][2 * i];
+            ss[i] += sm[w][gl][2 * i + 1];
+        }
+}
+
+template <int MAXR>
+__global__ __launch_bounds__(256) void k_in_small_fwd(const float *__restrict__ x, const float *__restrict__ gamma,
+                                                       const float *__restrict__ beta, float *__restrict__ y,
+                                                       float *__restrict__ mean, float *__restrict__ rstd, int C, long V,
+                                                       float eps, float slope) {
+    __shared__ double sm[4][SMW][8];
+    const int n = blockIdx.y, gl = threadIdx.x % SMW, r = threadIdx.x / SMW, RP = blockDim.x / SMW;
+    const int g = blockIdx.x * SMW + gl;
+    const bool act = g < (C >> 2);
+    const size_t base = ((size_t)n * V) * C + (size_t)g * 4;
+    float4 q[MAXR];
+#pragma unroll
+    for (int j = 0; j < MAXR; j++) {
+        const long v = r + (long)j * RP;
+        q[j] = (act && v < V) ? ld4<false>(x, base + (size_t)v * C) : make_float4(0.f, 0.f, 0.f, 0.f);
+    }
+    double s[4] = {0, 0, 0, 0}, ss[4] = {0, 0, 0, 0};
+#pragma unroll
+    for (int j = 0; j < MAXR; j++) {
+        const float f[4] = {q[j].x, q[j].y, q[j].z, q[j].w};
+#pragma unroll
+        for (int i = 0; i < 4; i++) {
+            s[i] += (double)f[i];
+            ss[i] += (double)f[i] * (double)f[i];
+        }
+    }
+    small_reduce(s, ss, sm, gl);
+    if (!act) return;
+    float mu[4], rs[4], ga[4], be[4];
+#pragma unroll
+    for (int i = 0; i < 4; i++) {
+        const double m = s[i] / (double)V;
+        double var = ss[i] / (double)V - m * m;
+        if (var < 0) var = 0;
+        mu[i] = (float)m;
+        rs[i] = (float)(1.0 / sqrt(var + (double)eps));
+        ga[i] = gamma[g * 4 + i];
+        be[i] = beta[g * 4 + i];
+    }
+    if (r == 0)
+#pragma unroll
+        for (int i = 0; i < 4; i++) {
+            mean[(size_t)n * C + g * 4 + i] = mu[i];
+            rstd[(size_t)n * C + g * 4 + i] = rs[i];
+        }
+#pragma unroll
+    for (int j = 0; j < MAXR; j++) {
+        const long v = r + (long)j * RP;
+        if (v < V) {
+            float f[4] = {q[j].x, q[j].y, q[j].z, q[j].w};
+#pragma unroll
+            for (int i = 0; i < 4; i++) {
+                const float xh = (f[i] - mu[i]) * rs[i];
+                const float z = fmaf(xh, ga[i], be[i]);
+                f[i] = z > 0.f ? z : z * slope;
+            }
+            st4<false>(y, base + (size_t)v * C, f[0], f[1], f[2], f[3]);
+        }
+    }
+}
+
+template <int MAXR>
+__global__ __launch_bounds__(256) void k_in_small_bwd(const float *__restrict__ x, const float *__restrict__ dy,
+                                                       const float *__restrict__ gamma, const float *__restrict__ beta,
+                                                       const float *__restrict__ mean, const float *__restrict__ rstd,
+                                                       float *__restrict__ dx, float *__restrict__ dgamma,
+                                                       float *__restrict__ dbeta, int N, int C, long V, float slope) {
+    __shared__ double sm[4][SMW][8];
+    const int gl = threadIdx.x % SMW, r = threadIdx.x / SMW, RP = blockDim.x / SMW;
+    const int g = blockIdx.x * SMW + gl;
+    const bool act = g < (C >> 2);
+    const int gc = act ? g : 0;
+    const float invV = 1.0f / (float)V;
+    float ga[4], be[4];
+#pragma unroll
+    for (int i = 0; i < 4; i++) {
+        ga[i] = gamma[gc * 4 + i];
+        be[i] = beta[gc * 4 + i];
+    }
+    double tg[4] = {0, 0, 0, 0}, tb[4] = {0, 0, 0, 0};
+    for (int n = 0; n < N; n++) {
+        const size_t base = ((size_t)n * V) * C + (size_t)gc * 4;
+        float mu[4], rs[4];
+#pragma unroll
+        for (int i = 0; i < 4; i++) {
+            mu[i] = mean[(size_t)n * C + gc * 4 + i];
+            rs[i] = rstd[(size_t)n * C + gc * 4 + i];
+        }
+        float4 q[MAXR], e[MAXR];
+#pragma unroll
+        for (int j = 0; j < MAXR; j++) {
+            const long v = r + (long)j * RP;
+            const bool in = act && v < V;
+            q[j] = in ? ld4<false>(x, base + (size_t)v * C) : make_float4(0.f, 0.f, 0.f, 0.f);
+            e[j] = in ? ld4<false>(dy, base + (size_t)v * C) : make_float4(0.f, 0.f, 0.f, 0.f);
+        }
+        double s[4] = {0, 0, 0, 0}, ss[4] = {0, 0, 0, 0};
+#pragma unroll
+        for (int j = 0; j < MAXR; j++) {
+            float f[4] = {q[j].x, q[j].y, q[j].z, q[j].w}, d[4] = {e[j].x, e[j].y, e[j].z, e[j].w};
+#pragma unroll
+            for (int i = 0; i < 4; i++) {
+                const float xh = (f[i] - mu[i]) * rs[i];
+                const float z = fmaf(xh, ga[i], be[i]);
+                const float dz = z > 0.f ? d[i] : d[i] * slope;
+                s[i] += (double)dz;
+                ss[i] += (double)dz * (double)xh;
+                f[i] = xh;
+                d[i] = dz;
+            }
+            q[j] = make_float4(f[0], f[1], f[2], f[3]);
+            e[j] = make_float4(d[0], d[1], d[2], d[3]);
+        }
+        if (n > 0) __syncthreads();
+        small_reduce(s, ss, sm, gl);
+        float m1[4], m2[4];
+#pragma unroll
+        for (int i = 0; i < 4; i++) {
+            m1[i] = (float)s[i] * invV;
+            m2[i] = (float)ss[i] * invV;
+            tb[i] += s[i];
+            tg[i] += ss[i];
+        }
+#pragma unroll
+        for (int j = 0; j < MAXR; j++) {
+            const long v = r + (long)j * RP;
+            if (act && v < V) {
+                const float xh[4] = {q[j].x, q[j].y, q[j].z, q[j].w}, dz[4] = {e[j].x, e[j].y, e[j].z, e[j].w};
+                float f[4];
+#pragma unroll
+                for (int i = 0; i < 4; i++) f[i] = ga[i] * rs[i] * (dz[i] - m1[i] - xh[i] * m2[i]);
+                st4<false>(dx, base + (size_t)v * C, f[0], f[1], f[2], f[3]);
+            }
+        }
+    }
+    if (act && r == 0)
+#pragma unroll
+        for (int i = 0; i < 4; i++) {
+            dgamma[g * 4 + i] = (float)tg[i];
+            dbeta[g * 4 + i] = (float)tb[i];
+        }
+}
+
 }
 
 using namespace mvd;
 
+constexpr long kInSmallMaxDefault = 327680;
+static long g_in_small_launches = 0;
+static int in_small_threads(long V) {
+    for (int t = 64; t <= 256; t *= 4)
+        if ((long)(t / SMW) * SM_MAXR >= V) return t;
+    return 0;
+}
+static long g_in_small_max = -1;
+static int in_small_ok(long V, int C, int nb = 0) {
+    static const int on = getenv("MVD_IN_SMALL") ? atoi(getenv("MVD_IN_SMALL")) : 1;
+    if (g_in_small_max < 0)
+        g_in_small_max = getenv("MVD_IN_SMALL_MAX") ? atol(getenv("MVD_IN_SMALL_MAX")) : kInSmallMaxDefault;
+    if (!on || C % 4 != 0 || V <= 0) return 0;
+    const long elems = V * C;
+    if (nb > 2 ? elems * nb > 2 * g_in_small_max : elems > g_in_small_max) return 0;
+    return in_small_threads(V);
+}
+
 extern "C" {
+
+int mvd_instnorm_single_launch(long V, int C) { return in_small_ok(V, C) > 0 ? 1 : 0; }
+long mvd_instnorm_single_launches(void) { return g_in_small_launches; }
+static long g_in_stats_pass_launches = 0;
+long mvd_instnorm_stats_pass_launches(void) { return g_in_stats_pass_launches; }
+int mvd_set_instnorm_small_max(long max_elems) {
+    g_in_small_max = max_elems < 0 ? -1 : max_elems;
+    return 0;
+}
 
 int mvd_instnorm_nblk(int N, long V, int C) { return norm_geom(N, V, C).nblk; }
 
@@ -581,6 +843,14 @@
     MVD_REQUIRE(ws_bytes >= mvd_instnorm_workspace_bytes(N, V, C), "instnorm_fwd: workspace too small");
     NormGeom g = norm_geom(N, V, C);
     hipStream_t s = as_stream(stream);
+    if (!xb && !yb) {
+        if (const int th = in_small_ok(V, C)) {
+            hipLaunchKernelGGL(k_in_small_fwd<SM_MAXR>, dim3(cdiv(C / 4, SMW), N), dim3(th), 0, s, x, gamma, beta, y, mean, rstd,
+                               C, V, eps, slope);
+            g_in_small_launches++;
+            return check_launch("instnorm forward (single launch)");
+        }
+    }
     double *partial = reinterpret_cast<double *>(ws);
     size_t sm = (size_t)g.R * C * 2 * sizeof(double);
     MVD_REQUIRE(sm <= 64 * 1024, "instnorm_fwd: C too large for the LDS reduce");
@@ -606,6 +876,7 @@
             hipLaunchKernelGGL((k_in_stats<4, false>), grid, dim3(g.threads), sm, s, x, partial, C, g.CG, g.R, V, g.chunk);
         else
             hipLaunchKernelGGL((k_in_stats<1, false>), grid, dim3(g.threads), sm, s, x, partial, C, g.CG, g.R, V, g.chunk);
+        g_in_stats_pass_launches++;
         if (check_launch("instnorm stats")) return 1;
         float *ss = reinterpret_cast<float *>(partial + (size_t)N * g.nblk * C * 2);
         const bool ssf = v4 && xb && yb;
@@ -646,12 +917,20 @@
 
 static int in_bwd(const float *x, bool xb, const float *dy, bool yb, const float *gamma, const float *beta,
                   const float *mean, const float *rstd, float *dx, float *dgamma, float *dbeta, int N, long V, int C,
-                  float slope, void *ws, size_t ws_bytes, void *stream) {
+                  float slope, void *ws, size_t ws_bytes, void *stream, const float *head_w = nullptr, int K = 0) {
     MVD_REQUIRE(x && dy && gamma && beta && mean && rstd && dx && dgamma && dbeta && ws, "instnorm_bwd: null pointer");
     MVD_REQUIRE(N > 0 && N <= 65535 && V > 0 && C > 0 && C <= 1024, "instnorm_bwd: bad shape");
     MVD_REQUIRE(ws_bytes >= mvd_instnorm_workspace_bytes(N, V, C), "instnorm_bwd: workspace too small");
     NormGeom g = norm_geom(N, V, C);
     hipStream_t s = as_stream(stream);
+    if (!xb && !yb && !head_w) {
+        if (const int th = in_small_ok(V, C, N)) {
+            hipLaunchKernelGGL(k_in_small_bwd<SM_MAXR>, dim3(cdiv(C / 4, SMW)), dim3(th), 0, s, x, dy, gamma, beta, mean, rstd, dx,
+                               dgamma, dbeta, N, C, V, slope);
+            g_in_small_launches++;
+            return check_launch("instnorm backward (single launch)");
+        }
+    }
     double *partial = reinterpret_cast<double *>(ws);
     float *sums = reinterpret_cast<float *>(partial + (size_t)N * g.nblk * C * 2);
     size_t sm = (size_t)g.R * C * 2 * sizeof(double);
@@ -659,11 +938,25 @@
     const bool v4 = (C % 4 == 0) && (g.CG * 4 == C);
     dim3 grid(g.nblk, N);
     MVD_REQUIRE(v4 || !(xb || yb), "instnorm_bwd: bf16 I/O needs C %% 4 == 0");
-    if (v4) {
+    MVD_REQUIRE(!head_w || (v4 && !xb && !yb && K > 0 && K <= HKMAX),
+                "instnorm_bwd: the logit-gradient form needs fp32, C %% 4 == 0 and K <= 8");
+    if (head_w) {
+        MVD_REQUIRE(g.threads <= 256, "instnorm_bwd: block size of the logit-gradient form");
+#define MVD_HEAD_STATS(KK)                                                                                                      \
+    case KK:                                                                                                                    \
+        hipLaunchKernelGGL((k_in_bwd_stats<4, false, false, KK>), grid, dim3(g.threads), sm, s, x, dy, gamma, beta, mean, rstd, \
+                           partial, C, g.CG, g.R, V, g.chunk, slope, head_w);                                                   \
+        break;
+        switch (K) {
+            MVD_HEAD_STATS(1) MVD_HEAD_STATS(2) MVD_HEAD_STATS(3) MVD_HEAD_STATS(4)
+            MVD_HEAD_STATS(5) MVD_HEAD_STATS(6) MVD_HEAD_STATS(7) MVD_HEAD_STATS(8)
+        }
+#undef MVD_HEAD_STATS
+    } else if (v4) {
         auto kern = xb ? (yb ? k_in_bwd_stats<4, true, true> : k_in_bwd_stats<4, true, false>)
                        : (yb ? k_in_bwd_stats<4, false, true> : k_in_bwd_stats<4, false, false>);
         hipLaunchKernelGGL(kern, grid, dim3(g.threads), sm, s, x, dy, gamma, beta, mean, rstd, partial, C, g.CG, g.R, V,
-                           g.chunk, slope);
+                           g.chunk, slope, (const float *)nullptr);
     } else
         hipLaunchKernelGGL((k_in_bwd_stats<1, false, false>), grid, dim3(g.threads), sm, s, x, dy, gamma, beta, mean, rstd,
                            partial, C, g.CG, g.R, V, g.chunk, slope);
@@ -683,8 +976,20 @@
         const long chunk2 = cdiv(V, nb2);
         auto kern = xb ? (yb ? k_in_bwd_apply_rows<true, true> : k_in_bwd_apply_rows<true, false>)
                        : (yb ? k_in_bwd_apply_rows<false, true> : k_in_bwd_apply_rows<false, false>);
-        hipLaunchKernelGGL(kern, dim3((unsigned)cdiv(V, chunk2), N), dim3(g.threads), 0, s, x, dy, gamma, beta, mean, rstd,
-                           sums, dx, C, g.CG, g.R, V, chunk2, slope);
+        if (head_w) {
+#define MVD_HEAD_APPLY(KK)                                                                                                        \
+    case KK:                                                                                                                      \
+        hipLaunchKernelGGL((k_in_bwd_apply_rows<false, false, KK>), dim3((unsigned)cdiv(V, chunk2), N), dim3(g.threads), 0, s, x, \
+                           dy, gamma, beta, mean, rstd, sums, dx, C, g.CG, g.R, V, chunk2, slope, head_w);                        \
+        break;
+            switch (K) {
+                MVD_HEAD_APPLY(1) MVD_HEAD_APPLY(2) MVD_HEAD_APPLY(3) MVD_HEAD_APPLY(4)
+                MVD_HEAD_APPLY(5) MVD_HEAD_APPLY(6) MVD_HEAD_APPLY(7) MVD_HEAD_APPLY(8)
+            }
+#undef MVD_HEAD_APPLY
+        } else
+            hipLaunchKernelGGL(kern, dim3((unsigned)cdiv(V, chunk2), N), dim3(g.threads), 0, s, x, dy, gamma, beta, mean, rstd,
+                               sums, dx, C, g.CG, g.R, V, chunk2, slope, (const float *)nullptr);
     }
     else
         hipLaunchKernelGGL(k_in_bwd_apply<1>, dim3(bx, N), dim3(256), 0, s, x, dy, gamma, beta, mean, rstd, sums, dx, C,
@@ -701,6 +1006,14 @@
                            const float *rstd, float *dx, float *dgamma, float *dbeta, int N, long V, int C,
                            float slope, void *ws, size_t ws_bytes, void *stream) {
     return in_bwd(x, false, dy, false, gamma, beta, mean, rstd, dx, dgamma, dbeta, N, V, C, slope, ws, ws_bytes, stream);
+}
+
+int mvd_instnorm_lrelu_bwd_head(const float *x, const float *dlogits, const float *w, int K, const float *gamma,
+                                const float *beta, const float *mean, const float *rstd, float *dx, float *dgamma,
+                                float *dbeta, int N, long V, int C, float slope, void *ws, size_t ws_bytes, void *stream) {
+    MVD_REQUIRE(w && (((uintptr_t)w) & 15) == 0, "instnorm_bwd_head: head weight (16-byte aligned) required");
+    return in_bwd(x, false, dlogits, false, gamma, beta, mean, rstd, dx, dgamma, dbeta, N, V, C, slope, ws, ws_bytes, stream, w,
+                  K);
 }
 
 int mvd_instnorm_lrelu_fwd_prestats(const float *x, const float *tile_stats, long ntiles, const float *gamma,
diff --git a/multimodal_mvd_seg_amd/ops.py b/multimodal_mvd_seg_amd/ops.py
--- a/multimodal_mvd_seg_amd/ops.py
+++ b/multimodal_mvd_seg_amd/ops.py
@@ -449,6 +449,7 @@
 
 
 BF16_CONV_STATS = [os.environ.get("MVD_BF16_CONV_STATS", "1") != "0"]
+DIRECT_CONV_STATS = [os.environ.get("MVD_DIRECT_CONV_STATS", "1") != "0"]
 
 
 def conv3d_fwd_bf16(x1, C1, x2, C2, wf, bias, y, N, D, H, W, K, ks, stride, ws, in_scale=None, in_shift=None, slope=0.01):
@@ -516,8 +517,19 @@
                 if done.value:
                     y._mvd_tile_stats = (stats, ntiles)
             else:
-                call("mvd_conv3d_fwd_wino", _p(x1), C1, _p(x2), C2, _p(wf), _p(uf), _p(bias), _p(y), N, D, H, W, K, i3(ks),
-                     i3(stride), _p(ws), ws.numel(), _stream())
+                ntiles = 0
+                if DIRECT_CONV_STATS[0] and len(ks) == 3 and not query("mvd_instnorm_single_launch", od[0] * od[1] * od[2], K):
+                    ntiles = query("mvd_conv3d_fwd_stats_tiles", N, D, H, W, C1, C2, K, i3(ks), i3(stride))
+                if ntiles > 0:
+                    stats = torch.empty((N, ntiles, K, 2), dtype=torch.float32, device=x1.device)
+                    done = ctypes.c_int(0)
+                    call("mvd_conv3d_fwd_stats", _p(x1), C1, _p(x2), C2, _p(wf), _p(bias), _p(y), _p(stats), ntiles,
+                         ctypes.byref(done), N, D, H, W, K, i3(ks), i3(stride), _p(ws), ws.numel(), _stream())
+                    if done.value:
+                        y._mvd_tile_stats = (stats, ntiles)
+                else:
+                    call("mvd_conv3d_fwd_wino", _p(x1), C1, _p(x2), C2, _p(wf), _p(uf), _p(bias), _p(y), N, D, H, W, K, i3(ks),
+                         i3(stride), _p(ws), ws.numel(), _stream())
         if timed:
             ev1 = torch.cuda.Event(enable_timing=True)
             ev1.record()
@@ -959,6 +971,9 @@
         return (None if joined is not None else dx), dw.view(ctx.wshape), db
 
 
+NORM_BWD_FROM_DL = [os.environ.get("MVD_NORM_BWD_FROM_DL", "1") != "0"]
+
+
 class NormActSegHeadFn(Function):
 
     @staticmethod
@@ -1012,7 +1027,8 @@
         dev = y0.device
         dl = dl.contiguous()
         need_x = ctx.needs_input_grad[0] or ctx.needs_input_grad[1] or ctx.needs_input_grad[2]
-        da = empty_cl3d(y0.shape, dev, y0.dtype) if need_x else None
+        from_dl = need_x and not bf and NORM_BWD_FROM_DL[0]
+        da = empty_cl3d(y0.shape, dev, y0.dtype) if need_x and not from_dl else None
         dw = torch.empty((K, C), dtype=torch.float32, device=dev)
         db = torch.empty((K,), dtype=torch.float32, device=dev)
         ws = _Workspace.get(query("mvd_seghead_bwd_workspace_bytes", N, V, C, K), dev)
@@ -1029,7 +1045,10 @@
             dg = sink_g if sink_g is not None else torch.empty((C,), dtype=torch.float32, device=dev)
             db_ = sink_b if sink_b is not None else torch.empty((C,), dtype=torch.float32, device=dev)
             ws = _Workspace.get(query("mvd_instnorm_workspace_bytes", N, V, C), dev)
-            if bf:
+            if from_dl:
+                call("mvd_instnorm_lrelu_bwd_head", _p(y0), _p(dl), _p(w), K, _p(g), _p(b), _p(mean), _p(rstd), _p(dy0), _p(dg),
+                     _p(db_), N, V, C, ctx.slope, _p(ws), ws.numel(), _stream())
+            elif bf:
                 call("mvd_instnorm_lrelu_bwd_bf16", _p(y0), 1, _p(da), _p(g), _p(b), _p(mean), _p(rstd), _p(dy0), _p(dg),
                      _p(db_), N, V, C, ctx.slope, _p(ws), ws.numel(), _stream())
             else:
```

Result: faster. 61.31 samples/s, median of 6 (+1.8%).
